# chzhang18/RAG

Hardware: AMD Instinct MI355X
Metric: disparity maps/sec at 384x1248 D=192 (Matching-Net forward) (higher is better)
Workload: dtype f32 (RAGMI_F32X3: level-3/6/12 3x3x3 convolutions with fp32 operands split into power-of-two-scaled FP16 hi+lo halves on the 16-bit matrix cores, hi*hi + hi*lo + lo*hi, fp32 accumulate: fp32-class accuracy, bound in include/rag_amd.h; strict_fp32 holds the RAGMI_F32 number); 1 GPU; BASELINE configs[1]: 1 stereo pair(s)/GPU/step, 384x1248, D=192, f32, all-conv genotype, (left_fea,right_fea)->disp, inputs resident in HBM; global_batch=1, launch=hipGraph, ranks_seen=1

## Files before the change

### include/rag_amd.h

```cpp
#ifndef RAG_AMD_H
#define RAG_AMD_H

#include <stdint.h>

#ifdef __cplusplus
extern "C" {
#endif

#define RAGMI_OK 0
#define RAGMI_EINVAL (-1)
#define RAGMI_EUNSUPPORTED (-2)
#define RAGMI_ELAUNCH (-3)

#define RAGMI_F32 0
#define RAGMI_BF16 1
#define RAGMI_F32X3 2

#define RAGMI_MAX_GROUPS 16

int ragmi_version(void);
const char* ragmi_last_error(void);

int ragmi_costvol_fwd(const void* left_fea, const void* right_fea, void* cost,
                      int B, int C, int d, int h, int w, int dtype, void* stream);

int64_t ragmi_conv3d_k3_packed_elems(int Cout, int Cin);
int ragmi_conv3d_k3_pack(const void* weight, void* packed, int Cout, int Cin, int dtype, void* stream);

int ragmi_conv3d_k3_fwd(const void* x, int64_t x_bstride,
                        const void* packed_weight, const void* scale, const void* shift, int relu,
                        void* y, int64_t y_bstride, const int32_t* y_group_ch,
                        const void* res, int64_t res_bstride, const int32_t* res_group_ch,
                        int B, int Cin, int Cout, int D, int H, int W,
                        int dtype, void* stream);

typedef struct {
  const void* weight;
  const void* scale;
  const void* shift;
  int32_t relu;
  void* y;
  int64_t y_bstride;
  int32_t y_ch0;
  int32_t cout;
} ragmi_tail_t;
int ragmi_down2_tail_supported(int D, int H, int W);

#define RAGMI_CONV_RELU 1
#define RAGMI_CONV_X_G4 2
#define RAGMI_CONV_Y_G4 4
#define RAGMI_TAIL_G4 4
#define RAGMI_TAIL_F32 8
#define RAGMI_TAIL_ROWS 16
#define RAGMI_OUT_F32 0x100
int ragmi_conv3d_k3_g4_caps(int Cin, int Cout, int B, int D, int H, int W, int nset, int ntail, int ndown, int dtype);

#define RAGMI_STORE_QUARTER_ROWS 2
int ragmi_conv3d_k3_quarter_store_supported(int Cin, int Cout, int B, int D, int H, int W, int nset, int ntail, int ndown, int dtype);
int ragmi_quarter_store_rows(int n_in, unsigned char* used);

int ragmi_conv3d_k3_fwd_ex(const void* x, int64_t x_bstride,
                           const void* packed_weight, const void* scale, const void* shift, int relu,
                           void* y, int64_t y_bstride, const int32_t* y_group_ch,
                           const void* res, int64_t res_bstride, const int32_t* res_group_ch,
                           int B, int Cin, int Cout, int D, int H, int W,
                           int store_main, int ntail, const ragmi_tail_t* tails, int dtype, void* stream);
int ragmi_conv3d_k3_dual_fwd_ex(const void* x, int64_t x_bstride,
                                int CinA, const void* packedA, const void* scaleA, const void* shiftA,
                                int CinB, const void* packedB, const void* scaleB, const void* shiftB,
                                int relu, void* y, int64_t y_bstride, const int32_t* y_group_ch,
                                const void* res, int64_t res_bstride, const int32_t* res_group_ch,
                                int B, int Cout, int D, int H, int W,
                                int store_main, int ntail, const ragmi_tail_t* tails, int dtype, void* stream);

int ragmi_conv3d_k3_small_fwd(const void* x, int64_t x_bstride, const void* weight, const void* scale,
                              const void* shift, int relu, void* y, int64_t y_bstride, int y_ch0,
                              const void* res, int64_t res_bstride, int res_ch0,
                              int B, int Cin, int Cout, int D, int H, int W, int dtype, void* stream);

int ragmi_conv3d_k3_small_fwd_ex(const void* x, int64_t x_bstride, const void* weight, const void* scale,
                                 const void* shift, int relu, void* y, int64_t y_bstride, int y_ch0,
                                 const void* res, int64_t res_bstride, int res_ch0,
                                 int B, int Cin, int Cout, int D, int H, int W, int dtype, int y_dtype, void* stream);

int ragmi_conv3d_k3_dual_fwd(const void* x, int64_t x_bstride,
                             int CinA, const void* packedA, const void* scaleA, const void* shiftA,
                             int CinB, const void* packedB, const void* scaleB, const void* shiftB,
                             int relu, void* y, int64_t y_bstride, const int32_t* y_group_ch,
                             const void* res, int64_t res_bstride, const int32_t* res_group_ch,
                             int B, int Cout, int D, int H, int W, int dtype, void* stream);

int ragmi_conv3d_k3_plan(int Cout, int B, int D, int H, int W, int nset, int32_t* log_tx,
                         int32_t* rows_per_lane, int32_t* launch_groups, int32_t max_launches);

int ragmi_conv3d_k1_fwd(const void* x, int64_t x_bstride,
                        const void* weight, const void* scale, const void* shift, int relu,
                        void* y, int64_t y_bstride, int y_ch0,
                        int B, int Cin, int Cout, int64_t DHW,
                        int dtype, void* stream);

int ragmi_conv3d_k1_chain_supported(int Cin, int Cmid, int Cout);
int ragmi_conv3d_k1_chain_fwd(const void* x, int64_t x_bstride, const void* weight1, const void* scale1, const void* shift1, int relu1,
                              int Cmid, const void* weight2, const void* scale2, const void* shift2, int relu2,
                              void* y, int64_t y_bstride, int y_ch0, int B, int Cin, int Cout, int64_t DHW, int dtype, void* stream);

int ragmi_conv3d_k1_fwd_ex(const void* x, int64_t x_bstride, const void* weight, int w_transposed, const void* scale,
                           const void* shift, int relu, void* y, int64_t y_bstride, int y_ch0, int B, int Cin,
                           int Cout, int64_t DHW, int dtype, void* stream);

int ragmi_conv3d_k1_resample_fwd(const void* x, int64_t x_bstride, int Di, int Hi, int Wi,
                                 const void* weight, const void* scale, const void* shift, int relu,
                                 void* y, int64_t y_bstride, int y_ch0,
                                 int B, int Cin, int Cout, int Do, int Ho, int Wo, int align_corners,
                                 int dtype, void* stream);

typedef struct {
  const void* x;
  int64_t x_bstride;
  int32_t Di, Hi, Wi;
  const void* weight;
  const void* scale;
  const void* shift;
  int32_t relu;
  int32_t y_ch0;
  int32_t Cin, Cout;
} ragmi_k1r_t;
int ragmi_conv3d_k1_resample_pair_fwd(const ragmi_k1r_t* a, const ragmi_k1r_t* b, void* y, int64_t y_bstride,
                                      int B, int Do, int Ho, int Wo, int align_corners, int dtype, void* stream);
int ragmi_conv3d_k1_resample_multi_fwd(const ragmi_k1r_t* const* specs, void* const* ys, const int64_t* y_bstrides, int n, int B,
                                       int Do, int Ho, int Wo, int align_corners, int dtype, void* stream);

typedef struct {
  const void* x;
  int64_t x_bstride;
  int32_t Cin, Hi, Wi;
  const void* weight;
  const void* scale;
  const void* shift;
  int32_t relu;
} ragmi_cell2d_in_t;
int ragmi_cell2d_supported(int C, int Cin0, int Cin1, int Cout, int H, int W, int dtype);
int ragmi_cell2d_fwd(const ragmi_cell2d_in_t* s0, const ragmi_cell2d_in_t* s1, int C, const void* packedA, const void* scaleA,
                     const void* shiftA, const void* packedB, const void* scaleB, const void* shiftB, int relu, void* y,
                     int64_t y_bstride, const int32_t* y_group_ch, int B, int Cout, int H, int W, int dtype, void* stream);

int ragmi_trilinear3d_fwd(const void* x, void* y, int B, int C,
                          int Di, int Hi, int Wi, int Do, int Ho, int Wo,
                          int align_corners, int dtype, void* stream);

int ragmi_upconv3d_c1_supported(int Cin, int Di, int Hi, int Wi);
int ragmi_upconv3d_c1_fwd(const void* x, int64_t x_bstride, const void* weight, const void* scale, const void* shift, int relu, void* y,
                          int64_t y_bstride, int y_ch0, int B, int Cin, int Di, int Hi, int Wi, int dtype, int y_dtype, void* stream);

int ragmi_trilinear3d_act_fwd(const void* x, int64_t x_bstride, void* y, int64_t y_bstride, int y_ch0, int relu, int B, int C,
                              int Di, int Hi, int Wi, int Do, int Ho, int Wo, int align_corners, int dtype, void* stream);

int ragmi_conv2d_k3_strided_fwd(const void* x, const void* weight, const void* scale, const void* shift, int relu,
                                void* y, int B, int Cin, int Cout, int H, int W, int stride, int dtype, void* stream);

int ragmi_add_fwd(const void* a, int64_t a_bstride, int a_ch0,
                  const void* b, int64_t b_bstride, int b_ch0,
                  void* y, int64_t y_bstride, int y_ch0,
                  int B, int C, int64_t DHW, int dtype, void* stream);

int ragmi_disp_softargmin_fwd(const void* cost, void* out, int B, int d, int h, int w,
                              int maxdisp, int Ho, int Wo, int dtype, void* stream);

int ragmi_disparity_regression_fwd(const void* prob, void* out, int B, int D, int H, int W,
                                   int dtype, void* stream);

int64_t ragmi_costvol_stem_weights_elems(int C, int Cout);
int ragmi_costvol_stem_prepare(const void* weight, void* variants, int C, int Cout, void* stream);
int64_t ragmi_costvol_stem_workspace_elems(int B, int C, int Cout, int D, int H, int W);
int ragmi_costvol_stem_fwd(const void* left, const void* right, const void* variants, const void* scale, const void* shift, int relu,
                           void* y, int64_t y_bstride, void* workspace, int B, int C, int Cout, int D, int H, int W,
                           int ntail, const ragmi_tail_t* tails, int dtype, void* stream);

int ragmi_costvol_stem_conv3d_supported(int C, int Cmid, int Cout, int B, int D, int H, int W, int ntail, int dtype);
int ragmi_costvol_stem_conv3d_fwd(const void* left, const void* right, const void* variants, const void* scale0, const void* shift0, int relu0,
                                  void* workspace, int ntail0, const ragmi_tail_t* tails0,
                                  const void* packed_weight, const void* scale, const void* shift, int relu,
                                  void* y, int64_t y_bstride, const int32_t* y_group_ch, int store_main, int ntail, const ragmi_tail_t* tails,
                                  int B, int C, int Cmid, int Cout, int D, int H, int W, int dtype, void* stream);

int ragmi_conv3d_k3_uses_x3(int Cin, int Cout, int B, int D, int H, int W, int nset, int has_res, int ntail, int dtype);

int ragmi_conv3d_k3_pack_ex(const void* weight, void* packed, int Cout, int Cin, int transpose, int planar2d, int dtype, void* stream);

int ragmi_conv3d_k3_pack_for(const void* weight, void* packed, int Cout, int Cin, int transpose, int planar2d, int for_dtype, void* stream);


int64_t ragmi_bn_workspace_elems(int B, int C, int64_t DHW);
int ragmi_bn_train_stats_fwd(const void* x, int64_t x_bstride, int B, int C, int64_t DHW, const void* gamma, const void* beta,
                             void* running_mean, void* running_var, void* num_batches_tracked, float momentum, float eps,
                             void* workspace, void* mean, void* invstd, void* scale, void* shift, void* stream);

int ragmi_bn_train_act_fwd(const void* x, int64_t x_bstride, int B, int C, int64_t DHW, const void* gamma, const void* beta,
                           void* running_mean, void* running_var, void* num_batches_tracked, float momentum, float eps, int relu,
                           void* workspace, void* mean, void* invstd, void* scale, void* shift, void* y, int64_t y_bstride, int y_ch0,
                           const void* res, int64_t res_bstride, int res_ch0, void* stream);

int ragmi_bn_act_bwd(const void* dy, int64_t dy_bstride, int dy_ch0, const void* x, int64_t x_bstride, const void* scale,
                     const void* shift, int relu, const void* mean, const void* invstd, int training, int B, int C, int64_t DHW,
                     void* workspace, void* dx, int64_t dx_bstride, void* dgamma, void* dbeta, int accumulate, void* stream);

int ragmi_bn_act_fwd(const void* x, int64_t x_bstride, const void* scale, const void* shift, int relu,
                     const void* res, int64_t res_bstride, int res_ch0,
                     void* y, int64_t y_bstride, int y_ch0, int B, int C, int64_t DHW, void* stream);

int ragmi_bn_act_bwd_coeffs(const void* dy, int64_t dy_bstride, int dy_ch0, const void* x, int64_t x_bstride,
                            const void* scale, const void* shift, int relu, const void* mean, const void* invstd, int training,
                            int B, int C, int64_t DHW, void* workspace, void* c1, void* c2, void* c3, void* dgamma, void* dbeta,
                            int accumulate, void* stream);

int ragmi_bn_act_bwd_apply(const void* dy, int64_t dy_bstride, int dy_ch0, const void* x, int64_t x_bstride,
                           const void* scale, const void* shift, int relu, const void* c1, const void* c2, const void* c3,
                           void* dx, int64_t dx_bstride, int B, int C, int64_t DHW, void* stream);

int64_t ragmi_conv3d_k3_wgrad_workspace_elems(int B, int Cin, int Cout, int D, int H, int W);
int ragmi_conv3d_k3_wgrad(const void* x, int64_t x_bstride, const void* g, int64_t g_bstride, int g_ch0, void* const* dw_list, int n_dw,
                          int accumulate, int planar2d, void* workspace, int B, int Cin, int Cout, int D, int H, int W, void* stream);

int ragmi_conv3d_k1_wgrad(const void* x, int64_t x_bstride, const void* g, int64_t g_bstride, int g_ch0, void* dw,
                          int B, int Cin, int Cout, int64_t DHW, void* stream);

int ragmi_trilinear3d_bwd(const void* dy, void* dx, int B, int C, int Di, int Hi, int Wi, int Do, int Ho, int Wo,
                          int align_corners, void* stream);

int ragmi_costvol_bwd(const void* dcost, void* dleft, void* dright, int B, int C, int d, int h, int w, void* stream);

int ragmi_disp_softargmin_bwd(const void* cost, const void* dout, void* dcost, int B, int d, int h, int w,
                              int maxdisp, int Ho, int Wo, void* stream);

int ragmi_conv2d_k3_strided_dgrad(const void* g, const void* weight, void* dx, int B, int Cin, int Cout, int H, int W, int stride,
                                  void* stream);
int ragmi_conv2d_k3_strided_wgrad(const void* x, const void* g, void* dw, int B, int Cin, int Cout, int H, int W, int stride,
                                  void* stream);

int ragmi_disparity_regression_bwd(const void* dout, void* dprob, int B, int D, int H, int W, void* stream);

int ragmi_stereo_metrics_fwd(const void* disp_est, const void* disp_gt, int B, int H, int W, float maxdisp, void* acc, void* out,
                             void* stream);

int ragmi_masked_smooth_l1_bwd(const void* disp_est, const void* disp_gt, const void* out, const void* gout, void* ddisp,
                               int B, int H, int W, float maxdisp, void* stream);

int64_t ragmi_selfsup_loss_workspace_elems(int B, int H, int W);
int ragmi_selfsup_loss_fwd(const void* left, const void* right, const void* disp, int B, int C, int H, int W, int dtype,
                           void* workspace, void* out, void* unit_grad, void* stream);

int ragmi_selfsup_loss_bwd(const void* unit_grad, const void* gout, void* grad, int64_t n, void* stream);

int ragmi_depth_head_supported(int Cin, int Hi, int Wi, int H, int W, int scale, int dtype);
int ragmi_depth_head_fwd(const void* y, const void* w3, const void* w1, const void* b1, void* out, int B, int Cin, int Hi, int Wi,
                         int H, int W, int scale, float max_depth, int dtype, void* stream);

int ragmi_depth_metrics_workspace_elems(long long n);
int ragmi_depth_metrics_fwd(const void* est, const void* gt, long long n, float variance_focus, void* workspace, void* out10, int dtype,
                            void* stream);

int64_t ragmi_depth_head_bwd_workspace_elems(int B, int Cin, int H, int W);
int ragmi_depth_head_bwd(const void* y, const void* w3, const void* w1, const void* b1, const void* d_out, void* dy, void* dw3,
                         void* dw1, void* db1, int accumulate, void* workspace, int B, int Cin, int Hi, int Wi, int H, int W, int scale,
                         float max_depth, int dtype, void* stream);

int ragmi_silog_loss_workspace_elems(long long n);
int ragmi_silog_loss_fwd(const void* est, const void* gt, long long n, float variance_focus, void* workspace, void* out, void* saved,
                         int dtype, void* stream);

int ragmi_silog_loss_bwd(const void* est, const void* gt, long long n, float variance_focus, const void* saved, const void* gout,
                         void* grad, int dtype, void* stream);

int64_t ragmi_sgd_workspace_bytes(void);
int ragmi_sgd_clip_step(void* param, void* grad, void* momentum_buf, int64_t n, float lr, float momentum, float weight_decay,
                        float max_norm, int first_step, void* workspace, void* norm_out, void* stream);

#define RAGMI_GT_F32 0
#define RAGMI_GT_U16 1
int ragmi_prep_batch(const void* left_u8, const void* right_u8, const void* gt, int gt_dtype, float gt_scale, const void* origin,
                     void* left, void* right, void* gt_out, int B, int Hs, int Ws, int H, int W, float mean0, float mean1, float mean2,
                     float std0, float std1, float std2, const void* stats_left, const void* stats_right, const void* stats_source,
                     void* stream);

int64_t ragmi_color_stats_workspace_elems(int B, int Hs, int Ws);
int ragmi_color_stats(const void* img_u8, int B, int Hs, int Ws, void* workspace, void* stats, void* stream);

int ragmi_color_transfer(const void* target_u8, const void* stats_target, const void* stats_source, void* out_u8, int B, int H, int W,
                         void* stream);

int ragmi_prep_batch_resized(const void* left_u8, const void* right_u8, const void* gt, int gt_dtype, float gt_scale, const void* origin,
                             void* left, void* right, void* gt_out, int B, int Hs, int Ws, int Hr, int Wr, int H, int W, float mean0,
                             float mean1, float mean2, float std0, float std1, float std2, const void* ybounds, const void* ytaps_i32,
                             const void* ytaps_f64, int yksize, const void* xbounds, const void* xtaps_i32, const void* xtaps_f64,
                             int xksize, void* stream);
int ragmi_resize_lanczos_u8(const void* src_u8, void* dst_u8, int B, int Hs, int Ws, int Hr, int Wr, const void* ybounds,
                            const void* ytaps_i32, int yksize, const void* xbounds, const void* xtaps_i32, int xksize, void* stream);
int ragmi_resize_lanczos_u16(const void* src_u16, void* dst_u16, int B, int Hs, int Ws, int Hr, int Wr, const void* ybounds,
                             const void* ytaps_f64, int yksize, const void* xbounds, const void* xtaps_f64, int xksize, void* stream);

int ragmi_graph_node_census(void* graph, int32_t* n_kernel, int32_t* n_memcpy, int32_t* n_memset, int32_t* n_other);

#ifdef __cplusplus
}
#endif
#endif
```

### rag_amd/_lib.py

```python
import ctypes
import os
import threading

_HERE = os.path.dirname(os.path.abspath(__file__))
_LIB = None
_LOCK = threading.Lock()

c_void_p, c_int, c_int64, c_float = ctypes.c_void_p, ctypes.c_int, ctypes.c_int64, ctypes.c_float
c_int32_p = ctypes.POINTER(ctypes.c_int32)

class TailSpec(ctypes.Structure):
    _fields_ = [("weight", c_void_p), ("scale", c_void_p), ("shift", c_void_p), ("relu", ctypes.c_int32),
                ("y", c_void_p), ("y_bstride", c_int64), ("y_ch0", ctypes.c_int32), ("cout", ctypes.c_int32)]


c_tail_p = ctypes.POINTER(TailSpec)


class K1RSpec(ctypes.Structure):
    _fields_ = [("x", c_void_p), ("x_bstride", c_int64), ("Di", ctypes.c_int32), ("Hi", ctypes.c_int32), ("Wi", ctypes.c_int32),
                ("weight", c_void_p), ("scale", c_void_p), ("shift", c_void_p), ("relu", ctypes.c_int32),
                ("y_ch0", ctypes.c_int32), ("Cin", ctypes.c_int32), ("Cout", ctypes.c_int32)]


c_k1r_p = ctypes.POINTER(K1RSpec)


class Cell2dIn(ctypes.Structure):
    _fields_ = [("x", c_void_p), ("x_bstride", c_int64), ("Cin", ctypes.c_int32), ("Hi", ctypes.c_int32), ("Wi", ctypes.c_int32),
                ("weight", c_void_p), ("scale", c_void_p), ("shift", c_void_p), ("relu", ctypes.c_int32)]


c_cell2d_p = ctypes.POINTER(Cell2dIn)

SIGNATURES = {
    "ragmi_version": (c_int, []),
    "ragmi_last_error": (ctypes.c_char_p, []),
    "ragmi_graph_node_census": (c_int, [c_void_p, c_int32_p, c_int32_p, c_int32_p, c_int32_p]),
    "ragmi_costvol_fwd": (c_int, [c_void_p, c_void_p, c_void_p, c_int, c_int, c_int, c_int, c_int, c_int, c_void_p]),
    "ragmi_costvol_stem_weights_elems": (c_int64, [c_int, c_int]),
    "ragmi_costvol_stem_prepare": (c_int, [c_void_p, c_void_p, c_int, c_int, c_void_p]),
    "ragmi_costvol_stem_workspace_elems": (c_int64, [c_int, c_int, c_int, c_int, c_int, c_int]),
    "ragmi_costvol_stem_fwd": (c_int, [c_void_p, c_void_p, c_void_p, c_void_p, c_void_p, c_int, c_void_p, c_int64, c_void_p,
                                       c_int, c_int, c_int, c_int, c_int, c_int, c_int, c_tail_p, c_int, c_void_p]),
    "ragmi_costvol_stem_conv3d_supported": (c_int, [c_int] * 9),
    "ragmi_costvol_stem_conv3d_fwd": (c_int, [c_void_p, c_void_p, c_void_p, c_void_p, c_void_p, c_int, c_void_p, c_int, c_tail_p,
                                              c_void_p, c_void_p, c_void_p, c_int, c_void_p, c_int64, c_int32_p, c_int, c_int, c_tail_p,
                                              c_int, c_int, c_int, c_int, c_int, c_int, c_int, c_int, c_void_p]),
    "ragmi_conv3d_k3_uses_x3": (c_int, [c_int] * 10),
    "ragmi_conv3d_k3_g4_caps": (c_int, [c_int] * 10),
    "ragmi_conv3d_k3_quarter_store_supported": (c_int, [c_int] * 10),
    "ragmi_quarter_store_rows": (c_int, [c_int, ctypes.POINTER(ctypes.c_ubyte)]),
    "ragmi_conv3d_k3_packed_elems": (c_int64, [c_int, c_int]),
    "ragmi_conv3d_k3_pack": (c_int, [c_void_p, c_void_p, c_int, c_int, c_int, c_void_p]),
    "ragmi_conv3d_k3_fwd": (c_int, [c_void_p, c_int64, c_void_p, c_void_p, c_void_p, c_int,
                                    c_void_p, c_int64, c_int32_p, c_void_p, c_int64, c_int32_p,
                                    c_int, c_int, c_int, c_int, c_int, c_int, c_int, c_void_p]),
    "ragmi_conv3d_k3_small_fwd": (c_int, [c_void_p, c_int64, c_void_p, c_void_p, c_void_p, c_int, c_void_p, c_int64, c_int,
                                          c_void_p, c_int64, c_int, c_int, c_int, c_int, c_int, c_int, c_int, c_int, c_void_p]),
    "ragmi_conv3d_k3_small_fwd_ex": (c_int, [c_void_p, c_int64, c_void_p, c_void_p, c_void_p, c_int, c_void_p, c_int64, c_int,
                                             c_void_p, c_int64, c_int, c_int, c_int, c_int, c_int, c_int, c_int, c_int, c_int, c_void_p]),
    "ragmi_conv3d_k3_dual_fwd": (c_int, [c_void_p, c_int64, c_int, c_void_p, c_void_p, c_void_p,
                                         c_int, c_void_p, c_void_p, c_void_p, c_int, c_void_p, c_int64, c_int32_p,
                                         c_void_p, c_int64, c_int32_p, c_int, c_int, c_int, c_int, c_int, c_int, c_void_p]),
    "ragmi_conv3d_k3_fwd_ex": (c_int, [c_void_p, c_int64, c_void_p, c_void_p, c_void_p, c_int,
                                       c_void_p, c_int64, c_int32_p, c_void_p, c_int64, c_int32_p,
                                       c_int, c_int, c_int, c_int, c_int, c_int, c_int, c_int, c_tail_p, c_int, c_void_p]),
    "ragmi_conv3d_k3_dual_fwd_ex": (c_int, [c_void_p, c_int64, c_int, c_void_p, c_void_p, c_void_p,
                                            c_int, c_void_p, c_void_p, c_void_p, c_int, c_void_p, c_int64, c_int32_p,
                                            c_void_p, c_int64, c_int32_p, c_int, c_int, c_int, c_int, c_int,
                                            c_int, c_int, c_tail_p, c_int, c_void_p]),
    "ragmi_conv3d_k3_plan": (c_int, [c_int, c_int, c_int, c_int, c_int, c_int, c_int32_p, c_int32_p, c_int32_p, c_int]),
    "ragmi_conv3d_k1_fwd": (c_int, [c_void_p, c_int64, c_void_p, c_void_p, c_void_p, c_int,
                                    c_void_p, c_int64, c_int, c_int, c_int, c_int, c_int64, c_int, c_void_p]),
    "ragmi_conv3d_k1_chain_supported": (c_int, [c_int] * 3),
    "ragmi_conv3d_k1_chain_fwd": (c_int, [c_void_p, c_int64, c_void_p, c_void_p, c_void_p, c_int, c_int, c_void_p, c_void_p, c_void_p, c_int,
                                          c_void_p, c_int64, c_int, c_int, c_int, c_int, c_int64, c_int, c_void_p]),
    "ragmi_conv3d_k1_fwd_ex": (c_int, [c_void_p, c_int64, c_void_p, c_int, c_void_p, c_void_p, c_int,
                                       c_void_p, c_int64, c_int, c_int, c_int, c_int, c_int64, c_int, c_void_p]),
    "ragmi_conv3d_k1_resample_fwd": (c_int, [c_void_p, c_int64, c_int, c_int, c_int, c_void_p, c_void_p, c_void_p, c_int,
                                             c_void_p, c_int64, c_int, c_int, c_int, c_int, c_int, c_int, c_int, c_int, c_int, c_void_p]),
    "ragmi_conv3d_k1_resample_pair_fwd": (c_int, [c_k1r_p, c_k1r_p, c_void_p, c_int64, c_int, c_int, c_int, c_int, c_int, c_int, c_void_p]),
    "ragmi_conv3d_k1_resample_multi_fwd": (c_int, [ctypes.POINTER(c_k1r_p), ctypes.POINTER(c_void_p), ctypes.POINTER(c_int64), c_int, c_int,
                                                   c_int, c_int, c_int, c_int, c_int, c_void_p]),
    "ragmi_down2_tail_supported": (c_int, [c_int, c_int, c_int]),
    "ragmi_cell2d_supported": (c_int, [c_int] * 7),
    "ragmi_cell2d_fwd": (c_int, [c_cell2d_p, c_cell2d_p, c_int, c_void_p, c_void_p, c_void_p, c_void_p, c_void_p, c_void_p, c_int,
                                 c_void_p, c_int64, c_int32_p, c_int, c_int, c_int, c_int, c_int, c_void_p]),
    "ragmi_upconv3d_c1_supported": (c_int, [c_int, c_int, c_int, c_int]),
    "ragmi_upconv3d_c1_fwd": (c_int, [c_void_p, c_int64, c_void_p, c_void_p, c_void_p, c_int, c_void_p, c_int64, c_int, c_int, c_int, c_int,
                                      c_int, c_int, c_int, c_int, c_void_p]),
    "ragmi_trilinear3d_act_fwd": (c_int, [c_void_p, c_int64, c_void_p, c_int64, c_int, c_int, c_int, c_int, c_int, c_int, c_int, c_int,
                                          c_int, c_int, c_int, c_int, c_void_p]),
    "ragmi_trilinear3d_fwd": (c_int, [c_void_p, c_void_p, c_int, c_int, c_int, c_int, c_int, c_int, c_int, c_int,
                                      c_int, c_int, c_void_p]),
    "ragmi_conv2d_k3_strided_fwd": (c_int, [c_void_p, c_void_p, c_void_p, c_void_p, c_int, c_void_p, c_int, c_int, c_int, c_int, c_int,
                                            c_int, c_int, c_void_p]),
    "ragmi_add_fwd": (c_int, [c_void_p, c_int64, c_int, c_void_p, c_int64, c_int, c_void_p, c_int64, c_int,
                              c_int, c_int, c_int64, c_int, c_void_p]),
    "ragmi_bn_workspace_elems": (c_int64, [c_int, c_int, c_int64]),
    "ragmi_bn_train_stats_fwd": (c_int, [c_void_p, c_int64, c_int, c_int, c_int64, c_void_p, c_void_p, c_void_p, c_void_p, c_void_p,
                                         c_float, c_float, c_void_p, c_void_p, c_void_p, c_void_p, c_void_p, c_void_p]),
    "ragmi_conv3d_k3_pack_ex": (c_int, [c_void_p, c_void_p, c_int, c_int, c_int, c_int, c_int, c_void_p]),
    "ragmi_conv3d_k3_pack_for": (c_int, [c_void_p, c_void_p, c_int, c_int, c_int, c_int, c_int, c_void_p]),
    "ragmi_sgd_workspace_bytes": (c_int64, []),
    "ragmi_sgd_clip_step": (c_int, [c_void_p, c_void_p, c_void_p, c_int64, c_float, c_float, c_float, c_float, c_int, c_void_p, c_void_p,
                                    c_void_p]),
    "ragmi_bn_train_act_fwd": (c_int, [c_void_p, c_int64, c_int, c_int, c_int64, c_void_p, c_void_p, c_void_p, c_void_p, c_void_p, c_float,
                                       c_float, c_int, c_void_p, c_void_p, c_void_p, c_void_p, c_void_p, c_void_p, c_int64, c_int,
                                       c_void_p, c_int64, c_int, c_void_p]),
    "ragmi_bn_act_bwd": (c_int, [c_void_p, c_int64, c_int, c_void_p, c_int64, c_void_p, c_void_p, c_int, c_void_p, c_void_p, c_int, c_int,
                                 c_int, c_int64, c_void_p, c_void_p, c_int64, c_void_p, c_void_p, c_int, c_void_p]),
    "ragmi_bn_act_fwd": (c_int, [c_void_p, c_int64, c_void_p, c_void_p, c_int, c_void_p, c_int64, c_int, c_void_p, c_int64, c_int,
                                 c_int, c_int, c_int64, c_void_p]),
    "ragmi_bn_act_bwd_coeffs": (c_int, [c_void_p, c_int64, c_int, c_void_p, c_int64, c_void_p, c_void_p, c_int, c_void_p, c_void_p, c_int,
                                        c_int, c_int, c_int64, c_void_p, c_void_p, c_void_p, c_void_p, c_void_p, c_void_p, c_int, c_void_p]),
    "ragmi_bn_act_bwd_apply": (c_int, [c_void_p, c_int64, c_int, c_void_p, c_int64, c_void_p, c_void_p, c_int, c_void_p, c_void_p,
                                       c_void_p, c_void_p, c_int64, c_int, c_int, c_int64, c_void_p]),
    "ragmi_conv3d_k3_wgrad_workspace_elems": (c_int64, [c_int, c_int, c_int, c_int, c_int, c_int]),
    "ragmi_conv3d_k3_wgrad": (c_int, [c_void_p, c_int64, c_void_p, c_int64, c_int, ctypes.POINTER(c_void_p), c_int, c_int, c_int, c_void_p,
                                      c_int, c_int, c_int, c_int, c_int, c_int, c_void_p]),
    "ragmi_conv3d_k1_wgrad": (c_int, [c_void_p, c_int64, c_void_p, c_int64, c_int, c_void_p, c_int, c_int, c_int, c_int64, c_void_p]),
    "ragmi_trilinear3d_bwd": (c_int, [c_void_p, c_void_p, c_int, c_int, c_int, c_int, c_int, c_int, c_int, c_int, c_int, c_void_p]),
    "ragmi_costvol_bwd": (c_int, [c_void_p, c_void_p, c_void_p, c_int, c_int, c_int, c_int, c_int, c_void_p]),
    "ragmi_conv2d_k3_strided_dgrad": (c_int, [c_void_p, c_void_p, c_void_p, c_int, c_int, c_int, c_int, c_int, c_int, c_void_p]),
    "ragmi_conv2d_k3_strided_wgrad": (c_int, [c_void_p, c_void_p, c_void_p, c_int, c_int, c_int, c_int, c_int, c_int, c_void_p]),
    "ragmi_disparity_regression_bwd": (c_int, [c_void_p, c_void_p, c_int, c_int, c_int, c_int, c_void_p]),
    "ragmi_stereo_metrics_fwd": (c_int, [c_void_p, c_void_p, c_int, c_int, c_int, c_float, c_void_p, c_void_p, c_void_p]),
    "ragmi_masked_smooth_l1_bwd": (c_int, [c_void_p, c_void_p, c_void_p, c_void_p, c_void_p, c_int, c_int, c_int, c_float, c_void_p]),
    "ragmi_selfsup_loss_workspace_elems": (c_int64, [c_int, c_int, c_int]),
    "ragmi_selfsup_loss_fwd": (c_int, [c_void_p, c_void_p, c_void_p, c_int, c_int, c_int, c_int, c_int, c_void_p, c_void_p, c_void_p,
                                       c_void_p]),
    "ragmi_selfsup_loss_bwd": (c_int, [c_void_p, c_void_p, c_void_p, c_int64, c_void_p]),
    "ragmi_depth_head_supported": (c_int, [c_int] * 7),
    "ragmi_depth_head_fwd": (c_int, [c_void_p, c_void_p, c_void_p, c_void_p, c_void_p, c_int, c_int, c_int, c_int, c_int, c_int, c_int,
                                     c_float, c_int, c_void_p]),
    "ragmi_depth_metrics_workspace_elems": (c_int, [ctypes.c_longlong]),
    "ragmi_depth_metrics_fwd": (c_int, [c_void_p, c_void_p, ctypes.c_longlong, c_float, c_void_p, c_void_p, c_int, c_void_p]),
    "ragmi_depth_head_bwd_workspace_elems": (c_int64, [c_int, c_int, c_int, c_int]),
    "ragmi_depth_head_bwd": (c_int, [c_void_p, c_void_p, c_void_p, c_void_p, c_void_p, c_void_p, c_void_p, c_void_p, c_void_p, c_int,
                                     c_void_p, c_int, c_int, c_int, c_int, c_int, c_int, c_int, c_float, c_int, c_void_p]),
    "ragmi_silog_loss_workspace_elems": (c_int, [ctypes.c_longlong]),
    "ragmi_silog_loss_fwd": (c_int, [c_void_p, c_void_p, ctypes.c_longlong, c_float, c_void_p, c_void_p, c_void_p, c_int, c_void_p]),
    "ragmi_silog_loss_bwd": (c_int, [c_void_p, c_void_p, ctypes.c_longlong, c_float, c_void_p, c_void_p, c_void_p, c_int, c_void_p]),
    "ragmi_prep_batch": (c_int, [c_void_p, c_void_p, c_void_p, c_int, c_float, c_void_p, c_void_p, c_void_p, c_void_p,
                                 c_int, c_int, c_int, c_int, c_int, c_float, c_float, c_float, c_float, c_float, c_float,
                                 c_void_p, c_void_p, c_void_p, c_void_p]),
    "ragmi_color_stats_workspace_elems": (c_int64, [c_int, c_int, c_int]),
    "ragmi_color_stats": (c_int, [c_void_p, c_int, c_int, c_int, c_void_p, c_void_p, c_void_p]),
    "ragmi_color_transfer": (c_int, [c_void_p, c_void_p, c_void_p, c_void_p, c_int, c_int, c_int, c_void_p]),
    "ragmi_prep_batch_resized": (c_int, [c_void_p, c_void_p, c_void_p, c_int, c_float, c_void_p, c_void_p, c_void_p, c_void_p,
                                         c_int, c_int, c_int, c_int, c_int, c_int, c_int, c_float, c_float, c_float, c_float, c_float,
                                         c_float, c_void_p, c_void_p, c_void_p, c_int, c_void_p, c_void_p, c_void_p, c_int, c_void_p]),
    "ragmi_resize_lanczos_u8": (c_int, [c_void_p, c_void_p, c_int, c_int, c_int, c_int, c_int, c_void_p, c_void_p, c_int, c_void_p,
                                        c_void_p, c_int, c_void_p]),
    "ragmi_resize_lanczos_u16": (c_int, [c_void_p, c_void_p, c_int, c_int, c_int, c_int, c_int, c_void_p, c_void_p, c_int, c_void_p,
                                         c_void_p, c_int, c_void_p]),
    "ragmi_disp_softargmin_bwd": (c_int, [c_void_p, c_void_p, c_void_p, c_int, c_int, c_int, c_int, c_int, c_int, c_int, c_void_p]),
    "ragmi_disp_softargmin_fwd": (c_int, [c_void_p, c_void_p, c_int, c_int, c_int, c_int, c_int, c_int, c_int,
                                          c_int, c_void_p]),
    "ragmi_disparity_regression_fwd": (c_int, [c_void_p, c_void_p, c_int, c_int, c_int, c_int, c_int, c_void_p]),
}


def lib_path() -> str:
    return os.environ.get("RAG_AMD_LIB", os.path.join(_HERE, "lib", "librag_amd.so"))


def load_library():
    global _LIB
    if _LIB is not None:
        return _LIB
    with _LOCK:
        if _LIB is None:
            path = lib_path()
            if not os.path.exists(path):
                raise RuntimeError(
                    f"rag_amd: HIP library not found at {path}. Build it with `make` at the repo root "
                    "(or `python -c 'import __graft_entry__ as g; g.build()'`). There is no CPU fallback.")
            lib = ctypes.CDLL(path)
            for name, (restype, argtypes) in SIGNATURES.items():
                fn = getattr(lib, name)
                fn.restype = restype
                fn.argtypes = argtypes
            _LIB = lib
    return _LIB


def check(status: int, what: str) -> None:
    if status != 0:
        msg = load_library().ragmi_last_error()
        raise RuntimeError(f"rag_amd.{what} failed with status {status}: {msg.decode() if msg else ''}")
```

### rag_amd/csrc/conv3d_c1.hip

```cpp
#include "conv3d_k3.h"

namespace ragmi {

constexpr int C1_TY = 64, C1_TX = 32, C1_THREADS = 512;
constexpr int C1_ROWS = C1_TY + 2, C1_COLS = C1_TX;
constexpr int C1_TILE = C1_ROWS * C1_COLS, C1_EDGE = C1_ROWS * 2;
constexpr int C1_NB = 2 * C1_TX + 2 * C1_ROWS;
static_assert(C1_TY * (C1_TX / 4) == C1_THREADS && C1_NB <= C1_THREADS, "staging map");
constexpr int C1_MAX_CIN = 64;
constexpr int64_t C1_MIN_VOXELS = 1 << 18;
#ifndef C1_ZSEG_OVERRIDE
constexpr int C1_ZSEG = 4;
#else
constexpr int C1_ZSEG = C1_ZSEG_OVERRIDE;
#endif

struct C1Args {
  const void* x;
  const float* w;
  const float* scale;
  const float* shift;
  void* y;
  int64_t x_bstride, y_bstride;
  int y_ch0, relu;
  int B, Cin, D, H, W;
  int tiles_x, tiles_y, nseg, nwork;
};

template <class T, class TO, int ZSEG>
__global__ __launch_bounds__(C1_THREADS, 2) void conv3d_c1_kernel(C1Args a) {
  constexpr int NP = ZSEG + 2;
  constexpr int NPS = (NP + 5) / 6 * 6;
  __shared__ __attribute__((aligned(16))) float tile[2][C1_TILE];
  __shared__ float edge[2][C1_EDGE];
  __shared__ __attribute__((aligned(16))) float wl[C1_MAX_CIN * 28];
  const int tid = threadIdx.x, tx = tid & 7, ty = tid >> 3;
  const int chunk = (a.nwork + 7) / 8, j = blockIdx.x;
  int t = (j & 7) * chunk + (j >> 3);
  if ((j >> 3) >= chunk || t >= a.nwork) return;
  const int x0 = (t % a.tiles_x) * C1_TX; t /= a.tiles_x;
  const int y0 = (t % a.tiles_y) * C1_TY; t /= a.tiles_y;
  const int seg = t % a.nseg, b = t / a.nseg;
  const int zs = seg * ZSEG, ze = min(a.D, zs + ZSEG);
  const int HW = a.H * a.W;
  const int64_t DHW = (int64_t)HW * a.D;
  for (int i = tid; i < a.Cin * 28; i += C1_THREADS) wl[i] = (i % 28) < 27 ? a.w[(i / 28) * 27 + i % 28] : 0.f;
  int offA, dstA, offB, dstB;
  bool okA, okB;
  {
    const int r = 1 + (tid >> 3), q = tid & 7, gy = y0 - 1 + r, gx = x0 + 4 * q;
    dstA = r * C1_COLS + 4 * q;
    okA = gy < a.H && gx + 3 < a.W;
    offA = okA ? gy * a.W + gx : 0;
  }
  {
    const int e = min(tid, C1_NB - 1);
    int r, gx;
    if (e < 2 * C1_TX) { r = e < C1_TX ? 0 : C1_ROWS - 1; gx = x0 + (e & (C1_TX - 1)); dstB = r * C1_COLS + (e & (C1_TX - 1)); }
    else { r = (e - 2 * C1_TX) >> 1; const int side = (e - 2 * C1_TX) & 1; gx = side ? x0 + C1_TX : x0 - 1; dstB = C1_TILE + r * 2 + side; }
    const int gy = y0 - 1 + r;
    okB = tid < C1_NB && (unsigned)gy < (unsigned)a.H && (unsigned)gx < (unsigned)a.W;
    offB = okB ? gy * a.W + gx : 0;
  }
  const bool hasB = tid < C1_NB;
  float* const pB[2] = {dstB < C1_TILE ? tile[0] + dstB : edge[0] + (dstB - C1_TILE), dstB < C1_TILE ? tile[1] + dstB : edge[1] + (dstB - C1_TILE)};
  const T* const xb = static_cast<const T*>(a.x) + (int64_t)b * a.x_bstride;
  float pfA[3][4], pfB[3];
  auto plane_live = [&](int zi) { const int z = zs - 1 + zi; return zi < NP && z >= 0 && z <= min(ze, a.D - 1); };
  auto prefetch = [&](int c, int zi, int slot) {
#ifdef C1_DIAG_NOLOAD
    return;
#endif
    const T* const pc = xb + (int64_t)min(c, a.Cin - 1) * DHW + (int64_t)min(max(zs - 1 + zi, 0), a.D - 1) * HW;
    ld4(pc + offA, pfA[slot]);
    pfB[slot] = ld(pc + offB);
  };
  auto commit = [&](int buf, int slot) {
    *reinterpret_cast<float4*>(tile[buf] + dstA) = okA ? make_float4(pfA[slot][0], pfA[slot][1], pfA[slot][2], pfA[slot][3]) : make_float4(0.f, 0.f, 0.f, 0.f);
    if (hasB) *pB[buf] = okB ? pfB[slot] : 0.f;
  };
  float acc[ZSEG][4];
#pragma unroll
  for (int k = 0; k < ZSEG; ++k)
#pragma unroll
    for (int i = 0; i < 4; ++i) acc[k][i] = 0.f;
  prefetch(0, 0, 0);
  prefetch(0, 1, 1);
  prefetch(0, 2, 2);
  commit(0, 0);
  __syncthreads();
  const float4* const my4 = reinterpret_cast<const float4*>(&tile[0][0]) + ty * (C1_COLS / 4) + tx;
  const float* const myedge = &edge[0][0] + ty * 2 + (tx == 7 ? 1 : 0);
  const bool left_edge = tx == 0, right_edge = tx == 7;
  for (int c = 0; c < a.Cin; ++c) {
    float w[28];
#pragma unroll
    for (int i = 0; i < 28; i += 4) {
      const float4 q = *reinterpret_cast<const float4*>(wl + c * 28 + i);
      w[i] = q.x; w[i + 1] = q.y; w[i + 2] = q.z; w[i + 3] = q.w;
    }
    static_for<NPS>([&](auto zi_) {
      constexpr int zi = decltype(zi_)::value;
      if constexpr ((zi + 3) % NPS < NP) prefetch(zi + 3 < NPS ? c : c + 1, (zi + 3) % NPS, zi % 3);
#ifdef C1_DIAG_NOFMA
      if (false) {
#else
      if (plane_live(zi)) {
#endif
        float in[3][6];
#pragma unroll
        for (int r = 0; r < 3; ++r) {
#ifdef C1_DIAG_NOLDS
          const float4 m = make_float4(pfA[0][0] + r, pfA[1][1], pfA[2][2], pfA[0][3] + zi);
          const float e = pfB[0];
#else
          const float4 m = my4[(zi & 1) * (C1_TILE / 4) + r * (C1_COLS / 4)];
          const float e = myedge[(zi & 1) * C1_EDGE + r * 2];
#endif
          const float fl = __int_as_float(__builtin_amdgcn_update_dpp(0, __float_as_int(m.w), 0x111, 0xF, 0xF, false));
          const float fr = __int_as_float(__builtin_amdgcn_update_dpp(0, __float_as_int(m.x), 0x101, 0xF, 0xF, false));
          in[r][0] = left_edge ? e : fl; in[r][1] = m.x; in[r][2] = m.y; in[r][3] = m.z; in[r][4] = m.w; in[r][5] = right_edge ? e : fr;
        }
        static_for<3>([&](auto dz_) {
          constexpr int dz = decltype(dz_)::value, k = zi - dz;
          if constexpr (zi < NP && k >= 0 && k < ZSEG) {
            if (zs + k < ze) {
#pragma unroll
              for (int dy = 0; dy < 3; ++dy)
#pragma unroll
                for (int dx = 0; dx < 3; ++dx)
#pragma unroll
                  for (int i = 0; i < 4; ++i) acc[k][i] = fmaf(w[dz * 9 + dy * 3 + dx], in[dy][i + dx], acc[k][i]);
            }
          }
        });
      }
      if constexpr ((zi + 1) % NPS < NP) commit((zi + 1) & 1, (zi + 1) % 3);
#ifndef C1_DIAG_NOBARRIER
      __syncthreads();
#endif
    });
  }
  const float sc = a.scale ? a.scale[0] : 1.f, sh = a.shift ? a.shift[0] : 0.f;
  TO* const yb = static_cast<TO*>(a.y) + (int64_t)b * a.y_bstride + (int64_t)a.y_ch0 * DHW;
  const int gx = x0 + 4 * tx, gy = y0 + ty;
  if (gy < a.H && gx < a.W) {
#pragma unroll
    for (int k = 0; k < ZSEG; ++k) {
      if (zs + k >= ze) continue;
      float v[4];
#pragma unroll
      for (int i = 0; i < 4; ++i) {
        const float u = fmaf(acc[k][i], sc, sh);
        v[i] = a.relu ? fmaxf(u, 0.f) : u;
      }
      st4(yb + (int64_t)(zs + k) * HW + gy * a.W + gx, v);
    }
  }
}

constexpr int CU_TY = 64, CU_TX = 32, CU_THREADS = 256, CU_ZSEG = 4;
constexpr int CU_PZ = CU_ZSEG / 2 + 2, CU_PY = CU_TY / 2 + 2, CU_PX = CU_TX / 2 + 2, CU_RS = CU_PX + 2;
constexpr int CU_BLK = CU_PZ * CU_PY * CU_RS;
constexpr int CU_NPF = (CU_PZ * CU_PY * CU_PX + CU_THREADS - 1) / CU_THREADS;

struct CUArgs {
  const void* x;
  const float* w;
  const float* scale;
  const float* shift;
  void* y;
  int64_t x_bstride, y_bstride;
  int y_ch0, relu;
  int B, Cin, Di, Hi, Wi;
  float sd, sh, sw;
  int tiles_x, tiles_y, nseg, nwork;
};

template <class T, class TO>
__global__ __launch_bounds__(CU_THREADS, 2) void upconv3d_c1_kernel(CUArgs a) {
  constexpr int ZSEG = CU_ZSEG, NP = ZSEG + 2;
  __shared__ __attribute__((aligned(16))) float blk[2][CU_BLK];
  __shared__ __attribute__((aligned(16))) float wl[C1_MAX_CIN * 28];
  const int tid = threadIdx.x, tx = tid & 7, ty = tid >> 3;
  const int D = 2 * a.Di, H = 2 * a.Hi, W = 2 * a.Wi;
  const int chunk = (a.nwork + 7) / 8, j = blockIdx.x;
  int t = (j & 7) * chunk + (j >> 3);
  if ((j >> 3) >= chunk || t >= a.nwork) return;
  const int x0 = (t % a.tiles_x) * CU_TX; t /= a.tiles_x;
  const int y0 = (t % a.tiles_y) * CU_TY; t /= a.tiles_y;
  const int seg = t % a.nseg, b = t / a.nseg;
  const int zs = seg * ZSEG, ze = min(D, zs + ZSEG);
  const int HWi = a.Hi * a.Wi;
  const int64_t DHWi = (int64_t)HWi * a.Di;
  for (int i = tid; i < a.Cin * 28; i += CU_THREADS) wl[i] = (i % 28) < 27 ? a.w[(i / 28) * 27 + i % 28] : 0.f;
  const int pz0 = zs / 2 - 1, py0 = y0 / 2 - 1, px0 = x0 / 2 - 1;
  int soff[CU_NPF];
#pragma unroll
  for (int p = 0; p < CU_NPF; ++p) {
    const int e = min(tid + p * CU_THREADS, CU_PZ * CU_PY * CU_PX - 1);
    const int cx = e % CU_PX, cy = (e / CU_PX) % CU_PY, cz = e / (CU_PX * CU_PY);
    soff[p] = min(max(pz0 + cz, 0), a.Di - 1) * HWi + min(max(py0 + cy, 0), a.Hi - 1) * a.Wi + min(max(px0 + cx, 0), a.Wi - 1);
  }
  const T* const xb = static_cast<const T*>(a.x) + (int64_t)b * a.x_bstride;
  float pf[CU_NPF];
  auto prefetch = [&](int c) {
    const T* const pc = xb + (int64_t)min(c, a.Cin - 1) * DHWi;
#pragma unroll
    for (int p = 0; p < CU_NPF; ++p) pf[p] = ld(pc + soff[p]);
  };
  auto commit = [&](float* buf) {
#pragma unroll
    for (int p = 0; p < CU_NPF; ++p) {
      const int e = tid + p * CU_THREADS;
      if (e < CU_PZ * CU_PY * CU_PX) buf[(e / CU_PX) * CU_RS + e % CU_PX] = pf[p];
    }
  };
  float wy0[4], wy1[4], wx0[6], wx1[6];
  bool ylow[4], xlow[6];
#pragma unroll
  for (int r = 0; r < 4; ++r) {
    const int gy = y0 + 2 * ty - 1 + r;
    const LinIdx l = lin_index(min(max(gy, 0), H - 1), a.Hi, H, a.sh, 1);
    const int expect = py0 + ty + (r >= 2 ? 1 : 0);
    ylow[r] = l.i0 < expect;
    const bool in = (unsigned)gy < (unsigned)H;
    wy0[r] = in ? l.w0 : 0.f; wy1[r] = in ? l.w1 : 0.f;
  }
#pragma unroll
  for (int i = 0; i < 6; ++i) {
    const int gx = x0 + 4 * tx - 1 + i;
    const LinIdx l = lin_index(min(max(gx, 0), W - 1), a.Wi, W, a.sw, 1);
    const int expect = px0 + 2 * tx + (i >= 4 ? 2 : (i >= 2 ? 1 : 0));
    xlow[i] = l.i0 < expect;
    const bool in = (unsigned)gx < (unsigned)W;
    wx0[i] = in ? l.w0 : 0.f; wx1[i] = in ? l.w1 : 0.f;
  }
  float acc[ZSEG][2][4];
#pragma unroll
  for (int k = 0; k < ZSEG; ++k)
#pragma unroll
    for (int r = 0; r < 2; ++r)
#pragma unroll
      for (int i = 0; i < 4; ++i) acc[k][r][i] = 0.f;
  prefetch(0);
  commit(blk[0]);
  __syncthreads();
  const int wbase = ty * CU_RS + 2 * tx;
  for (int c = 0; c < a.Cin; ++c) {
    const float* const cur = blk[c & 1];
    prefetch(c + 1);
    float w[28];
#pragma unroll
    for (int i = 0; i < 28; i += 4) {
      const float4 q = *reinterpret_cast<const float4*>(wl + c * 28 + i);
      w[i] = q.x; w[i + 1] = q.y; w[i + 2] = q.z; w[i + 3] = q.w;
    }
    static_for<NP>([&](auto zi_) {
      constexpr int zi = decltype(zi_)::value;
      const int z = zs - 1 + zi;
      if (z >= 0 && z <= min(ze, D - 1)) {
        const LinIdx lz = lin_index(z, a.Di, D, a.sd, 1);
        const int pa = lz.i0 - pz0, pb = lz.i1 - pz0;
        float in[4][6];
        {
          float rz[3][4];
#pragma unroll
          for (int rr = 0; rr < 3; ++rr) {
            const float* const qa = cur + pa * (CU_PY * CU_RS) + wbase + rr * CU_RS;
            const float* const qb = cur + pb * (CU_PY * CU_RS) + wbase + rr * CU_RS;
            const float2 a0 = *reinterpret_cast<const float2*>(qa), a1 = *reinterpret_cast<const float2*>(qa + 2);
            const float2 b0 = *reinterpret_cast<const float2*>(qb), b1 = *reinterpret_cast<const float2*>(qb + 2);
            rz[rr][0] = lerp2(lz.w0, a0.x, lz.w1, b0.x); rz[rr][1] = lerp2(lz.w0, a0.y, lz.w1, b0.y);
            rz[rr][2] = lerp2(lz.w0, a1.x, lz.w1, b1.x); rz[rr][3] = lerp2(lz.w0, a1.y, lz.w1, b1.y);
          }
          float yv[4][4];
#pragma unroll
          for (int r = 0; r < 4; ++r)
#pragma unroll
            for (int q = 0; q < 4; ++q) {
              const float lo = r >= 2 ? (ylow[r] ? rz[0][q] : rz[1][q]) : rz[0][q];
              const float hi = r >= 2 ? (ylow[r] ? rz[1][q] : rz[2][q]) : rz[1][q];
              yv[r][q] = lerp2(wy0[r], lo, wy1[r], hi);
            }
#pragma unroll
          for (int r = 0; r < 4; ++r)
#pragma unroll
            for (int i = 0; i < 6; ++i) {
              const int e = i >= 4 ? 2 : (i >= 2 ? 1 : 0);
              const float lo = e > 0 ? (xlow[i] ? yv[r][e - 1] : yv[r][e]) : yv[r][e];
              const float hi = e > 0 ? (xlow[i] ? yv[r][e] : yv[r][e + 1]) : yv[r][e + 1];
              in[r][i] = lerp2(wx0[i], lo, wx1[i], hi);
            }
        }
        static_for<3>([&](auto dz_) {
          constexpr int dz = decltype(dz_)::value, k = zi - dz;
          if constexpr (k >= 0 && k < ZSEG) {
            if (zs + k < ze) {
#pragma unroll
              for (int r = 0; r < 2; ++r)
#pragma unroll
                for (int dy = 0; dy < 3; ++dy)
#pragma unroll
                  for (int dx = 0; dx < 3; ++dx)
#pragma unroll
                    for (int i = 0; i < 4; ++i) acc[k][r][i] = fmaf(w[dz * 9 + dy * 3 + dx], in[r + dy][i + dx], acc[k][r][i]);
            }
          }
        });
      }
    });
    commit(blk[(c + 1) & 1]);
    __syncthreads();
  }
  const float sc = a.scale ? a.scale[0] : 1.f, sh = a.shift ? a.shift[0] : 0.f;
  const int64_t HW = (int64_t)H * W;
  TO* const yb = static_cast<TO*>(a.y) + (int64_t)b * a.y_bstride + (int64_t)a.y_ch0 * HW * D;
  const int gx = x0 + 4 * tx;
#pragma unroll
  for (int k = 0; k < ZSEG; ++k) {
    if (zs + k >= ze) continue;
#pragma unroll
    for (int r = 0; r < 2; ++r) {
      const int gy = y0 + 2 * ty + r;
      if (gy >= H || gx >= W) continue;
      float v[4];
#pragma unroll
      for (int i = 0; i < 4; ++i) {
        const float u = fmaf(acc[k][r][i], sc, sh);
        v[i] = a.relu ? fmaxf(u, 0.f) : u;
      }
      st4(yb + (int64_t)(zs + k) * HW + (int64_t)gy * W + gx, v);
    }
  }
}

template <class T, class TO>
static int upconv_launch_typed(CUArgs a, hipStream_t st) {
  const int D = 2 * a.Di, H = 2 * a.Hi, W = 2 * a.Wi;
  a.tiles_x = (int)ceil_div(W, CU_TX); a.tiles_y = (int)ceil_div(H, CU_TY); a.nseg = (int)ceil_div(D, CU_ZSEG);
  const int64_t nwork = (int64_t)a.tiles_x * a.tiles_y * a.nseg * a.B;
  RAGMI_REQUIRE(nwork < (1ll << 28), RAGMI_EUNSUPPORTED, "upconv3d_c1: too many tiles");
  a.nwork = (int)nwork;
  hipLaunchKernelGGL((upconv3d_c1_kernel<T, TO>), dim3((unsigned)(ceil_div(nwork, 8) * 8)), dim3(CU_THREADS), 0, st, a);
  return check_launch("upconv3d_c1");
}

}

extern "C" int ragmi_upconv3d_c1_supported(int Cin, int Di, int Hi, int Wi) {
  using namespace ragmi;
  return (Cin >= 1 && Cin <= C1_MAX_CIN && Di >= 2 && Hi >= 2 && Wi >= 2 && (2 * Wi) % 4 == 0 && (int64_t)Cin * Di * Hi * Wi < (1ll << 31)) ? 1 : 0;
}

extern "C" int ragmi_upconv3d_c1_fwd(const void* x, int64_t x_bstride, const void* weight, const void* scale, const void* shift, int relu,
                                     void* y, int64_t y_bstride, int y_ch0, int B, int Cin, int Di, int Hi, int Wi, int dtype, int y_dtype,
                                     void* stream) {
  using namespace ragmi;
  RAGMI_REQUIRE(x && weight && y, RAGMI_EINVAL, "upconv3d_c1: null pointer");
  RAGMI_REQUIRE((scale == nullptr) == (shift == nullptr), RAGMI_EINVAL, "upconv3d_c1: scale/shift must both be given or both NULL");
  RAGMI_REQUIRE(B > 0 && B <= 65535 && y_ch0 >= 0, RAGMI_EINVAL, "upconv3d_c1: bad size");
  RAGMI_REQUIRE(dtype_ok(dtype) && (y_dtype == dtype || (dtype == RAGMI_BF16 && y_dtype == RAGMI_F32)), RAGMI_EUNSUPPORTED,
                "upconv3d_c1: dtype %d -> %d not built", dtype, y_dtype);
  RAGMI_REQUIRE(ragmi_upconv3d_c1_supported(Cin, Di, Hi, Wi), RAGMI_EUNSUPPORTED,
                "upconv3d_c1: needs 1..%d input channels, every input axis >= 2 and an even input width", C1_MAX_CIN);
  RAGMI_REQUIRE(y_bstride % 4 == 0 && aligned4(y, y_dtype), RAGMI_EUNSUPPORTED, "upconv3d_c1: output rows must be 16-byte aligned");
  CUArgs a{};
  a.x = x; a.w = (const float*)weight; a.scale = (const float*)scale; a.shift = (const float*)shift; a.y = y;
  a.x_bstride = x_bstride; a.y_bstride = y_bstride; a.y_ch0 = y_ch0; a.relu = relu ? 1 : 0;
  a.B = B; a.Cin = Cin; a.Di = Di; a.Hi = Hi; a.Wi = Wi;
  a.sd = lin_scale(Di, 2 * Di, 1); a.sh = lin_scale(Hi, 2 * Hi, 1); a.sw = lin_scale(Wi, 2 * Wi, 1);
  hipStream_t st = static_cast<hipStream_t>(stream);
  if (dtype == RAGMI_BF16) return y_dtype == RAGMI_F32 ? upconv_launch_typed<bf16_t, float>(a, st) : upconv_launch_typed<bf16_t, bf16_t>(a, st);
  return upconv_launch_typed<float, float>(a, st);
}

namespace ragmi {

bool c1_eligible(const K3Args& a, int dtype, int y_dtype) {
#ifdef C1_DISABLE
  return false;
#endif
  if (a.Cout != 1 || a.res != nullptr || a.Cin > C1_MAX_CIN || a.W % 4 != 0) return false;
  if ((int64_t)a.D * a.H * a.W < C1_MIN_VOXELS || (int64_t)a.Cin * a.D * a.H * a.W >= (1ll << 31)) return false;
  return a.x_bstride % 4 == 0 && a.y_bstride % 4 == 0 && aligned4(a.x, dtype) && aligned4(a.y, y_dtype);
}

template <class T, class TO>
static int c1_launch_typed(const C1Args& a, hipStream_t st) {
  constexpr int ZSEG = C1_ZSEG;
  C1Args b = a;
  b.tiles_x = (int)ceil_div(a.W, C1_TX); b.tiles_y = (int)ceil_div(a.H, C1_TY); b.nseg = (int)ceil_div(a.D, ZSEG);
  const int64_t nwork = (int64_t)b.tiles_x * b.tiles_y * b.nseg * a.B;
  RAGMI_REQUIRE(nwork < (1ll << 28), RAGMI_EUNSUPPORTED, "conv3d_c1: too many tiles");
  b.nwork = (int)nwork;
  const unsigned grid = (unsigned)(ceil_div(nwork, 8) * 8);
  hipLaunchKernelGGL((conv3d_c1_kernel<T, TO, ZSEG>), dim3(grid), dim3(C1_THREADS), 0, st, b);
  return check_launch("conv3d_c1");
}

int c1_launch(const K3Args& k, int dtype, int y_dtype, hipStream_t st) {
  C1Args a{};
  a.x = k.x; a.w = k.wp[0]; a.scale = k.scale[0]; a.shift = k.shift[0]; a.y = k.y;
  a.x_bstride = k.x_bstride; a.y_bstride = k.y_bstride; a.y_ch0 = k.y_ch[0]; a.relu = k.relu & 1;
  a.B = k.B; a.Cin = k.Cin; a.D = k.D; a.H = k.H; a.W = k.W;
  if (dtype == RAGMI_BF16) return y_dtype == RAGMI_F32 ? c1_launch_typed<bf16_t, float>(a, st) : c1_launch_typed<bf16_t, bf16_t>(a, st);
  return c1_launch_typed<float, float>(a, st);
}

}
```

### rag_amd/modules.py

```python
from __future__ import annotations

from collections import namedtuple
from types import MappingProxyType
from typing import Dict, List, Optional, Sequence, Tuple

import numpy as np

import torch
import torch.nn as nn

from . import autograd as ag
from . import ops

Genotype = namedtuple("Genotype_2D", "normal normal_concat reduce reduce_concat")
PRIMITIVES_3D = ["skip_connect_3d", "3d_conv_3x3"]

ALL_CONV_ROWS = np.array([[0, 1], [1, 1], [2, 1], [3, 1], [5, 1], [6, 1]])
ALL_SKIP_ROWS = np.array([[0, 0], [1, 0], [2, 0], [3, 0], [5, 0], [6, 0]])
ALL_CONV_GENOTYPE = Genotype(normal=ALL_CONV_ROWS, normal_concat=None, reduce=ALL_CONV_ROWS, reduce_concat=None)


def _volume(size) -> int:
    n = 1
    for v in size:
        n *= int(v)
    return n


ALL_SKIP_GENOTYPE = Genotype(normal=ALL_SKIP_ROWS, normal_concat=None, reduce=ALL_SKIP_ROWS, reduce_concat=None)


class Identity_3d(nn.Module):

    def forward(self, x):
        return x


class _ConvBR(nn.Module):

    NDIM = 3

    def __init__(self, C_in, C_out, kernel_size, stride, padding, bn=True, relu=True):
        super().__init__()
        self.relu = relu
        self.use_bn = bn
        if self.NDIM == 3:
            self.conv = nn.Conv3d(C_in, C_out, kernel_size, stride=stride, padding=padding, bias=False)
            self.bn = nn.BatchNorm3d(C_out)
        else:
            self.conv = nn.Conv2d(C_in, C_out, kernel_size, stride=stride, padding=padding, bias=False)
            self.bn = nn.BatchNorm2d(C_out)
        self._initialize_weights()
        self._cache = None

    def _initialize_weights(self):
        nn.init.kaiming_normal_(self.conv.weight, mode="fan_out", nonlinearity="relu")
        nn.init.constant_(self.bn.weight, 1)
        nn.init.constant_(self.bn.bias, 0)

    def _geometry(self) -> int:
        k, n = self.conv.kernel_size, self.NDIM
        same = self.conv.padding == tuple((ki - 1) // 2 for ki in k) and self.conv.dilation == (1,) * n and self.conv.groups == 1
        if same and k in ((1,) * n, (3,) * n) and self.conv.stride == (1,) * n:
            return k[0]
        if same and n == 2 and k == (3, 3) and self.conv.stride[0] == self.conv.stride[1] > 1:
            return -3
        raise NotImplementedError("rag_amd ConvBR: only 1x1(x1)/pad0 and 3x3(x3)/pad1 at stride 1 (plus the strided 2-D 3x3 "
                                  "stem) are built (everything the reference instantiates)")

    def _small(self) -> bool:
        return (self.NDIM == 3 and self.conv.out_channels <= 2 and self.conv.in_channels % 4 == 0
                and self.conv.in_channels <= 128)

    def stamp(self) -> tuple:
        w, bn = self.conv.weight, self.bn
        return (w.data_ptr(), w._version, bn.weight._version, bn.bias._version, bn.running_mean._version,
                bn.running_var._version, bn.weight.data_ptr(), str(w.device), self.use_bn)

    def prepared(self) -> Tuple[torch.Tensor, Optional[torch.Tensor], Optional[torch.Tensor]]:
        if self.use_bn and self.bn.training:
            raise RuntimeError("rag_amd ConvBR: folded BatchNorm parameters requested in train mode (internal error: "
                               "train-mode units run through rag_amd.autograd)")
        stamp = self.stamp()
        if self._cache is None or self._cache[0] != stamp:
            k = self._geometry()
            w = self.conv.weight.detach()
            with torch.no_grad():
                if k == -3 or (k == 3 and self._small()):
                    wk = w.contiguous()
                elif k == 3:
                    wk = ops.conv3d_k3_pack(w)
                else:
                    wk = w.reshape(w.shape[0], w.shape[1]).contiguous()
                if self.use_bn:
                    bn = self.bn
                    scale = (bn.weight.detach() * torch.rsqrt(bn.running_var.detach() + bn.eps)).float().contiguous()
                    shift = (bn.bias.detach() - bn.running_mean.detach() * scale).float().contiguous()
                else:
                    scale = shift = None
            self._cache = (stamp, wk, scale, shift)
        return self._cache[1], self._cache[2], self._cache[3]

    def autograd_mode(self, *inputs) -> bool:
        return (ag.needs_grad(*inputs, self.conv.weight, self.bn.weight, self.bn.bias)
                or (self.use_bn and self.bn.training))

    def _forward_autograd(self, x: torch.Tensor, resample_to: Optional[Sequence[int]]) -> torch.Tensor:
        if x.dtype != torch.float32:
            raise NotImplementedError("rag_amd: the training path is fp32 (bf16 storage is inference only)")
        if self._geometry() == -3:
            return ag.StridedStemFn.apply(x if x.dim() == 4 else x.squeeze(2), self.conv.weight, self.bn.weight, self.bn.bias, self)
        squeeze = x.dim() == 4
        if squeeze:
            x = x.unsqueeze(2)
        if resample_to is not None:
            x = ag.resample(x, resample_to, True)
        y = ag.ConvBRFn.apply(x, self.conv.weight, self.bn.weight, self.bn.bias, self)
        return y.squeeze(2) if squeeze else y

    def costvol_fusable(self, C_fea: int) -> bool:
        return (self.NDIM == 3 and self._geometry() == 3 and self.conv.in_channels == 2 * C_fea and C_fea <= 16
                and self.conv.out_channels <= 16)

    def costvol_variants(self) -> torch.Tensor:
        w = self.conv.weight
        key = (w.data_ptr(), w._version, str(w.device))
        hit = getattr(self, "_cv_cache", None)
        if hit is None or hit[0] != key:
            with torch.no_grad():
                hit = (key, ops.costvol_stem_prepare(w.detach()))
            self._cv_cache = hit
        return hit[1]

    def forward_costvol(self, left_fea, right_fea, maxdisp, tails=None, out_g4: bool = False) -> torch.Tensor:
        _wk, scale, shift = self.prepared()
        return ops.costvol_stem(left_fea, right_fea, maxdisp, self.costvol_variants(), self.conv.out_channels, scale, shift,
                                self.relu, tails=tails, out_g4=out_g4)

    def as_tail(self, out: torch.Tensor, out_ch0: int, g4: bool = False) -> "ops.Tail":
        if self._geometry() != 1 or self.conv.out_channels > 4:
            raise ValueError("only 1x1x1 ConvBR with <= 4 output channels can be fused as a tail")
        wk, scale, shift = self.prepared()
        return ops.Tail(wk, scale, shift, self.relu, out, out_ch0, g4=g4)

    def as_down_tails(self, out: torch.Tensor, out_ch0: int) -> List["ops.Tail"]:
        if self._geometry() != 1 or self.conv.out_channels > 8:
            raise ValueError("only 1x1x1 ConvBR with <= 8 output channels can be fused as down-sampling tails")
        wk, scale, shift = self.prepared()
        tails = []
        for c0 in range(0, self.conv.out_channels, 4):
            c1 = min(c0 + 4, self.conv.out_channels)
            tails.append(ops.Tail(wk[c0:c1], None if scale is None else scale[c0:c1], None if shift is None else shift[c0:c1],
                                  self.relu, out, out_ch0 + c0, down=True))
        return tails

    def forward(self, x: torch.Tensor, out: Optional[torch.Tensor] = None, out_ch0: int = 0,
                resample_to: Optional[Sequence[int]] = None, tails: Optional[Sequence["ops.Tail"]] = None,
                store_main: bool = True, out_dtype: Optional[torch.dtype] = None, x_g4: bool = False) -> torch.Tensor:
        if self.autograd_mode(x):
            if out is not None or tails:
                raise RuntimeError("rag_amd ConvBR: fused destinations/tails belong to the inference executor")
            return self._forward_autograd(x, resample_to)
        k = self._geometry()
        wk, scale, shift = self.prepared()
        cout = self.conv.out_channels
        if x_g4 and (k != 3 or self._small() or resample_to is not None or x.dim() != 5):
            raise RuntimeError("rag_amd ConvBR: a G4 input is taken by the 3x3x3 form only")
        if k == -3:
            return ops.conv2d_k3_strided(x if x.dim() == 4 else x[:, :, 0], wk, scale, shift, self.relu, self.conv.stride[0])
        squeeze = x.dim() == 4
        if squeeze:
            x = x.unsqueeze(2)
        mixed = out is not None and out.dtype != x.dtype
        if mixed:
            if k != 1 or x.dtype != torch.bfloat16 or out.dtype != torch.float32:
                raise RuntimeError("rag_amd ConvBR: only a 1x1x1 conv crosses from bf16 storage to an fp32 destination")
            resample_to = tuple(x.shape[2:]) if resample_to is None else resample_to
        elif resample_to is not None and tuple(resample_to) == tuple(x.shape[2:]):
            resample_to = None
        if resample_to is not None:
            if k != 1:
                raise NotImplementedError("ConvBR: fused resample is built for the 1x1x1 form only")
            if out is None:
                out = torch.empty((x.shape[0], cout) + tuple(int(v) for v in resample_to), device=x.device, dtype=x.dtype)
            if not mixed and _volume(resample_to) > _volume(x.shape[2:]) and cout <= x.shape[1]:
                low = torch.empty((x.shape[0], cout) + tuple(x.shape[2:]), device=x.device, dtype=x.dtype)
                ops.conv3d_k1(x, wk, scale, shift, False, low)
                ops.trilinear3d_act(low, resample_to, True, self.relu, out, out_ch0)
            else:
                ops.conv3d_k1_resample(x, resample_to, True, wk, scale, shift, self.relu, out, out_ch0)
            return out[:, :, 0] if squeeze else out
        if out is None:
            odt = out_dtype if (out_dtype is not None and k == 3 and self._small()) else x.dtype
            out = torch.empty((x.shape[0], cout) + tuple(x.shape[2:]), device=x.device, dtype=odt)
        if k == 3 and self._small():
            ops.conv3d_k3_small(x, wk, scale, shift, self.relu, out, out_ch0)
        elif k == 3:
            groups = [out_ch0 + 4 * g for g in range(ops.packed_groups(cout))]
            ops.conv3d_k3(x, wk, cout, scale, shift, self.relu, out, groups, tails=tails, store_main=store_main, x_g4=x_g4)
        else:
            ops.conv3d_k1(x, wk, scale, shift, self.relu, out, out_ch0)
        return out[:, :, 0] if squeeze else out


class ConvBR_3d(_ConvBR):
    NDIM = 3


class ConvBR_2d(_ConvBR):
    NDIM = 2


class Identity_2d(nn.Module):

    def forward(self, x):
        return x


def _skip(C, stride):
    if stride != 1:
        raise NotImplementedError("skip_connect_3d with stride != 1 is dead code in the reference (FactorizedReduce typo)")
    return Identity_3d()


OPS_3d = {
    "skip_connect_3d": _skip,
    "3d_conv_3x3": lambda C, stride: ConvBR_3d(C, C, 3, stride, 1),
}


PRIMITIVES = ["skip_connect_2d", "conv_3x3"]


def _skip_2d(C, stride):
    if stride != 1:
        raise NotImplementedError("skip_connect_2d with stride != 1 is dead code in the reference")
    return Identity_2d()


OPS_2d = {"skip_connect_2d": _skip_2d, "conv_3x3": lambda C, stride: ConvBR_2d(C, C, 3, stride, 1)}


class DisparityRegression(nn.Module):

    def __init__(self, maxdisp):
        super().__init__()
        self.maxdisp = maxdisp

    def forward(self, x):
        assert x.is_contiguous() is True
        if ag.needs_grad(x):
            return ag.DispRegFn.apply(x, self.maxdisp)
        return ops.disparity_regression(x, self.maxdisp)


class Disp(nn.Module):

    def __init__(self, maxdisp=192):
        super().__init__()
        self.maxdisp = maxdisp
        self.softmax = nn.Softmin(dim=1)
        self.disparity = DisparityRegression(maxdisp=self.maxdisp)

    def forward(self, x):
        if ag.needs_grad(x):
            return ag.DispFn.apply(x, self.maxdisp)
        return ops.disp_softargmin(x, self.maxdisp)


class _Cell(nn.Module):

    def __init__(self, steps, block_multiplier, prev_prev_fmultiplier, prev_filter_multiplier, genotype,
                 filter_multiplier, downup_sample):
        super().__init__()
        self.genotype = genotype
        self.C_in = block_multiplier * filter_multiplier
        self.C_out = filter_multiplier
        self.C_prev = int(block_multiplier * prev_filter_multiplier)
        self.C_prev_prev = int(block_multiplier * prev_prev_fmultiplier)
        self.downup_sample = downup_sample
        self.pre_preprocess = self.CONV(self.C_prev_prev, self.C_out, 1, 1, 0)
        self.preprocess = self.CONV(self.C_prev, self.C_out, 1, 1, 0)
        self._steps = steps
        self.block_multiplier = block_multiplier
        self._ops = nn.ModuleList()
        if downup_sample == -1:
            self.scale = 0.5
        elif downup_sample == 1:
            self.scale = 2
        for x in self._rows():
            self._ops.append(self.OPS[self.PRIMS[x[1]]](self.C_out, stride=1))
        self._fused_cache: Dict[tuple, tuple] = {}

    def _rows(self):
        raise NotImplementedError

    def scale_dimension(self, dim, scale):
        return int((float(dim) - 1.0) * scale + 1.0) if dim % 2 == 1 else int(float(dim) * scale)

    def _contributions(self) -> Dict[int, List[Tuple[int, nn.Module]]]:
        selected = set(int(v) for v in np.asarray(self._rows())[:, 0])
        contribs: Dict[int, List[Tuple[int, nn.Module]]] = {}
        offset, n_states, ops_index = 0, 2, 0
        for _ in range(self._steps):
            lst = []
            for j in range(n_states):
                if offset + j in selected:
                    lst.append((j, self._ops[ops_index]))
                    ops_index += 1
            contribs[n_states] = lst
            offset += n_states
            n_states += 1
        return contribs

    def _fused(self, mods: Sequence[ConvBR_3d]):
        key = tuple(id(m) for m in mods)
        stamps = tuple(m.stamp() for m in mods)
        hit = self._fused_cache.get(key)
        if hit is None or hit[0] != stamps:
            prep = [m.prepared() for m in mods]
            if len(mods) == 1:
                fused = prep[0]
            else:
                with torch.no_grad():
                    wk = ops.conv3d_k3_pack(torch.cat([m.conv.weight.detach() for m in mods]))
                fused = (wk, torch.cat([p[1] for p in prep]), torch.cat([p[2] for p in prep]))
            hit = (stamps, fused)
            self._fused_cache[key] = hit
        return hit[1]

    def _convbrs(self):
        units = self.__dict__.get("_convbr_cache")
        if units is None:
            units = [m for m in self.modules() if isinstance(m, _ConvBR)]
            self.__dict__["_convbr_cache"] = units
        return units

    def autograd_mode(self, *inputs) -> bool:
        units = self._convbrs()
        if torch.is_grad_enabled():
            if any(t is not None and t.requires_grad for t in inputs):
                return True
            if any(m.conv.weight.requires_grad or m.bn.weight.requires_grad or m.bn.bias.requires_grad for m in units):
                return True
        return any(m.use_bn and m.bn.training for m in units)

    def forward(self, prev_prev_input, prev_input):
        run = self._run_autograd if self.autograd_mode(prev_prev_input, prev_input) else self._run
        if prev_input.dim() == 4:
            return prev_input, run(prev_prev_input.unsqueeze(2), prev_input.unsqueeze(2)).squeeze(2)
        return prev_input, run(prev_prev_input, prev_input)

    def _run_autograd(self, prev_prev_input, prev_input):
        s0, s1 = prev_prev_input, prev_input
        if self.downup_sample != 0:
            s1 = ag.resample(s1, self.out_size(s1.shape[2:]), True)
        s0 = ag.resample(s0, s1.shape[2:], True)
        if s0.shape[1] != self.C_out:
            s0 = self.pre_preprocess(s0)
        s1 = self.preprocess(s1)
        states = [s0, s1]
        contribs = self._contributions()
        n_states = 2 + self._steps
        pending: Dict[int, list] = {k: [] for k in contribs}
        for k, lst in contribs.items():
            if not lst:
                raise ValueError("Cell_3d: a step with no selected branch (the reference fails in torch.cat here too)")
        for j in range(n_states):
            if j >= 2:
                acc = pending[j][0]
                for h in pending[j][1:]:
                    acc = ag.AddFn.apply(acc, h)
                states.append(acc)
            out_ops = [(k, op) for k, lst in contribs.items() for (src, op) in lst if src == j]
            convs = [(k, op) for (k, op) in out_ops if isinstance(op, _ConvBR)]
            grouped = (len(convs) > 1 and all(op._geometry() == 3 and op.use_bn and op.relu for _k, op in convs)
                       and states[j].dtype == torch.float32)
            if grouped:
                params = [p for _k, op in convs for p in (op.conv.weight, op.bn.weight, op.bn.bias)]
                fuse = all(len(pending[k]) == 1 and pending[k][0].dtype == torch.float32 for k, _op in convs)
                res = [pending[k][0] for k, _op in convs] if fuse else []
                outs = dict(zip([k for k, _op in convs],
                                ag.ConvBRGroupFn.apply(states[j], tuple(op for _k, op in convs), *params, *res)))
                if fuse:
                    for k, _op in convs:
                        pending[k].clear()
            for k, op in out_ops:
                pending[k].append(outs[k] if (grouped and isinstance(op, _ConvBR)) else op(states[j]))
        return torch.cat(states[-self.block_multiplier:], dim=1)

    def out_size(self, prev_size: Sequence[int]) -> Tuple[int, int, int]:
        if self.downup_sample == 0:
            return tuple(int(v) for v in prev_size)
        return tuple(self.scale_dimension(int(v), self.scale) for v in prev_size)

    def dual_branches(self, s0_in_pre: bool):
        contribs = self._contributions()
        a, b = ([(k, op) for k, lst in contribs.items() for (src, op) in lst if src == j and isinstance(op, _ConvBR)] for j in (0, 1))
        first_cat = 2 + self._steps - self.block_multiplier
        if not (a and s0_in_pre and [k for k, _ in a] == [k for k, _ in b] and all(len(contribs[k]) == 2 for k, _ in a)
                and len({k >= first_cat for k, _ in a}) == 1):
            return None, None, False
        return a, b, len(a) == self._steps and self.block_multiplier == self._steps

    def _run(self, prev_prev_input, prev_input, plan: Optional["_CellPlan"] = None, pre: Optional[torch.Tensor] = None,
             tails: Optional[Sequence["ops.Tail"]] = None):
        C = self.C_out
        if C % 4 != 0 or self.block_multiplier > self._steps:
            raise NotImplementedError("rag_amd.Cell_3d: filter_multiplier must be a multiple of 4 and "
                                      "block_multiplier <= steps (true for every cell the reference builds)")
        s0, s1 = prev_prev_input, prev_input
        pre_has = plan.has if plan is not None else (False, False)
        a, b, whole = self.dual_branches(pre_has[0] or s0.shape[1] != C)
        if plan is None:
            plan = _CellPlan(size=self.out_size(s1.shape[2:]), dtype=s1.dtype, has=pre_has, g4=False, dual=whole, store_main=True, tails=False,
                             shared_pre=False, quarter=False)
        size = tuple(int(v) for v in plan.size)
        if not pre_has[0] and s0.shape[1] == C and tuple(s0.shape[2:]) != size:
            s0 = ops.trilinear3d(s0, size, True)
        D, H, W = size
        if (D == 1 and whole and pre is None and not tails and plan.store_main and s0.shape[1] != C and s1.dtype == torch.float32
                and s0.dtype == torch.float32 and ops.get_conv_precision() == "f16x3"
                and ops.cell2d_supported(C, s0.shape[1], s1.shape[1], C * self._steps, H, W)):
            cat = torch.empty((s1.shape[0], self.block_multiplier * C, D, H, W), device=s1.device, dtype=s1.dtype)
            pa, sa, ha = self._fused([op for _k, op in a])
            pb, sb, hb = self._fused([op for _k, op in b])
            groups = [(k - 2) * C + 4 * g for k, _op in a for g in range(C // 4)]
            ops.cell2d(s0, self.pre_preprocess.prepared() + (self.pre_preprocess.relu,), s1,
                       self.preprocess.prepared() + (self.preprocess.relu,), C, pa, sa, ha, pb, sb, hb, C * self._steps, True, cat, groups)
            return cat
        if pre is None:
            pre = torch.empty((s1.shape[0], 2 * C, D, H, W), device=s1.device, dtype=plan.dtype)
        B, dev, adt = pre.shape[0], pre.device, pre.dtype
        n_states = 2 + self._steps
        first_cat = n_states - self.block_multiplier
        contribs = self._contributions()
        cat = (pre if not plan.store_main else
               torch.empty((B, self.block_multiplier * C, D, H, W), device=dev, dtype=adt))
        scratch = (torch.empty((B, (first_cat - 2) * C, D, H, W), device=dev, dtype=adt)
                   if first_cat > 2 else None)

        where: List[Tuple[torch.Tensor, int]] = []
        grows = any(s is not None and _volume(size) > _volume(s.shape[2:]) and C <= s.shape[1] for s in (s0, s1))
        if not pre_has[0] and not pre_has[1] and s0.shape[1] != C and not grows and s0.dtype == s1.dtype == adt:
            w0, sc0, sh0 = self.pre_preprocess.prepared()
            w1, sc1, sh1 = self.preprocess.prepared()
            ops.conv3d_k1_resample_pair([(s0, w0, sc0, sh0, self.pre_preprocess.relu, 0),
                                         (s1, w1, sc1, sh1, self.preprocess.relu, C)], size, pre)
            where.append((pre, 0))
        else:
            if pre_has[0]:
                where.append((pre, 0))
            elif s0.shape[1] != C:
                self.pre_preprocess(s0, out=pre, out_ch0=0, resample_to=size)
                where.append((pre, 0))
            else:
                where.append((s0.contiguous(), 0))
            if not pre_has[1]:
                self.preprocess(s1, out=pre, out_ch0=C, resample_to=size)
        where.append((pre, C))
        for k in range(2, n_states):
            where.append((cat, (k - first_cat) * C) if k >= first_cat else (scratch, (k - 2) * C))

        written = {k: False for k in contribs}
        pending_id = {k: [j for (j, op) in lst if not isinstance(op, _ConvBR)] for k, lst in contribs.items()}
        for k, lst in contribs.items():
            if not lst:
                raise ValueError("Cell_3d: a step with no selected branch (the reference fails in torch.cat here too)")

        def finalize(k: int) -> None:
            buf, ch = where[k]
            ids = pending_id[k]
            while ids:
                if not written[k]:
                    if len(ids) >= 2:
                        (ba, ca), (bb, cb) = where[ids[0]], where[ids[1]]
                        ops.add(ba, ca, bb, cb, buf, ch, C)
                        del ids[:2]
                    else:
                        bs, cs = where[ids.pop(0)]
                        torch.mul(bs[:, cs:cs + C], 1, out=buf[:, ch:ch + C])
                    written[k] = True
                else:
                    bs, cs = where[ids.pop(0)]
                    ops.add(buf, ch, bs, cs, buf, ch, C)

        done = set()
        if a is not None:
            pa, sa, ha = self._fused([op for _k, op in a])
            pb, sb, hb = self._fused([op for _k, op in b])
            groups = [where[k][1] + 4 * g for k, _op in a for g in range(C // 4)]
            ops.conv3d_k3_dual(pre, C, pa, sa, ha, pb, sb, hb, C * len(a), True, where[a[0][0]][0], groups,
                               tails=tails, store_main=plan.store_main, x_g4=plan.g4, quarter=plan.quarter)
            for j, branches in enumerate((a, b)):
                for k, op in branches:
                    written[k] = True
                    done.add((j, id(op)))

        for j in range(n_states):
            if j >= 2:
                finalize(j)
            parts: Dict[object, list] = {}
            for k, lst in contribs.items():
                for (src, op) in lst:
                    if src != j or not isinstance(op, _ConvBR) or (j, id(op)) in done:
                        continue
                    if written[k]:
                        res = where[k]
                    else:
                        ready = [i for i in pending_id[k] if i <= j]
                        if ready:
                            pending_id[k].remove(ready[0])
                            res = where[ready[0]]
                        else:
                            res = None
                    written[k] = True
                    parts.setdefault(None if res is None else id(res[0]), []).append((k, op, res))
            if not parts:
                continue
            xbuf, xch = where[j]
            x = xbuf[:, xch:xch + C]
            for items in parts.values():
                mods = [op for (_k, op, _r) in items]
                packed, scale, shift = self._fused(mods)
                out_groups, res_groups = [], []
                for (k, _op, res) in items:
                    out_groups += [where[k][1] + 4 * g for g in range(C // 4)]
                    if res is not None:
                        res_groups += [res[1] + 4 * g for g in range(C // 4)]
                res_buf = items[0][2][0] if items[0][2] is not None else None
                by_buf: Dict[int, list] = {}
                for idx, (k, _op, _res) in enumerate(items):
                    by_buf.setdefault(id(where[k][0]), []).append(idx)
                if len(by_buf) == 1:
                    ops.conv3d_k3(x, packed, C * len(mods), scale, shift, True, where[items[0][0]][0], out_groups,
                                  res_buf, res_groups if res_buf is not None else None)
                else:
                    for idxs in by_buf.values():
                        sub = [items[i] for i in idxs]
                        p2, s2, h2 = self._fused([op for (_k, op, _r) in sub])
                        og = [where[k][1] + 4 * g for (k, _o, _r) in sub for g in range(C // 4)]
                        rg = [r[1] + 4 * g for (_k, _o, r) in sub if r is not None for g in range(C // 4)]
                        ops.conv3d_k3(x, p2, C * len(sub), s2, h2, True, where[sub[0][0]][0], og,
                                      res_buf, rg if res_buf is not None else None)
        for k in contribs:
            finalize(k)
        return cat if plan.store_main else None


class Cell_3d(_Cell):
    CONV, OPS, PRIMS = ConvBR_3d, OPS_3d, PRIMITIVES_3D

    def _rows(self):
        return self.genotype.reduce


class Cell_2d(_Cell):
    CONV, OPS, PRIMS = ConvBR_2d, OPS_2d, PRIMITIVES

    def _rows(self):
        return self.genotype.normal


_CELL3D_ARCH = ((4, 4, 4, 0), (4, 4, 4, 0), (4, 4, 4, 0), (4, 4, 8, -1),
                (4, 8, 16, -1), (8, 16, 8, 1), (16, 8, 16, -1), (8, 16, 16, 0))


_CellPlan = namedtuple("_CellPlan", "size dtype has g4 dual store_main tails shared_pre quarter")
_ChainPlan = namedtuple("_ChainPlan", "sizes cdt consumers stored cells stem0_g4 stems_fused stem_tail_rows")


def _down_tail_ok(prod, cons, B, src, dst, src_dt, dst_dt) -> bool:
    return ((src_dt != torch.float32 or ops.get_conv_precision() == "f16x3")
            and (dst_dt == src_dt or (src_dt == torch.bfloat16 and dst_dt == torch.float32))
            and tuple(2 * v for v in dst) == tuple(src) and ops.down2_tail_supported(*src)
            and cons.C_out <= 8 and cons.C_out % 4 == 0 and prod.downup_sample == 0 and prod.C_out == 4 and prod.C_out * prod._steps <= 16
            and ops.conv3d_k3_uses_x3(2 * prod.C_out, prod.C_out * prod._steps, B, *src, nset=2, ntail=1, dtype=src_dt))


def _plan_chain(stem0, stem1, cells, B: int, C_fea: int, vol, adt: torch.dtype, folded: bool) -> _ChainPlan:
    n = len(cells)
    f32, bf16 = torch.float32, torch.bfloat16
    caps = ops.conv3d_k3_g4_caps
    x3 = (adt == f32 and ops.get_conv_precision() == "f16x3") or adt == bf16
    sizes, cdt = {-2: tuple(vol), -1: tuple(vol)}, {-2: adt, -1: adt}
    cout = {-2: stem0.conv.out_channels, -1: stem1.conv.out_channels}
    for i, c in enumerate(cells):
        sizes[i] = c.out_size(sizes[i - 1])
        deep = adt == bf16 and ops.bf16_deep_fp32_enabled() and (
            _volume(sizes[i]) * ops.bf16_deep_fp32_ratio() <= _volume(vol) or f32 in (cdt[i - 1], cdt[i - 2]))
        cdt[i] = f32 if deep else adt
        cout[i] = c.block_multiplier * c.C_out

    consumers = {}
    for i in range(-2, n):
        found = []
        for j, role in ((i + 1, 1), (i + 2, 0)):
            c = cells[j] if 0 <= j < n else None
            if c is None or (role == 0 and (c.C_prev_prev == c.C_out or (j > 0 and cells[j - 1].downup_sample != 0))):
                continue
            if c.downup_sample == 0 and c.C_out == 4 and cdt[j] == cdt[i]:
                found.append((j, role, False))
            elif c.downup_sample == -1 and i >= 0 and _down_tail_ok(cells[i], c, B, sizes[i], sizes[j], cdt[i], cdt[j]):
                found.append((j, role, True))
        consumers[i] = tuple(found)
    nfull = {i: sum(not d for (_j, _r, d) in consumers[i]) for i in consumers}
    ndown = {i: sum((cells[j].C_out + 3) // 4 for (j, _r, d) in consumers[i] if d) for i in consumers}
    dual = [c.dual_branches((i, 0, False) in consumers[i - 2] or (i, 0, True) in consumers[i - 2] or cout[i - 2] != c.C_out)[2]
            for i, c in enumerate(cells)]
    tails = {i: bool(consumers[i]) and dual[i] and cout[i] <= 16 for i in range(n)}
    tails[-2] = tails[-1] = True

    g4_ok = x3 and ops.g4_enabled()
    writes = {i: bool(g4_ok and nfull[i] and tails[i]
                      and caps(2 * c.C_out, cout[i], B, *sizes[i], nset=2, ntail=nfull[i], ndown=ndown[i], dtype=cdt[i]) & 2)
              for i, c in enumerate(cells)}
    writes[-2] = bool(g4_ok and nfull[-2] and (folded or caps(stem0.conv.in_channels, cout[-2], B, *vol, nset=1, ntail=nfull[-2], dtype=adt) & 2))
    writes[-1] = bool(g4_ok and nfull[-1] and caps(cout[-2], cout[-1], B, *vol, nset=1, ntail=nfull[-1], dtype=adt) & 2)
    g4 = [bool((j, 1, False) in consumers[j - 1] and (j, 0, False) in consumers[j - 2] and writes[j - 1] and writes[j - 2] and dual[j]
               and caps(2 * c.C_out, cout[j], B, *sizes[j], nset=2, ntail=nfull[j] if tails[j] else 0, ndown=ndown[j] if tails[j] else 0,
                        dtype=cdt[j]) & 1) for j, c in enumerate(cells)]
    changed = True
    while changed:
        changed = False
        for i in range(-2, n):
            js = [j for (j, _r, d) in consumers[i] if not d]
            if len({g4[j] for j in js}) > 1:
                for j in js:
                    g4[j] = False
                changed = True
    alone = folded and (0, 0, False) in consumers[-2]
    stem0_g4 = bool(g4_ok and alone and caps(cout[-2], cout[-1], B, *vol, nset=1, ntail=nfull[-1], dtype=adt) & 1)
    stems_fused = bool(x3 and alone and ops.stem_fusion_enabled() and cout[-2] == 12 and stem1._geometry() == 3 and not stem1._small()
                       and ops.costvol_stem_conv3d_supported(C_fea, 12, cout[-1], B, *vol, ntail=nfull[-1], dtype=adt))
    stem_tail_rows = stems_fused and ops.stem_tail_rows_enabled() and cout[-1] == 12

    stored = {i: i == n - 1 or not tails[i] or len(consumers[i]) < sum(0 <= j < n for j in (i + 1, i + 2)) for i in range(-1, n)}
    stored[-2] = not stems_fused
    quarter = {i: bool(ops.quarter_store_enabled() and 0 <= i and i + 2 < n and stored[i] and tails[i] and dual[i]
                       and consumers[i] == ((i + 1, 1, True),) and cdt[i] == cdt[i + 2] == f32 and ops.get_conv_precision() == "f16x3"
                       and cells[i + 2].C_prev_prev != cells[i + 2].C_out
                       and tuple(4 * v for v in sizes[i + 2]) == tuple(sizes[i])
                       and ops.quarter_store_supported(2 * cells[i].C_out, cout[i], B, *sizes[i], nset=2, ntail=0, ndown=ndown[i], dtype=cdt[i]))
               for i in range(n)}
    has = [[False, False] for _ in cells]
    plans = []
    for i in range(-2, n):
        if i >= 0:
            j = i + 1
            shared = (j < n and not any(has[i]) and not has[j][0] and sizes[i] == sizes[j] != sizes[i - 1] and stored[i - 2] and stored[i - 1]
                      and cout[i - 2] != cells[i].C_out and cout[i - 1] != cells[j].C_out and len({cdt[i - 2], cdt[i - 1], cdt[i], cdt[j]}) == 1
                      and _volume(sizes[i]) <= min(_volume(sizes[i - 2]), _volume(sizes[i - 1])))
            if shared:
                has[i], has[j][0] = [True, True], True
            plans.append(_CellPlan(sizes[i], cdt[i], tuple(has[i]), g4[i], dual[i], stored[i], tails[i], shared, quarter[i]))
        for (j, role, _d) in consumers[i]:
            has[j][role] = True
    ro = MappingProxyType
    return _ChainPlan(ro(sizes), ro(cdt), ro(consumers), ro(stored), tuple(plans), stem0_g4, stems_fused, stem_tail_rows)


class MatchingNet(nn.Module):

    def __init__(self, genotype=ALL_CONV_GENOTYPE, maxdisp: int = 192):
        super().__init__()
        self._init_matching(genotype, maxdisp)

    def _init_matching(self, genotype, maxdisp):
        self._step = 3
        self._block_multiplier = 3
        self._filter_multiplier = 4
        self._num_layers_3d = 8
        initial_fm = self._filter_multiplier * self._block_multiplier
        if not hasattr(self, "length"):
            self.length, self.arch_init = {}, {}
        for name in ("stem_3d0", "stem_3d1", "last_3_3d", "last_6_3d", "last_12_3d"):
            self.length[name] = 1
            self.arch_init[name] = [0]
        self.cells_3d = nn.ModuleList()
        self.stem3d0 = nn.ModuleList([ConvBR_3d(initial_fm * 2, initial_fm, 3, stride=1, padding=1)])
        self.stem3d1 = nn.ModuleList([ConvBR_3d(initial_fm, initial_fm, 3, stride=1, padding=1)])
        for i in range(self._num_layers_3d):
            self.cells_3d.append(nn.ModuleList([self._new_cell_3d(i, genotype)]))
            self.arch_init["cell_3d" + str(i)] = [0]
            self.length["cell_3d" + str(i)] = 1
        self.last_3_3d = nn.ModuleList([ConvBR_3d(initial_fm, 1, 3, 1, 1, bn=False, relu=False)])
        self.last_6_3d = nn.ModuleList([ConvBR_3d(initial_fm * 2, initial_fm, 1, 1, 0)])
        self.last_12_3d = nn.ModuleList([ConvBR_3d(initial_fm * 4, initial_fm * 2, 1, 1, 0)])
        self.maxdisp = maxdisp
        self.disp = Disp(self.maxdisp)

    def _new_cell_3d(self, i: int, genotype) -> Cell_3d:
        pp, p, fm, du = _CELL3D_ARCH[i]
        return Cell_3d(self._step, self._block_multiplier, pp, p, genotype, fm, du)

    def matching(self, x, task_arch, path=None, features=None):
        def unit(name):
            return task_arch[name][0] if task_arch is not None else None

        cells = []
        for i, cell in enumerate(self.cells_3d):
            arch_cell = None
            if task_arch is not None:
                arch_cell = task_arch["cell_3d" + str(i)][0]
            elif path is not None:
                arch_cell = path[i + 1]
            cells.append(cell[arch_cell])
        last = self._run_chain(x, self.stem3d0[unit("stem_3d0")], self.stem3d1[unit("stem_3d1")], cells, features)
        return self._head(self._vol_size(x, features), last, unit("last_3_3d"), unit("last_6_3d"), unit("last_12_3d"))

    def search_matching(self, x, selected_ops, t, features=None):
        cells = [cell[selected_ops[i + 10]] for i, cell in enumerate(self.cells_3d)]
        last = self._run_chain(x, self.stem3d0[selected_ops[8]], self.stem3d1[selected_ops[9]], cells, features)
        return self._head(self._vol_size(x, features), last, t, t, t)

    def _vol_size(self, x, features):
        if x is not None:
            return tuple(x.shape[2:])
        return (int(self.maxdisp / 3),) + tuple(features[0].shape[2:])

    def _run_chain(self, x, stem0, stem1, cells, features=None):
        train = (stem0.autograd_mode(*(features if x is None else (x,))) or stem1.autograd_mode()
                 or any(c.autograd_mode() for c in cells))
        if x is None and (train or not stem0.costvol_fusable(features[0].shape[1])):
            x = self.cost_volume(*features)
        if train:
            out = (stem0(x),)
            out = (out[0], stem1(out[0]))
            for c in cells:
                out = c(out[0], out[1])
            return out[-1]
        n = len(cells)
        ref = x if x is not None else features[0]
        B, dev = ref.shape[0], ref.device
        plan = _plan_chain(stem0, stem1, cells, B, ref.shape[1], self._vol_size(x, features), ref.dtype, x is None)
        sizes, keep1 = plan.sizes, plan.stored[-1]
        self.last_g4_plan = {"pre": {j: cp.g4 for j, cp in enumerate(plan.cells)}, "stem0_out": plan.stem0_g4,
                             "stems_fused": plan.stems_fused, **({"stem_tail_rows": plan.stem_tail_rows} if plan.stems_fused else {}),
                             "quarter": {j: cp.quarter for j, cp in enumerate(plan.cells)}}
        pre: Dict[int, torch.Tensor] = {}

        def buf(j):
            if j not in pre:
                pre[j] = torch.empty((B, 2 * cells[j].C_out) + sizes[j], device=dev, dtype=plan.cdt[j])
            return pre[j]

        def unit(j, role):
            return cells[j].preprocess if role else cells[j].pre_preprocess, buf(j), cells[j].C_out * role

        def tails(i):
            out = []
            for (j, role, down) in plan.consumers[i]:
                mod, dst, ch0 = unit(j, role)
                out += mod.as_down_tails(dst, ch0) if down else [mod.as_tail(dst, ch0, g4=plan.cells[j].g4)]
            return out or None

        T: Dict[int, Optional[torch.Tensor]] = {-2: None}
        t0, t1 = tails(-2), tails(-1)
        if plan.stems_fused:
            _w0, scale0, shift0 = stem0.prepared()
            wk1, scale1, shift1 = stem1.prepared()
            cout1 = stem1.conv.out_channels
            if plan.stem_tail_rows:
                key = (stem1.stamp(), cells[0].pre_preprocess.stamp())
                hit = getattr(stem1, "_rows_cache", None)
                if hit is None or hit[0] != key:
                    with torch.no_grad():
                        hit = (key, ops.conv3d_k3_pack(ops.stem_tail_rows_weight(stem1.conv.weight.detach(), t0[0].weight2d)))
                    stem1._rows_cache = hit
                wk1 = hit[1]
            out1 = torch.empty((B, cout1) + sizes[-1], device=dev, dtype=ref.dtype) if keep1 else None
            ops.costvol_stem_conv3d(features[0], features[1], self.maxdisp, stem0.costvol_variants(), 12, scale0, shift0, stem0.relu, t0,
                                    wk1, cout1, scale1, shift1, stem1.relu, out1, [4 * g for g in range(ops.packed_groups(cout1))],
                                    tails=t1, store_main=keep1, tail0_rows=plan.stem_tail_rows)
        else:
            if x is None:
                T[-2] = stem0.forward_costvol(features[0], features[1], self.maxdisp, tails=t0, out_g4=plan.stem0_g4)
            else:
                T[-2] = stem0(x, tails=t0)
            out1 = stem1(T[-2], tails=t1, store_main=keep1, x_g4=plan.stem0_g4)
        T[-1] = out1 if keep1 else None
        for i, (c, cp) in enumerate(zip(cells, plan.cells)):
            if cp.shared_pre:
                cj = cells[i + 1]
                ops.conv3d_k1_resample_multi([(T[i - 2],) + c.pre_preprocess.prepared() + (c.pre_preprocess.relu, buf(i), 0),
                                              (T[i - 1],) + c.preprocess.prepared() + (c.preprocess.relu, buf(i), c.C_out),
                                              (T[i - 1],) + cj.pre_preprocess.prepared() + (cj.pre_preprocess.relu, buf(i + 1), 0)], sizes[i])
            T[i] = c._run(T[i - 2], T[i - 1], cp, pre.get(i), tails(i) if cp.tails else None)
            if not cp.tails:
                for (j, role, down) in plan.consumers[i]:
                    mod, dst, ch0 = unit(j, role)
                    mod(T[i], out=dst, out_ch0=ch0, resample_to=sizes[j] if down else None)
            T.pop(i - 2, None)
        return T[n - 1]

    def _head(self, vol, last_output, i3, i6, i12):
        d, h, w = vol
        f32 = torch.float32
        if last_output.size()[3] == h:
            return self.last_3_3d[i3](last_output, out_dtype=f32)
        heads = (self.last_3_3d[i3], self.last_6_3d[i6], self.last_12_3d[i12])
        up = ag.resample if any(m.autograd_mode(last_output) for m in heads) else ops.trilinear3d
        def up_last3(y):
            m3 = self.last_3_3d[i3]
            if (up is ops.trilinear3d and m3._small() and m3.conv.out_channels == 1 and tuple(y.shape[2:]) == (d // 2, h // 2, w // 2)
                    and (d, h, w) == (2 * (d // 2), 2 * (h // 2), 2 * (w // 2)) and ops.upconv3d_c1_supported(y.shape[1], d // 2, h // 2, w // 2)):
                wk, scale, shift = m3.prepared()
                return ops.upconv3d_c1(y, wk, scale, shift, m3.relu, out_dtype=f32)
            return m3(up(y, (d, h, w), True), out_dtype=f32)

        if last_output.size()[3] == h // 2:
            return up_last3(self.last_6_3d[i6](last_output))
        if last_output.size()[3] == h // 4:
            m12 = self.last_12_3d[i12]
            if (last_output.dtype == torch.bfloat16 and ops.bf16_head_fp32_enabled() and not m12.autograd_mode(last_output)
                    and m12._geometry() == 1):
                y12 = m12(last_output, out=torch.empty((last_output.shape[0], m12.conv.out_channels) + tuple(last_output.shape[2:]),
                                                       device=last_output.device, dtype=f32))
            else:
                m6 = self.last_6_3d[i6]
                half = (d // 2, h // 2, w // 2)
                if (up is ops.trilinear3d and m12._geometry() == 1 and m6._geometry() == 1 and ops.chain_k1_enabled()
                        and _volume(half) > _volume(last_output.shape[2:]) and m6.conv.out_channels <= m6.conv.in_channels
                        and ops.conv3d_k1_chain_supported(m12.conv.in_channels, m12.conv.out_channels, m6.conv.out_channels)):
                    w1, s1, h1 = m12.prepared()
                    w2, s2, h2 = m6.prepared()
                    low = torch.empty((last_output.shape[0], m6.conv.out_channels) + tuple(last_output.shape[2:]), device=last_output.device,
                                      dtype=last_output.dtype)
                    ops.conv3d_k1_chain(last_output, w1, s1, h1, m12.relu, w2, s2, h2, False, low)
                    y = torch.empty((last_output.shape[0], m6.conv.out_channels) + half, device=last_output.device, dtype=last_output.dtype)
                    ops.trilinear3d_act(low, half, True, m6.relu, y, 0)
                    return up_last3(y)
                y12 = m12(last_output)
            y = self.last_6_3d[i6](y12, resample_to=(d // 2, h // 2, w // 2))
            return up_last3(y)
        raise ValueError("MatchingNet: feature height must be a multiple of 4 (input H a multiple of 12)")

    def cost_volume(self, left_fea, right_fea):
        if ag.needs_grad(left_fea, right_fea):
            return ag.CostVolFn.apply(left_fea, right_fea, self.maxdisp)
        return ops.costvol(left_fea, right_fea, self.maxdisp)

    def forward(self, left_fea, right_fea, task_arch=None):
        if task_arch is None:
            task_arch = self.arch_init
        if left_fea.shape != right_fea.shape or left_fea.dim() != 4:
            raise ValueError("MatchingNet: left/right features must both be [B, C, h, w]")
        cost = self.matching(None, task_arch, None, features=(left_fea, right_fea))
        return self.disp(cost)
```

### rag_amd/ops.py

```python
from __future__ import annotations

import ctypes
import os
from typing import List, Optional, Sequence

import torch

from ._lib import K1RSpec, TailSpec, check, load_library

F32, BF16, F32X3 = 0, 1, 2
_DT = {torch.float32: F32, torch.bfloat16: BF16}

_CONV_PRECISIONS = ("f16x3", "fp32")
_PRECISION_ALIASES = {"bf16x3": "f16x3", "split": "f16x3"}
_conv_precision = "fp32" if os.environ.get("RAGMI_X3", "1").strip() == "0" else "f16x3"


def set_conv_precision(precision: str) -> str:
    global _conv_precision
    precision = _PRECISION_ALIASES.get(precision, precision)
    if precision not in _CONV_PRECISIONS:
        raise ValueError(f"conv precision must be one of {_CONV_PRECISIONS}, got {precision!r}")
    old, _conv_precision = _conv_precision, precision
    return old


def get_conv_precision() -> str:
    return _conv_precision


class conv_precision:

    def __init__(self, precision: str):
        self.precision = precision

    def __enter__(self):
        self.old = set_conv_precision(self.precision)
        return self

    def __exit__(self, *exc):
        set_conv_precision(self.old)
        return False


def _conv_dt(dt: int) -> int:
    return F32X3 if (dt == F32 and _conv_precision == "f16x3") else dt


def _stream() -> int:
    return torch.cuda.current_stream().cuda_stream


def _need_gpu(*ts: torch.Tensor) -> None:
    for t in ts:
        if t is None:
            continue
        if not t.is_cuda:
            raise RuntimeError("rag_amd ops run on the MI355X only (got a CPU tensor); there is no CPU fallback")
        if t.dtype != torch.float32:
            raise RuntimeError(f"rag_amd ops: dtype {t.dtype} not built for this argument (fp32 only)")


def _act(*ts: torch.Tensor) -> int:
    dt = None
    for t in ts:
        if t is None:
            continue
        if not t.is_cuda:
            raise RuntimeError("rag_amd ops run on the MI355X only (got a CPU tensor); there is no CPU fallback")
        if t.dtype not in _DT:
            raise RuntimeError(f"rag_amd ops: activation dtype {t.dtype} not built (float32 or bfloat16)")
        if dt is not None and t.dtype != dt:
            raise RuntimeError("rag_amd ops: activation tensors of one call must share a dtype")
        dt = t.dtype
    return _DT[dt]


def _act_with_tails(x, out, res, tails) -> int:
    dt = _act(x, out, res, *[t.out for t in (tails or []) if not (t.down and x.dtype == torch.bfloat16 and t.out.dtype == torch.float32)])
    for t in (tails or []):
        if not t.out.is_cuda:
            raise RuntimeError("rag_amd ops run on the MI355X only (got a CPU tensor); there is no CPU fallback")
    return dt


def _planes(t: torch.Tensor) -> int:
    inner = 1
    for i in range(t.dim() - 1, 0, -1):
        if t.shape[i] != 1 and t.stride(i) != inner:
            raise RuntimeError(f"rag_amd ops: planes must be dense N-C-D-H-W, got strides {t.stride()} for {tuple(t.shape)}")
        inner *= t.shape[i]
    return int(t.stride(0))


def _i32_array(vals: Optional[Sequence[int]]):
    if vals is None:
        return None
    return (ctypes.c_int32 * len(vals))(*[int(v) for v in vals])


CONV_X_G4, CONV_Y_G4, TAIL_G4 = 2, 4, 4
TAIL_ROWS = 16
_STEM_TAIL_ROWS = [os.environ.get("RAGMI_STEM_TAIL_ROWS", "1") != "0"]


def set_stem_tail_rows(enabled: bool) -> None:
    _STEM_TAIL_ROWS[0] = bool(enabled)


def stem_tail_rows_enabled() -> bool:
    return _STEM_TAIL_ROWS[0]


TAIL_F32, OUT_F32 = 8, 0x100
_BF16_DEEP_F32 = [os.environ.get("RAGMI_BF16_DEEP_F32", "1") != "0"]


def set_bf16_deep_fp32(enabled: bool) -> None:
    _BF16_DEEP_F32[0] = bool(enabled)


def bf16_deep_fp32_enabled() -> bool:
    return _BF16_DEEP_F32[0]


_BF16_HEAD_F32 = [os.environ.get("RAGMI_BF16_HEAD_F32", "1") != "0"]


def set_bf16_head_fp32(enabled: bool) -> None:
    _BF16_HEAD_F32[0] = bool(enabled)


def bf16_head_fp32_enabled() -> bool:
    return _BF16_HEAD_F32[0]


_BF16_DEEP_RATIO = [int(os.environ.get("RAGMI_BF16_DEEP_RATIO", "8"))]


def bf16_deep_fp32_ratio() -> int:
    return _BF16_DEEP_RATIO[0]
_G4 = [os.environ.get("RAGMI_G4", "1") != "0"]


_FUSE_STEMS = [os.environ.get("RAGMI_FUSE_STEMS", "1") != "0"]


def set_stem_fusion(enabled: bool) -> None:
    _FUSE_STEMS[0] = bool(enabled)


def stem_fusion_enabled() -> bool:
    return _FUSE_STEMS[0]


STORE_QUARTER_ROWS = 2
_QUARTER_STORE = [os.environ.get("RAGMI_QUARTER_STORE", "1") != "0"]


def set_quarter_store(enabled: bool) -> None:
    _QUARTER_STORE[0] = bool(enabled)


def quarter_store_enabled() -> bool:
    return _QUARTER_STORE[0]


def quarter_store_supported(cin: int, cout: int, B: int, D: int, H: int, W: int, nset: int = 2, ntail: int = 0, ndown: int = 1,
                            dtype: torch.dtype = torch.float32) -> bool:
    return bool(load_library().ragmi_conv3d_k3_quarter_store_supported(cin, cout, B, D, H, W, nset, ntail, ndown, _conv_dt(_DT[dtype])))


def quarter_store_rows(n_in: int) -> Optional[List[bool]]:
    used = (ctypes.c_ubyte * max(int(n_in), 1))()
    if not load_library().ragmi_quarter_store_rows(int(n_in), used):
        return None
    return [bool(v) for v in used]


def set_g4(enabled: bool) -> None:
    _G4[0] = bool(enabled)


def g4_enabled() -> bool:
    return _G4[0]



def to_g4(t: torch.Tensor) -> torch.Tensor:
    B, C = t.shape[:2]
    sp = tuple(t.shape[2:])
    perm = (0, 1) + tuple(range(3, 3 + len(sp))) + (2,)
    return t.reshape((B, C // 4, 4) + sp).permute(perm).contiguous().view(t.shape)


def from_g4(t: torch.Tensor) -> torch.Tensor:
    B, C = t.shape[:2]
    sp = tuple(t.shape[2:])
    n = len(sp)
    perm = (0, 1, 2 + n) + tuple(range(2, 2 + n))
    return t.reshape((B, C // 4) + sp + (4,)).permute(perm).contiguous().view(t.shape)


def conv3d_k3_g4_caps(cin: int, cout: int, B: int, D: int, H: int, W: int, nset: int = 1, ntail: int = 0, ndown: int = 0,
                      dtype: torch.dtype = torch.float32) -> int:
    return int(load_library().ragmi_conv3d_k3_g4_caps(cin, cout, B, D, H, W, nset, ntail, ndown, _conv_dt(_DT[dtype])))


class Tail:

    def __init__(self, weight2d: torch.Tensor, scale: Optional[torch.Tensor], shift: Optional[torch.Tensor], relu: bool,
                 out: torch.Tensor, out_ch0: int, down: bool = False, g4: bool = False):
        _need_gpu(weight2d, scale, shift)
        _act(out)
        for t in (weight2d, scale, shift):
            if t is not None and not t.is_contiguous():
                raise ValueError("Tail: weight / scale / shift must be contiguous (row slices of contiguous tensors are)")
        self.weight2d, self.scale, self.shift, self.relu, self.out, self.out_ch0 = weight2d, scale, shift, relu, out, out_ch0
        self.down = bool(down)
        self.g4 = bool(g4)
        if self.g4 and (self.down or weight2d.shape[0] != 4 or out_ch0 % 4 or not out.is_contiguous()):
            raise ValueError("Tail: a G4 destination takes a full-resolution tail of 4 channels at a group-aligned channel of a contiguous tensor")

    def spec(self) -> TailSpec:
        p = lambda t: t.data_ptr() if t is not None else None
        f32 = TAIL_F32 if (self.down and self.out.dtype == torch.float32) else 0
        return TailSpec(p(self.weight2d), p(self.scale), p(self.shift), int(self.relu) | (2 if self.down else 0) | (TAIL_G4 if self.g4 else 0) | f32, self.out.data_ptr(),
                        _planes(self.out), int(self.out_ch0), int(self.weight2d.shape[0]))


def _tail_array(tails: Optional[Sequence["Tail"]]):
    if not tails:
        return 0, None
    if sum(1 for t in tails if not t.down) > 2 or sum(1 for t in tails if t.down) > 2:
        raise ValueError("at most two full-resolution and two down-sampling tails per conv launch")
    arr = (TailSpec * len(tails))(*[t.spec() for t in tails])
    return len(tails), arr


def costvol(left_fea: torch.Tensor, right_fea: torch.Tensor, maxdisp: int, out: Optional[torch.Tensor] = None) -> torch.Tensor:
    dt = _act(left_fea, right_fea, out)
    if left_fea.shape != right_fea.shape or left_fea.dim() != 4:
        raise ValueError("costvol: left/right features must both be [B, C, h, w]")
    left_fea, right_fea = left_fea.contiguous(), right_fea.contiguous()
    B, C, h, w = left_fea.shape
    d = int(maxdisp / 3)
    if out is None:
        out = torch.empty((B, 2 * C, d, h, w), device=left_fea.device, dtype=left_fea.dtype)
    check(load_library().ragmi_costvol_fwd(left_fea.data_ptr(), right_fea.data_ptr(), out.data_ptr(),
                                           B, C, d, h, w, dt, _stream()), "costvol")
    return out


def costvol_stem_prepare(weight: torch.Tensor) -> torch.Tensor:
    _need_gpu(weight)
    Cout, C2 = weight.shape[:2]
    if tuple(weight.shape[2:]) != (3, 3, 3) or C2 % 2:
        raise ValueError("costvol_stem_prepare: weight must be [Cout, 2C, 3, 3, 3]")
    lib = load_library()
    out = torch.empty((lib.ragmi_costvol_stem_weights_elems(C2 // 2, Cout),), device=weight.device, dtype=torch.float32)
    check(lib.ragmi_costvol_stem_prepare(weight.detach().contiguous().data_ptr(), out.data_ptr(), C2 // 2, Cout, _stream()),
          "costvol_stem_prepare")
    return out


def costvol_stem(left_fea: torch.Tensor, right_fea: torch.Tensor, maxdisp: int, variants: torch.Tensor, cout: int,
                 scale: Optional[torch.Tensor], shift: Optional[torch.Tensor], relu: bool, out: Optional[torch.Tensor] = None,
                 tails: Optional[Sequence[Tail]] = None, out_g4: bool = False) -> torch.Tensor:
    _need_gpu(variants, scale, shift)
    dt = _act(left_fea, right_fea, out, *[t.out for t in (tails or [])])
    if left_fea.shape != right_fea.shape or left_fea.dim() != 4:
        raise ValueError("costvol_stem: left/right features must both be [B, C, h, w]")
    left_fea, right_fea = left_fea.contiguous(), right_fea.contiguous()
    B, C, h, w = left_fea.shape
    d = int(maxdisp / 3)
    if out is None:
        out = torch.empty((B, cout, d, h, w), device=left_fea.device, dtype=left_fea.dtype)
    if tuple(out.shape[2:]) != (d, h, w) or out.shape[1] < cout or out.shape[0] != B:
        raise ValueError("costvol_stem: out must be [B, >=Cout, maxdisp/3, h, w]")
    lib = load_library()
    ws = torch.empty((lib.ragmi_costvol_stem_workspace_elems(B, C, cout, d, h, w),), device=left_fea.device, dtype=torch.float32)
    ntail, tarr = _tail_array(tails)
    p = lambda t: t.data_ptr() if t is not None else None
    if out_g4 and (not out.is_contiguous() or out.shape[1] != cout):
        raise ValueError("costvol_stem: a G4 output is a contiguous [B, Cout, ...] buffer")
    check(lib.ragmi_costvol_stem_fwd(left_fea.data_ptr(), right_fea.data_ptr(), variants.data_ptr(), p(scale), p(shift), int(relu) | (CONV_Y_G4 if out_g4 else 0),
                                     out.data_ptr(), _planes(out), ws.data_ptr(), B, C, cout, d, h, w, ntail, tarr, _conv_dt(dt), _stream()),
          "costvol_stem")
    return out


def costvol_stem_conv3d_supported(C: int, cmid: int, cout: int, B: int, d: int, h: int, w: int, ntail: int = 0,
                                  dtype: torch.dtype = torch.float32) -> bool:
    return bool(load_library().ragmi_costvol_stem_conv3d_supported(C, cmid, cout, B, d, h, w, ntail, _conv_dt(_DT[dtype])))


def costvol_stem_conv3d(left_fea: torch.Tensor, right_fea: torch.Tensor, maxdisp: int, variants: torch.Tensor, cmid: int,
                        scale0: Optional[torch.Tensor], shift0: Optional[torch.Tensor], relu0: bool, tails0: Optional[Sequence[Tail]],
                        packed: torch.Tensor, cout: int, scale: Optional[torch.Tensor], shift: Optional[torch.Tensor], relu: bool,
                        out: Optional[torch.Tensor], out_group_ch: Optional[Sequence[int]] = None,
                        tails: Optional[Sequence[Tail]] = None, store_main: bool = True, tail0_rows: bool = False) -> Optional[torch.Tensor]:
    _need_gpu(variants, scale0, shift0, packed, scale, shift)
    dt = _act(left_fea, right_fea, out, *[t.out for t in (tails0 or [])], *[t.out for t in (tails or [])])
    if left_fea.shape != right_fea.shape or left_fea.dim() != 4:
        raise ValueError("costvol_stem_conv3d: left/right features must both be [B, C, h, w]")
    if out is None and store_main:
        raise ValueError("costvol_stem_conv3d: store_main needs an output buffer")
    left_fea, right_fea = left_fea.contiguous(), right_fea.contiguous()
    B, C, h, w = left_fea.shape
    d = int(maxdisp / 3)
    lib = load_library()
    ws = torch.empty((lib.ragmi_costvol_stem_workspace_elems(B, C, cmid, d, h, w),), device=left_fea.device, dtype=torch.float32)
    n0, t0 = _tail_array(tails0)
    n1, t1 = _tail_array(tails)
    if tail0_rows:
        if n0 != 1 or cout != 12:
            raise ValueError("costvol_stem_conv3d: tail0_rows takes exactly one tail behind a 12-channel stem3d1")
        t0[0].relu |= TAIL_ROWS
    p = lambda t: t.data_ptr() if t is not None else None
    check(lib.ragmi_costvol_stem_conv3d_fwd(left_fea.data_ptr(), right_fea.data_ptr(), variants.data_ptr(), p(scale0), p(shift0), int(relu0),
                                            ws.data_ptr(), n0, t0, packed.data_ptr(), p(scale), p(shift), int(relu),
                                            p(out), _planes(out) if out is not None else 0, _i32_array(out_group_ch), int(store_main), n1, t1,
                                            B, C, cmid, cout, d, h, w, _conv_dt(dt), _stream()), "costvol_stem_conv3d")
    return out


def stem_tail_rows_weight(weight: torch.Tensor, tail_weight2d: torch.Tensor) -> torch.Tensor:
    if weight.dim() != 5 or weight.shape[0] != 12 or tuple(tail_weight2d.shape) != (4, weight.shape[1]):
        raise ValueError("stem_tail_rows_weight: a [12, Cin, 3, 3, 3] weight and a [4, Cin] tail")
    rows = torch.zeros((4,) + tuple(weight.shape[1:]), device=weight.device, dtype=weight.dtype)
    rows[:, :, 1, 1, 1] = tail_weight2d
    return torch.cat([weight, rows], dim=0).contiguous()


def conv3d_k3_pack(weight: torch.Tensor, transpose: bool = False, for_current_precision: bool = False) -> torch.Tensor:
    _need_gpu(weight)
    planar = weight.dim() == 4
    if tuple(weight.shape[2:]) != ((3, 3) if planar else (3, 3, 3)):
        raise ValueError("conv3d_k3_pack: weight must be [Cout, Cin, 3, 3, 3] (or [Cout, Cin, 3, 3])")
    Cout, Cin = (weight.shape[1], weight.shape[0]) if transpose else (weight.shape[0], weight.shape[1])
    lib = load_library()
    n = lib.ragmi_conv3d_k3_packed_elems(Cout, Cin)
    packed = torch.empty((n,), device=weight.device, dtype=torch.float32)
    w = weight.detach().contiguous()
    if for_current_precision:
        check(lib.ragmi_conv3d_k3_pack_for(w.data_ptr(), packed.data_ptr(), Cout, Cin, int(transpose), int(planar), _conv_dt(F32), _stream()),
              "conv3d_k3_pack_for")
    else:
        check(lib.ragmi_conv3d_k3_pack_ex(w.data_ptr(), packed.data_ptr(), Cout, Cin, int(transpose), int(planar), F32, _stream()),
              "conv3d_k3_pack")
    return packed


def conv3d_k3_plan(cout: int, B: int, D: int, H: int, W: int, nset: int = 1):
    log_tx, rows = ctypes.c_int32(), ctypes.c_int32()
    groups = (ctypes.c_int32 * 16)()
    n = load_library().ragmi_conv3d_k3_plan(cout, B, D, H, W, nset, ctypes.byref(log_tx), ctypes.byref(rows), groups, 16)
    if n < 0:
        check(n, "conv3d_k3_plan")
    return log_tx.value, rows.value, [groups[i] for i in range(n)]


def packed_groups(cout: int) -> int:
    return (cout + 3) // 4


def conv3d_k3(x: torch.Tensor, packed: torch.Tensor, cout: int, scale: Optional[torch.Tensor], shift: Optional[torch.Tensor],
              relu: bool, out: torch.Tensor, out_group_ch: Optional[Sequence[int]] = None,
              res: Optional[torch.Tensor] = None, res_group_ch: Optional[Sequence[int]] = None,
              tails: Optional[Sequence[Tail]] = None, store_main: bool = True, x_g4: bool = False) -> torch.Tensor:
    if x_g4 and not x.is_contiguous():
        raise ValueError("conv3d_k3: a G4 input is a contiguous buffer")
    _need_gpu(packed, scale, shift)
    dt = _act_with_tails(x, out, res, tails)
    B, Cin, D, H, W = x.shape
    xb = _planes(x)
    yb = _planes(out)
    rb = _planes(res) if res is not None else 0
    ng = packed_groups(cout)
    if out_group_ch is not None and len(out_group_ch) != ng:
        raise ValueError("conv3d_k3: out_group_ch needs one entry per group of 4 output channels")
    if res is not None and res_group_ch is None:
        res_group_ch = out_group_ch
    if tuple(out.shape[2:]) != (D, H, W) or out.shape[0] != B:
        raise ValueError("conv3d_k3: out must be [B, C, D, H, W] of the input's spatial size")
    max_ch = max(out_group_ch) + 4 if out_group_ch is not None else cout
    if max_ch > out.shape[1] + (3 if cout % 4 else 0):
        raise ValueError("conv3d_k3: destination channels exceed the output buffer")
    ntail, tarr = _tail_array(tails)
    check(load_library().ragmi_conv3d_k3_fwd_ex(
        x.data_ptr(), xb, packed.data_ptr(),
        scale.data_ptr() if scale is not None else None, shift.data_ptr() if shift is not None else None, int(relu) | (CONV_X_G4 if x_g4 else 0),
        out.data_ptr(), yb, _i32_array(out_group_ch),
        res.data_ptr() if res is not None else None, rb, _i32_array(res_group_ch),
        B, Cin, cout, D, H, W, int(store_main), ntail, tarr, _conv_dt(dt), _stream()), "conv3d_k3")
    return out


def conv3d_k3_small(x: torch.Tensor, weight: torch.Tensor, scale, shift, relu: bool, out: torch.Tensor, out_ch0: int = 0,
                    res: Optional[torch.Tensor] = None, res_ch0: int = 0) -> torch.Tensor:
    _need_gpu(weight, scale, shift)
    dt = _act(x, res)
    ydt = _act(out)
    if ydt != dt and not (dt == BF16 and ydt == F32):
        raise RuntimeError("conv3d_k3_small: out must have x's dtype (or be float32 when x is bfloat16)")
    B, Cin, D, H, W = x.shape
    cout = weight.shape[0]
    w = weight.detach().contiguous()
    if out_ch0 + cout > out.shape[1] or tuple(out.shape[2:]) != (D, H, W):
        raise ValueError("conv3d_k3_small: output buffer too small / wrong spatial size")
    ptr = lambda t: t.data_ptr() if t is not None else None
    check(load_library().ragmi_conv3d_k3_small_fwd_ex(
        x.data_ptr(), _planes(x), w.data_ptr(), ptr(scale), ptr(shift), int(relu), out.data_ptr(), _planes(out), out_ch0,
        ptr(res), _planes(res) if res is not None else 0, res_ch0, B, Cin, cout, D, H, W, dt, ydt, _stream()), "conv3d_k3_small")
    return out


def conv3d_k3_dual(x: torch.Tensor, cin_a: int, packed_a: torch.Tensor, scale_a, shift_a,
                   packed_b: torch.Tensor, scale_b, shift_b, cout: int, relu: bool, out: torch.Tensor,
                   out_group_ch: Optional[Sequence[int]] = None, res: Optional[torch.Tensor] = None,
                   res_group_ch: Optional[Sequence[int]] = None, tails: Optional[Sequence[Tail]] = None,
                   store_main: bool = True, x_g4: bool = False, quarter: bool = False) -> torch.Tensor:
    if quarter and not store_main:
        raise ValueError("conv3d_k3_dual: quarter=True qualifies a main store")
    if x_g4 and not x.is_contiguous():
        raise ValueError("conv3d_k3_dual: a G4 input is a contiguous buffer")
    _need_gpu(packed_a, packed_b, scale_a, shift_a, scale_b, shift_b)
    dt = _act_with_tails(x, out, res, tails)
    B, Cx, D, H, W = x.shape
    ng = packed_groups(cout)
    if out_group_ch is not None and len(out_group_ch) != ng:
        raise ValueError("conv3d_k3_dual: out_group_ch needs one entry per group of 4 output channels")
    if res is not None and res_group_ch is None:
        res_group_ch = out_group_ch
    if tuple(out.shape[2:]) != (D, H, W) or out.shape[0] != B or not 0 < cin_a < Cx:
        raise ValueError("conv3d_k3_dual: bad shapes")
    ptr = lambda t: t.data_ptr() if t is not None else None
    ntail, tarr = _tail_array(tails)
    check(load_library().ragmi_conv3d_k3_dual_fwd_ex(
        x.data_ptr(), _planes(x), cin_a, packed_a.data_ptr(), ptr(scale_a), ptr(shift_a),
        Cx - cin_a, packed_b.data_ptr(), ptr(scale_b), ptr(shift_b), int(relu) | (CONV_X_G4 if x_g4 else 0),
        out.data_ptr(), _planes(out), _i32_array(out_group_ch),
        ptr(res), _planes(res) if res is not None else 0, _i32_array(res_group_ch),
        B, cout, D, H, W, int(store_main) | (STORE_QUARTER_ROWS if quarter else 0), ntail, tarr, _conv_dt(dt), _stream()), "conv3d_k3_dual")
    return out


def conv3d_k1(x: torch.Tensor, weight2d: torch.Tensor, scale: Optional[torch.Tensor], shift: Optional[torch.Tensor],
              relu: bool, out: torch.Tensor, out_ch0: int = 0, transposed: bool = False) -> torch.Tensor:
    _need_gpu(weight2d, scale, shift)
    dt = _act(x, out)
    B, Cin = x.shape[:2]
    Cout = weight2d.shape[1 if transposed else 0]
    if not weight2d.is_contiguous() or weight2d.shape[0 if transposed else 1] != Cin:
        raise ValueError("conv3d_k1: weight must be contiguous [Cout, Cin] (or [Cin, Cout] with transposed=True)")
    dhw = 1
    for s in x.shape[2:]:
        dhw *= s
    if out_ch0 + Cout > out.shape[1] or tuple(out.shape[2:]) != tuple(x.shape[2:]):
        raise ValueError("conv3d_k1: output buffer too small / wrong spatial size")
    check(load_library().ragmi_conv3d_k1_fwd_ex(
        x.data_ptr(), _planes(x), weight2d.data_ptr(), int(transposed),
        scale.data_ptr() if scale is not None else None, shift.data_ptr() if shift is not None else None, int(relu),
        out.data_ptr(), _planes(out), out_ch0, B, Cin, Cout, dhw, dt, _stream()), "conv3d_k1")
    return out


_CHAIN_K1 = [os.environ.get("RAGMI_CHAIN_K1", "1") != "0"]


def set_chain_k1(enabled: bool) -> None:
    _CHAIN_K1[0] = bool(enabled)


def chain_k1_enabled() -> bool:
    return _CHAIN_K1[0]


def conv3d_k1_chain_supported(cin: int, cmid: int, cout: int) -> bool:
    return bool(load_library().ragmi_conv3d_k1_chain_supported(int(cin), int(cmid), int(cout)))


def conv3d_k1_chain(x: torch.Tensor, w1: torch.Tensor, scale1, shift1, relu1: bool, w2: torch.Tensor, scale2, shift2, relu2: bool,
                    out: torch.Tensor, out_ch0: int = 0) -> torch.Tensor:
    _need_gpu(w1, scale1, shift1, w2, scale2, shift2)
    dt = _act(x, out)
    B, Cin = x.shape[:2]
    Cmid, Cout = w1.shape[0], w2.shape[0]
    if not (w1.is_contiguous() and w2.is_contiguous()) or w1.shape[1] != Cin or w2.shape[1] != Cmid:
        raise ValueError("conv3d_k1_chain: weights must be contiguous [Cmid, Cin] and [Cout, Cmid]")
    dhw = 1
    for sdim in x.shape[2:]:
        dhw *= sdim
    if out_ch0 + Cout > out.shape[1] or tuple(out.shape[2:]) != tuple(x.shape[2:]):
        raise ValueError("conv3d_k1_chain: output buffer too small / wrong spatial size")
    p = lambda t: t.data_ptr() if t is not None else None
    check(load_library().ragmi_conv3d_k1_chain_fwd(x.data_ptr(), _planes(x), w1.data_ptr(), p(scale1), p(shift1), int(relu1), Cmid,
                                                   w2.data_ptr(), p(scale2), p(shift2), int(relu2), out.data_ptr(), _planes(out), out_ch0,
                                                   B, Cin, Cout, dhw, dt, _stream()), "conv3d_k1_chain")
    return out


def conv3d_k1_resample(x: torch.Tensor, size: Sequence[int], align_corners: bool, weight2d: torch.Tensor,
                       scale: Optional[torch.Tensor], shift: Optional[torch.Tensor], relu: bool, out: torch.Tensor,
                       out_ch0: int = 0) -> torch.Tensor:
    _need_gpu(weight2d, scale, shift)
    if x.dtype == torch.bfloat16 and out.dtype == torch.float32:
        dt = _act(x) | OUT_F32
        _act(out)
    else:
        dt = _act(x, out)
    B, Cin, Di, Hi, Wi = x.shape
    Do, Ho, Wo = [int(v) for v in size]
    Cout = weight2d.shape[0]
    if out_ch0 + Cout > out.shape[1] or tuple(out.shape[2:]) != (Do, Ho, Wo):
        raise ValueError("conv3d_k1_resample: output buffer too small / wrong spatial size")
    check(load_library().ragmi_conv3d_k1_resample_fwd(
        x.data_ptr(), _planes(x), Di, Hi, Wi, weight2d.data_ptr(),
        scale.data_ptr() if scale is not None else None, shift.data_ptr() if shift is not None else None, int(relu),
        out.data_ptr(), _planes(out), out_ch0, B, Cin, Cout, Do, Ho, Wo, int(bool(align_corners)), dt, _stream()),
        "conv3d_k1_resample")
    return out


def conv3d_k1_resample_pair(specs, size: Sequence[int], out: torch.Tensor) -> torch.Tensor:
    arr = []
    dt = _act(out, *[s[0] for s in specs])
    for (x, w2d, scale, shift, relu, ch0) in specs:
        _need_gpu(w2d, scale, shift)
        p = lambda t: t.data_ptr() if t is not None else None
        arr.append(K1RSpec(x.data_ptr(), _planes(x), x.shape[2], x.shape[3], x.shape[4], w2d.data_ptr(), p(scale), p(shift),
                           int(relu), int(ch0), x.shape[1], w2d.shape[0]))
        if ch0 + w2d.shape[0] > out.shape[1]:
            raise ValueError("conv3d_k1_resample_pair: output buffer too small")
    Do, Ho, Wo = [int(v) for v in size]
    if tuple(out.shape[2:]) != (Do, Ho, Wo):
        raise ValueError("conv3d_k1_resample_pair: wrong output spatial size")
    check(load_library().ragmi_conv3d_k1_resample_pair_fwd(ctypes.byref(arr[0]), ctypes.byref(arr[1]), out.data_ptr(), _planes(out),
                                                           out.shape[0], Do, Ho, Wo, 1, dt, _stream()), "conv3d_k1_resample_pair")
    return out


def conv3d_k1_resample_multi(specs, size: Sequence[int]) -> None:
    if not 1 <= len(specs) <= 3:
        raise ValueError("conv3d_k1_resample_multi: 1..3 specs")
    dt = _act(*[s[0] for s in specs], *[s[5] for s in specs])
    Do, Ho, Wo = [int(v) for v in size]
    arr, ys, bs = [], [], []
    p = lambda t: t.data_ptr() if t is not None else None
    for (x, w2d, scale, shift, relu, out, ch0) in specs:
        _need_gpu(w2d, scale, shift)
        if tuple(out.shape[2:]) != (Do, Ho, Wo) or ch0 + w2d.shape[0] > out.shape[1] or out.shape[0] != x.shape[0]:
            raise ValueError("conv3d_k1_resample_multi: output buffer too small / wrong size")
        arr.append(K1RSpec(x.data_ptr(), _planes(x), x.shape[2], x.shape[3], x.shape[4], w2d.data_ptr(), p(scale), p(shift),
                           int(relu), int(ch0), x.shape[1], w2d.shape[0]))
        ys.append(out.data_ptr())
        bs.append(_planes(out))
    n = len(arr)
    from ._lib import c_k1r_p
    parr = (c_k1r_p * n)(*[ctypes.pointer(a) for a in arr])
    check(load_library().ragmi_conv3d_k1_resample_multi_fwd(parr, (ctypes.c_void_p * n)(*ys), (ctypes.c_int64 * n)(*bs), n, specs[0][0].shape[0],
                                                            Do, Ho, Wo, 1, dt, _stream()), "conv3d_k1_resample_multi")


def cell2d_supported(C: int, cin0: int, cin1: int, cout: int, H: int, W: int, dtype=torch.float32) -> bool:
    if dtype != torch.float32:
        return False
    return bool(load_library().ragmi_cell2d_supported(int(C), int(cin0), int(cin1), int(cout), int(H), int(W), _conv_dt(_DT[dtype])))


def cell2d(s0: torch.Tensor, pre0, s1: torch.Tensor, pre1, C: int, packed_a: torch.Tensor, scale_a, shift_a,
           packed_b: torch.Tensor, scale_b, shift_b, cout: int, relu: bool, out: torch.Tensor,
           out_group_ch: Optional[Sequence[int]] = None) -> torch.Tensor:
    from ._lib import Cell2dIn
    _need_gpu(packed_a, packed_b, scale_a, shift_a, scale_b, shift_b)
    dt = _act(s0, s1, out)
    H, W = int(out.shape[-2]), int(out.shape[-1])
    B = out.shape[0]
    p = lambda t: t.data_ptr() if t is not None else None
    ins = []
    for x, (w2d, sc, sh, rl) in ((s0, pre0), (s1, pre1)):
        _need_gpu(w2d, sc, sh)
        if x.shape[0] != B or w2d.shape != (C, x.shape[1]) or not w2d.is_contiguous():
            raise ValueError("cell2d: input / 1x1 weight shapes do not match")
        ins.append(Cell2dIn(x.data_ptr(), _planes(x), x.shape[1], x.shape[-2], x.shape[-1], w2d.data_ptr(), p(sc), p(sh), int(bool(rl))))
    groups = list(out_group_ch) if out_group_ch is not None else [4 * g for g in range(cout // 4)]
    if len(groups) != cout // 4 or cout % 4 or any(g < 0 or g + 4 > out.shape[1] for g in groups):
        raise ValueError("cell2d: bad destination channel groups")
    garr = (ctypes.c_int32 * len(groups))(*groups)
    check(load_library().ragmi_cell2d_fwd(ctypes.byref(ins[0]), ctypes.byref(ins[1]), int(C), packed_a.data_ptr(), p(scale_a), p(shift_a),
                                          packed_b.data_ptr(), p(scale_b), p(shift_b), int(bool(relu)), out.data_ptr(), _planes(out), garr,
                                          B, int(cout), H, W, _conv_dt(dt), _stream()), "cell2d")
    return out


def conv2d_k3_strided(x: torch.Tensor, weight: torch.Tensor, scale, shift, relu: bool, stride: int) -> torch.Tensor:
    _need_gpu(weight, scale, shift)
    dt = _act(x)
    x = x.contiguous()
    B, Cin, H, W = x.shape
    Cout = weight.shape[0]
    Ho, Wo = (H - 1) // stride + 1, (W - 1) // stride + 1
    out = torch.empty((B, Cout, Ho, Wo), device=x.device, dtype=x.dtype)
    w = weight.detach().contiguous()
    p = lambda t: t.data_ptr() if t is not None else None
    check(load_library().ragmi_conv2d_k3_strided_fwd(x.data_ptr(), w.data_ptr(), p(scale), p(shift), int(relu), out.data_ptr(),
                                                     B, Cin, Cout, H, W, int(stride), dt, _stream()), "conv2d_k3_strided")
    return out


def down2_tail_supported(D: int, H: int, W: int) -> bool:
    return bool(load_library().ragmi_down2_tail_supported(int(D), int(H), int(W)))


def upconv3d_c1_supported(cin: int, di: int, hi: int, wi: int) -> bool:
    return bool(load_library().ragmi_upconv3d_c1_supported(int(cin), int(di), int(hi), int(wi)))


def upconv3d_c1(x: torch.Tensor, weight: torch.Tensor, scale: Optional[torch.Tensor], shift: Optional[torch.Tensor], relu: bool,
                out: Optional[torch.Tensor] = None, out_ch0: int = 0, out_dtype: Optional[torch.dtype] = None) -> torch.Tensor:
    _need_gpu(weight, scale, shift)
    dt = _act(x)
    B, Cin, Di, Hi, Wi = x.shape
    if tuple(weight.shape) != (1, Cin, 3, 3, 3):
        raise ValueError("upconv3d_c1: weight must be [1, Cin, 3, 3, 3]")
    if out is None:
        out = torch.empty((B, 1, 2 * Di, 2 * Hi, 2 * Wi), device=x.device, dtype=out_dtype or x.dtype)
    ydt = _act(out)
    if tuple(out.shape[2:]) != (2 * Di, 2 * Hi, 2 * Wi) or out.shape[0] != B or out_ch0 >= out.shape[1]:
        raise ValueError("upconv3d_c1: out must be [B, >= out_ch0 + 1, 2Di, 2Hi, 2Wi]")
    ptr = lambda t: t.data_ptr() if t is not None else None
    check(load_library().ragmi_upconv3d_c1_fwd(x.data_ptr(), _planes(x), weight.detach().contiguous().data_ptr(), ptr(scale), ptr(shift),
                                               int(relu), out.data_ptr(), _planes(out), int(out_ch0), B, Cin, Di, Hi, Wi, dt, ydt, _stream()),
          "upconv3d_c1")
    return out


def trilinear3d(x: torch.Tensor, size: Sequence[int], align_corners: bool) -> torch.Tensor:
    dt = _act(x)
    x = x.contiguous()
    B, C, Di, Hi, Wi = x.shape
    Do, Ho, Wo = [int(s) for s in size]
    out = torch.empty((B, C, Do, Ho, Wo), device=x.device, dtype=x.dtype)
    check(load_library().ragmi_trilinear3d_fwd(x.data_ptr(), out.data_ptr(), B, C, Di, Hi, Wi, Do, Ho, Wo,
                                               int(bool(align_corners)), dt, _stream()), "trilinear3d")
    return out


def trilinear3d_act(x: torch.Tensor, size: Sequence[int], align_corners: bool, relu: bool, out: torch.Tensor,
                    out_ch0: int = 0) -> torch.Tensor:
    dt = _act(x, out)
    B, C, Di, Hi, Wi = x.shape
    Do, Ho, Wo = [int(s) for s in size]
    if out_ch0 + C > out.shape[1] or tuple(out.shape[2:]) != (Do, Ho, Wo):
        raise ValueError("trilinear3d_act: output buffer too small / wrong spatial size")
    check(load_library().ragmi_trilinear3d_act_fwd(x.data_ptr(), _planes(x), out.data_ptr(), _planes(out), out_ch0, int(relu), B, C,
                                                   Di, Hi, Wi, Do, Ho, Wo, int(bool(align_corners)), dt, _stream()), "trilinear3d_act")
    return out


def add(a: torch.Tensor, a_ch0: int, b: torch.Tensor, b_ch0: int, out: torch.Tensor, out_ch0: int, channels: int) -> torch.Tensor:
    dt = _act(a, b, out)
    dhw = 1
    for s in a.shape[2:]:
        dhw *= s
    check(load_library().ragmi_add_fwd(a.data_ptr(), _planes(a), a_ch0, b.data_ptr(), _planes(b), b_ch0,
                                       out.data_ptr(), _planes(out), out_ch0, a.shape[0], channels, dhw, dt, _stream()), "add")
    return out


def disp_softargmin(cost: torch.Tensor, maxdisp: int) -> torch.Tensor:
    dt = _act(cost)
    if cost.dim() == 5:
        if cost.shape[1] != 1:
            raise ValueError("disp_softargmin: expected a single-channel cost volume")
        cost = cost[:, 0]
    cost = cost.contiguous()
    B, d, h, w = cost.shape
    out = torch.empty((B, 3 * h, 3 * w), device=cost.device, dtype=torch.float32)
    check(load_library().ragmi_disp_softargmin_fwd(cost.data_ptr(), out.data_ptr(), B, d, h, w, int(maxdisp),
                                                   3 * h, 3 * w, dt, _stream()), "disp_softargmin")
    return out


def disparity_regression(prob: torch.Tensor, maxdisp: int) -> torch.Tensor:
    dt = _act(prob)
    assert prob.is_contiguous()
    B, D, H, W = prob.shape
    if D != maxdisp:
        raise ValueError("disparity_regression: prob.shape[1] must equal maxdisp")
    out = torch.empty((B, H, W), device=prob.device, dtype=torch.float32)
    check(load_library().ragmi_disparity_regression_fwd(prob.data_ptr(), out.data_ptr(), B, D, H, W, dt, _stream()),
          "disparity_regression")
    return out


def _vol(t: torch.Tensor) -> int:
    n = 1
    for s in t.shape[2:]:
        n *= s
    return n


def bn_train_stats(x: torch.Tensor, gamma: torch.Tensor, beta: torch.Tensor, running_mean: Optional[torch.Tensor],
                   running_var: Optional[torch.Tensor], num_batches_tracked: Optional[torch.Tensor], momentum: float, eps: float):
    _need_gpu(x, gamma, beta, running_mean, running_var)
    B, C = x.shape[:2]
    lib = load_library()
    ws = torch.empty((lib.ragmi_bn_workspace_elems(B, C, _vol(x)),), device=x.device, dtype=torch.float32)
    out = torch.empty((4, C), device=x.device, dtype=torch.float32)
    if num_batches_tracked is not None and num_batches_tracked.dtype != torch.int64:
        raise RuntimeError("bn_train_stats: num_batches_tracked must be int64")
    p = lambda t: t.data_ptr() if t is not None else None
    check(lib.ragmi_bn_train_stats_fwd(x.data_ptr(), _planes(x), B, C, _vol(x), gamma.data_ptr(), beta.data_ptr(), p(running_mean),
                                       p(running_var), p(num_batches_tracked), float(momentum), float(eps), ws.data_ptr(),
                                       out[0].data_ptr(), out[1].data_ptr(), out[2].data_ptr(), out[3].data_ptr(), _stream()),
          "bn_train_stats")
    return out


def bn_train_act(x: torch.Tensor, gamma: torch.Tensor, beta: torch.Tensor, running_mean: Optional[torch.Tensor],
                 running_var: Optional[torch.Tensor], num_batches_tracked: Optional[torch.Tensor], momentum: float, eps: float, relu: bool,
                 res: Optional[torch.Tensor] = None):
    _need_gpu(x, gamma, beta, running_mean, running_var, res)
    B, C = x.shape[:2]
    if res is not None and tuple(res.shape) != tuple(x.shape):
        raise ValueError("bn_train_act: res must have the shape of x")
    lib = load_library()
    ws = torch.empty((lib.ragmi_bn_workspace_elems(B, C, _vol(x)),), device=x.device, dtype=torch.float32)
    st = torch.empty((4, C), device=x.device, dtype=torch.float32)
    y = torch.empty(x.shape, device=x.device, dtype=torch.float32)
    if num_batches_tracked is not None and num_batches_tracked.dtype != torch.int64:
        raise RuntimeError("bn_train_act: num_batches_tracked must be int64")
    p = lambda t: t.data_ptr() if t is not None else None
    check(lib.ragmi_bn_train_act_fwd(x.data_ptr(), _planes(x), B, C, _vol(x), gamma.data_ptr(), beta.data_ptr(), p(running_mean),
                                     p(running_var), p(num_batches_tracked), float(momentum), float(eps), int(relu), ws.data_ptr(),
                                     st[0].data_ptr(), st[1].data_ptr(), st[2].data_ptr(), st[3].data_ptr(), y.data_ptr(), _planes(y), 0,
                                     p(res), _planes(res) if res is not None else 0, 0, _stream()), "bn_train_act")
    return y, st


def bn_act_bwd(dy: torch.Tensor, x: torch.Tensor, scale, shift, relu: bool, mean, invstd, training: bool,
               out: Optional[torch.Tensor] = None, dgamma_into: Optional[torch.Tensor] = None, dbeta_into: Optional[torch.Tensor] = None):
    _need_gpu(dy, x, scale, shift, mean, invstd, out, dgamma_into, dbeta_into)
    B, C = x.shape[:2]
    lib = load_library()
    ws = torch.empty((lib.ragmi_bn_workspace_elems(B, C, _vol(x)),), device=x.device, dtype=torch.float32)
    dx = out if out is not None else torch.empty(x.shape, device=x.device, dtype=torch.float32)
    direct = dgamma_into is not None and dbeta_into is not None
    gb = None if direct else torch.empty((2, C), device=x.device, dtype=torch.float32)
    dg, db = (dgamma_into, dbeta_into) if direct else (gb[0], gb[1])
    check(lib.ragmi_bn_act_bwd(dy.data_ptr(), _planes(dy), 0, x.data_ptr(), _planes(x), scale.data_ptr(), shift.data_ptr(), int(relu),
                               mean.data_ptr(), invstd.data_ptr(), int(training), B, C, _vol(x), ws.data_ptr(), dx.data_ptr(), _planes(dx),
                               dg.data_ptr(), db.data_ptr(), int(direct), _stream()), "bn_act_bwd")
    return dx, (None if direct else gb[0]), (None if direct else gb[1])


def bn_act(x: torch.Tensor, scale: torch.Tensor, shift: torch.Tensor, relu: bool, out: Optional[torch.Tensor] = None,
           out_ch0: int = 0, res: Optional[torch.Tensor] = None, res_ch0: int = 0) -> torch.Tensor:
    _need_gpu(x, scale, shift, out, res)
    B, C = x.shape[:2]
    if out is None:
        out = torch.empty_like(x)
    check(load_library().ragmi_bn_act_fwd(x.data_ptr(), _planes(x), scale.data_ptr(), shift.data_ptr(), int(relu),
                                          res.data_ptr() if res is not None else None, _planes(res) if res is not None else 0, res_ch0,
                                          out.data_ptr(), _planes(out), out_ch0, B, C, _vol(x), _stream()), "bn_act")
    return out


def bn_act_bwd_coeffs(dy: torch.Tensor, dy_ch0: int, x: torch.Tensor, scale, shift, relu: bool, mean, invstd, training: bool,
                      dgamma_into: Optional[torch.Tensor] = None, dbeta_into: Optional[torch.Tensor] = None):
    _need_gpu(dy, x, scale, shift, mean, invstd, dgamma_into, dbeta_into)
    B, C = x.shape[:2]
    lib = load_library()
    ws = torch.empty((lib.ragmi_bn_workspace_elems(B, C, _vol(x)),), device=x.device, dtype=torch.float32)
    out = torch.empty((5, C), device=x.device, dtype=torch.float32)
    direct = dgamma_into is not None or dbeta_into is not None
    if direct and (dgamma_into is None or dbeta_into is None):
        raise ValueError("bn_act_bwd_coeffs: pass both dgamma_into and dbeta_into, or neither")
    dg, db = (dgamma_into, dbeta_into) if direct else (out[3], out[4])
    check(lib.ragmi_bn_act_bwd_coeffs(dy.data_ptr(), _planes(dy), dy_ch0, x.data_ptr(), _planes(x), scale.data_ptr(), shift.data_ptr(),
                                      int(relu), mean.data_ptr(), invstd.data_ptr(), int(training), B, C, _vol(x), ws.data_ptr(),
                                      out[0].data_ptr(), out[1].data_ptr(), out[2].data_ptr(), dg.data_ptr(), db.data_ptr(), int(direct),
                                      _stream()), "bn_act_bwd_coeffs")
    return out


def bn_act_bwd_apply(dy: torch.Tensor, dy_ch0: int, x: torch.Tensor, scale, shift, relu: bool, c1, c2, c3,
                     out: Optional[torch.Tensor] = None) -> torch.Tensor:
    _need_gpu(dy, x, scale, shift, c1, c2, c3, out)
    B, C = x.shape[:2]
    dx = out if out is not None else torch.empty(x.shape, device=x.device, dtype=torch.float32)
    check(load_library().ragmi_bn_act_bwd_apply(dy.data_ptr(), _planes(dy), dy_ch0, x.data_ptr(), _planes(x), scale.data_ptr(),
                                                shift.data_ptr(), int(relu), c1.data_ptr(), c2.data_ptr(), c3.data_ptr(), dx.data_ptr(),
                                                _planes(dx), B, C, _vol(x), _stream()), "bn_act_bwd_apply")
    return dx


def conv3d_k3_wgrad(x: torch.Tensor, g: torch.Tensor, cout: int, g_ch0: int = 0, into: Optional[Sequence[torch.Tensor]] = None,
                    planar2d: bool = False):
    _need_gpu(x, g, *(into or []))
    B, Cin, D, H, W = x.shape
    lib = load_library()
    n = lib.ragmi_conv3d_k3_wgrad_workspace_elems(B, Cin, cout, D, H, W)
    if n < 0:
        check(-2, "conv3d_k3_wgrad_workspace_elems")
    ws = torch.empty((n,), device=x.device, dtype=torch.float32)
    if into is None:
        dw = torch.empty((cout, Cin, 3, 3) if planar2d else (cout, Cin, 3, 3, 3), device=x.device, dtype=torch.float32)
        dsts, acc = [dw], 0
    else:
        want = (cout // len(into), Cin, 3, 3) if planar2d else (cout // len(into), Cin, 3, 3, 3)
        if any(tuple(t.shape) != want or not t.is_contiguous() for t in into):
            raise ValueError(f"conv3d_k3_wgrad: every destination must be a contiguous {want} tensor")
        dw, dsts, acc = None, list(into), 1
    arr = (ctypes.c_void_p * len(dsts))(*[t.data_ptr() for t in dsts])
    check(lib.ragmi_conv3d_k3_wgrad(x.data_ptr(), _planes(x), g.data_ptr(), _planes(g), g_ch0, arr, len(dsts), acc, int(planar2d),
                                    ws.data_ptr(), B, Cin, cout, D, H, W, _stream()), "conv3d_k3_wgrad")
    return dw


def conv3d_k1_wgrad(x: torch.Tensor, g: torch.Tensor, cout: int, g_ch0: int = 0, into: Optional[torch.Tensor] = None) -> torch.Tensor:
    _need_gpu(x, g, into)
    B, Cin = x.shape[:2]
    if into is not None and (into.numel() != cout * Cin or not into.is_contiguous()):
        raise ValueError("conv3d_k1_wgrad: destination must be contiguous with cout*Cin elements")
    dw = into if into is not None else torch.zeros((cout, Cin), device=x.device, dtype=torch.float32)
    check(load_library().ragmi_conv3d_k1_wgrad(x.data_ptr(), _planes(x), g.data_ptr(), _planes(g), g_ch0, dw.data_ptr(), B, Cin, cout,
                                               _vol(x), _stream()), "conv3d_k1_wgrad")
    return dw


def trilinear3d_bwd(dy: torch.Tensor, in_size: Sequence[int], align_corners: bool) -> torch.Tensor:
    _need_gpu(dy)
    dy = dy.contiguous()
    B, C, Do, Ho, Wo = dy.shape
    Di, Hi, Wi = [int(v) for v in in_size]
    dx = torch.empty((B, C, Di, Hi, Wi), device=dy.device, dtype=torch.float32)
    check(load_library().ragmi_trilinear3d_bwd(dy.data_ptr(), dx.data_ptr(), B, C, Di, Hi, Wi, Do, Ho, Wo, int(bool(align_corners)),
                                               _stream()), "trilinear3d_bwd")
    return dx


def costvol_bwd(dcost: torch.Tensor):
    _need_gpu(dcost)
    dcost = dcost.contiguous()
    B, C2, d, h, w = dcost.shape
    dl = torch.empty((B, C2 // 2, h, w), device=dcost.device, dtype=torch.float32)
    dr = torch.empty_like(dl)
    check(load_library().ragmi_costvol_bwd(dcost.data_ptr(), dl.data_ptr(), dr.data_ptr(), B, C2 // 2, d, h, w, _stream()), "costvol_bwd")
    return dl, dr


def disp_softargmin_bwd(cost: torch.Tensor, dout: torch.Tensor, maxdisp: int) -> torch.Tensor:
    _need_gpu(cost, dout)
    shape = cost.shape
    c4 = (cost[:, 0] if cost.dim() == 5 else cost).contiguous()
    B, d, h, w = c4.shape
    dout = dout.contiguous()
    dc = torch.zeros_like(c4)
    check(load_library().ragmi_disp_softargmin_bwd(c4.data_ptr(), dout.data_ptr(), dc.data_ptr(), B, d, h, w, int(maxdisp), 3 * h, 3 * w,
                                                   _stream()), "disp_softargmin_bwd")
    return dc.reshape(shape)


def conv2d_k3_strided_dgrad(g: torch.Tensor, weight: torch.Tensor, in_hw: Sequence[int], stride: int) -> torch.Tensor:
    _need_gpu(g, weight)
    g, w = g.contiguous(), weight.detach().contiguous()
    B, Cout = g.shape[:2]
    Cin, (H, W) = w.shape[1], [int(v) for v in in_hw]
    if tuple(g.shape[2:]) != ((H - 1) // stride + 1, (W - 1) // stride + 1):
        raise ValueError("conv2d_k3_strided_dgrad: gradient size does not match the input size / stride")
    dx = torch.empty((B, Cin, H, W), device=g.device, dtype=torch.float32)
    check(load_library().ragmi_conv2d_k3_strided_dgrad(g.data_ptr(), w.data_ptr(), dx.data_ptr(), B, Cin, Cout, H, W, int(stride),
                                                       _stream()), "conv2d_k3_strided_dgrad")
    return dx


def conv2d_k3_strided_wgrad(x: torch.Tensor, g: torch.Tensor, stride: int, into: Optional[torch.Tensor] = None) -> torch.Tensor:
    _need_gpu(x, g, into)
    x, g = x.contiguous(), g.contiguous()
    B, Cin, H, W = x.shape
    Cout = g.shape[1]
    if into is not None and (tuple(into.shape) != (Cout, Cin, 3, 3) or not into.is_contiguous()):
        raise ValueError("conv2d_k3_strided_wgrad: destination must be a contiguous [Cout, Cin, 3, 3] tensor")
    dw = into if into is not None else torch.zeros((Cout, Cin, 3, 3), device=x.device, dtype=torch.float32)
    check(load_library().ragmi_conv2d_k3_strided_wgrad(x.data_ptr(), g.data_ptr(), dw.data_ptr(), B, Cin, Cout, H, W, int(stride),
                                                       _stream()), "conv2d_k3_strided_wgrad")
    return dw


def disparity_regression_bwd(dout: torch.Tensor, maxdisp: int) -> torch.Tensor:
    _need_gpu(dout)
    dout = dout.contiguous()
    B, H, W = dout.shape
    dp = torch.empty((B, int(maxdisp), H, W), device=dout.device, dtype=torch.float32)
    check(load_library().ragmi_disparity_regression_bwd(dout.data_ptr(), dp.data_ptr(), B, int(maxdisp), H, W, _stream()),
          "disparity_regression_bwd")
    return dp



def conv3d_k3_uses_x3(cin: int, cout: int, B: int, D: int, H: int, W: int, nset: int = 1, has_res: bool = False, ntail: int = 0,
                      dtype: torch.dtype = torch.float32) -> bool:
    return bool(load_library().ragmi_conv3d_k3_uses_x3(cin, cout, B, D, H, W, nset, int(has_res), ntail, _conv_dt(_DT[dtype])))


def sgd_clip_step(param: torch.Tensor, grad: torch.Tensor, buf: torch.Tensor, lr: float, momentum: float, weight_decay: float,
                  max_norm: float, first_step: bool, workspace: Optional[torch.Tensor] = None,
                  norm_out: Optional[torch.Tensor] = None) -> torch.Tensor:
    _need_gpu(param, grad, buf, workspace, norm_out)
    for t in (param, grad, buf):
        if t.dim() != 1 or t.dtype != torch.float32 or not t.is_contiguous() or t.numel() != param.numel():
            raise RuntimeError("sgd_clip_step: param / grad / momentum buffers must be flat contiguous fp32 of equal length")
    lib = load_library()
    if workspace is None:
        workspace = torch.empty((lib.ragmi_sgd_workspace_bytes() // 4,), device=param.device, dtype=torch.float32)
    if norm_out is None:
        norm_out = torch.empty((1,), device=param.device, dtype=torch.float32)
    check(lib.ragmi_sgd_clip_step(param.data_ptr(), grad.data_ptr(), buf.data_ptr(), param.numel(), float(lr), float(momentum),
                                  float(weight_decay), float(max_norm), int(first_step), workspace.data_ptr(), norm_out.data_ptr(),
                                  _stream()), "sgd_clip_step")
    return norm_out


def depth_head_supported(cin: int, hi: int, wi: int, h: int, w: int, scale: int = 3, dtype=torch.float32) -> bool:
    return bool(load_library().ragmi_depth_head_supported(cin, hi, wi, h, w, scale, _DT.get(dtype, -1)))


def depth_head(y: torch.Tensor, w3: torch.Tensor, w1: torch.Tensor, b1: torch.Tensor, size: Sequence[int], scale: int = 3,
               max_depth: float = 80.0) -> torch.Tensor:
    for t in (y, w3, w1, b1):
        if not t.is_cuda:
            raise RuntimeError("rag_amd ops run on the MI355X only (got a CPU tensor); there is no CPU fallback")
    if y.dim() != 4 or w3.numel() != 9 * y.shape[1] or w1.numel() != 9 or b1.numel() != 1:
        raise ValueError("depth_head: y must be [B, Cin, Hi, Wi], w3 [1, Cin, 3, 3], w1 [1, 1, 3, 3], b1 [1]")
    dtypes = {y.dtype, w3.dtype, w1.dtype, b1.dtype}
    dt = _DT.get(y.dtype, -1) if len(dtypes) == 1 else -1
    y, w3, w1, b1 = y.contiguous(), w3.contiguous(), w1.contiguous(), b1.contiguous()
    B, C, Hi, Wi = y.shape
    H, W = (int(v) for v in size)
    out = torch.empty((B, scale * H, scale * W), device=y.device, dtype=torch.float32)
    check(load_library().ragmi_depth_head_fwd(y.data_ptr(), w3.data_ptr(), w1.data_ptr(), b1.data_ptr(), out.data_ptr(), B, C, Hi, Wi,
                                              H, W, int(scale), float(max_depth), dt, _stream()), "depth_head")
    return out


def depth_metrics(est: torch.Tensor, gt: torch.Tensor, variance_focus: float = 0.85) -> torch.Tensor:
    for t in (est, gt):
        if not t.is_cuda:
            raise RuntimeError("rag_amd ops run on the MI355X only (got a CPU tensor); there is no CPU fallback")
    if est.shape != gt.shape or est.numel() == 0:
        raise ValueError("depth_metrics: est and gt must have the same non-empty shape")
    dt = _DT.get(est.dtype, -1) if est.dtype == gt.dtype else -1
    est, gt = est.contiguous(), gt.contiguous()
    lib = load_library()
    n = est.numel()
    ws = torch.empty((max(2, lib.ragmi_depth_metrics_workspace_elems(n)),), device=est.device, dtype=torch.float32)
    out = torch.empty((10,), device=est.device, dtype=torch.float32)
    check(lib.ragmi_depth_metrics_fwd(est.data_ptr(), gt.data_ptr(), n, float(variance_focus), ws.data_ptr(), out.data_ptr(), dt,
                                      _stream()), "depth_metrics")
    return out


def depth_head_bwd(y: torch.Tensor, w3: torch.Tensor, w1: torch.Tensor, b1: torch.Tensor, d_out: torch.Tensor, size: Sequence[int],
                   scale: int = 3, max_depth: float = 80.0, dw3_into: Optional[torch.Tensor] = None,
                   dw1_into: Optional[torch.Tensor] = None, db1_into: Optional[torch.Tensor] = None):
    _need_gpu(y, w3, w1, b1, d_out)
    if y.dim() != 4 or w3.numel() != 9 * y.shape[1] or w1.numel() != 9 or b1.numel() != 1:
        raise ValueError("depth_head_bwd: y must be [B, Cin, Hi, Wi], w3 [1, Cin, 3, 3], w1 [1, 1, 3, 3], b1 [1]")
    B, C, Hi, Wi = y.shape
    H, W = (int(v) for v in size)
    if tuple(d_out.shape) != (B, scale * H, scale * W):
        raise ValueError(f"depth_head_bwd: d_out must be [{B}, {scale * H}, {scale * W}], got {tuple(d_out.shape)}")
    dtypes = {y.dtype, w3.dtype, w1.dtype, b1.dtype, d_out.dtype}
    dt = _DT.get(y.dtype, -1) if len(dtypes) == 1 else -1
    y, w3, w1, b1, d_out = y.contiguous(), w3.contiguous(), w1.contiguous(), b1.contiguous(), d_out.contiguous()
    outs, acc = [], 0
    for bit, (w, into) in enumerate(((w3, dw3_into), (w1, dw1_into), (b1, db1_into))):
        if into is not None:
            if into.numel() != w.numel() or into.dtype != torch.float32 or not into.is_contiguous() or into.device != w.device:
                raise ValueError("depth_head_bwd: an *_into target must be a contiguous fp32 tensor of the weight's size")
            outs.append(into)
            acc |= 1 << bit
        else:
            outs.append(torch.empty(w.shape, device=w.device, dtype=torch.float32))
    dy = torch.empty((B, C, Hi, Wi), device=y.device, dtype=torch.float32)
    lib = load_library()
    ws = torch.empty((max(2, lib.ragmi_depth_head_bwd_workspace_elems(B, C, H, W)),), device=y.device, dtype=torch.float32)
    check(lib.ragmi_depth_head_bwd(y.data_ptr(), w3.data_ptr(), w1.data_ptr(), b1.data_ptr(), d_out.data_ptr(), dy.data_ptr(),
                                   outs[0].data_ptr(), outs[1].data_ptr(), outs[2].data_ptr(), acc, ws.data_ptr(), B, C, Hi, Wi, H, W,
                                   int(scale), float(max_depth), dt, _stream()), "depth_head_bwd")
    return dy, outs[0], outs[1], outs[2]


def silog_loss(est: torch.Tensor, gt: torch.Tensor, variance_focus: float = 0.85):
    for t in (est, gt):
        if not t.is_cuda:
            raise RuntimeError("rag_amd ops run on the MI355X only (got a CPU tensor); there is no CPU fallback")
    if est.shape != gt.shape or est.numel() == 0:
        raise ValueError("silog_loss: est and gt must have the same non-empty shape")
    dt = _DT.get(est.dtype, -1) if est.dtype == gt.dtype else -1
    est, gt = est.contiguous(), gt.contiguous()
    lib = load_library()
    n = est.numel()
    ws = torch.empty((max(2, lib.ragmi_silog_loss_workspace_elems(n)),), device=est.device, dtype=torch.float32)
    out = torch.empty((1,), device=est.device, dtype=torch.float32)
    saved = torch.empty((3,), device=est.device, dtype=torch.float64)
    check(lib.ragmi_silog_loss_fwd(est.data_ptr(), gt.data_ptr(), n, float(variance_focus), ws.data_ptr(), out.data_ptr(),
                                   saved.data_ptr(), dt, _stream()), "silog_loss")
    return out, saved


def silog_loss_bwd(est: torch.Tensor, gt: torch.Tensor, saved: torch.Tensor, gout: torch.Tensor, variance_focus: float = 0.85):
    _need_gpu(gout)
    dt = _DT.get(est.dtype, -1) if est.dtype == gt.dtype else -1
    est, gt, gout = est.contiguous(), gt.contiguous(), gout.reshape(-1)[:1].contiguous()
    grad = torch.empty(est.shape, device=est.device, dtype=torch.float32)
    check(load_library().ragmi_silog_loss_bwd(est.data_ptr(), gt.data_ptr(), est.numel(), float(variance_focus), saved.data_ptr(),
                                              gout.data_ptr(), grad.data_ptr(), dt, _stream()), "silog_loss_bwd")
    return grad
```

Before: 1140 disparity maps/s.

## Add FP16 hi/lo matrix-core path for C1 upsample-conv head, opt-in via env

Adds a new kernel for the fused trilinear-upsample plus 3x3x3 single-output-channel head conv. It splits fp32 operands into FP16 hi/lo halves and runs them on the matrix cores, using pre-packed weight fragments that are cached per module. The existing FMA kernel is also split into a select-free interior body and a boundary body with per-tile selection, and odd input widths now go through a float2 store path. The matrix-core path is gated behind RAGMI_HEAD_X3, which defaults off, so by default only the interior/boundary specialization of the old kernel runs.

```diff
diff --git a/include/rag_amd.h b/include/rag_amd.h
--- a/include/rag_amd.h
+++ b/include/rag_amd.h
@@ -148,9 +148,17 @@
                           int Di, int Hi, int Wi, int Do, int Ho, int Wo,
                           int align_corners, int dtype, void* stream);
 
+#define RAGMI_UPCONV_SELECT_BODY 1
+#define RAGMI_UPCONV_NO_X3 2
 int ragmi_upconv3d_c1_supported(int Cin, int Di, int Hi, int Wi);
+int ragmi_upconv3d_c1_uses_x3(int Cin, int Di, int Hi, int Wi, int dtype);
+int64_t ragmi_upconv3d_c1_pack_bytes(int Cin);
+int ragmi_upconv3d_c1_pack(const void* weight, int Cin, void* packed, void* stream);
 int ragmi_upconv3d_c1_fwd(const void* x, int64_t x_bstride, const void* weight, const void* scale, const void* shift, int relu, void* y,
                           int64_t y_bstride, int y_ch0, int B, int Cin, int Di, int Hi, int Wi, int dtype, int y_dtype, void* stream);
+int ragmi_upconv3d_c1_fwd_ex(const void* x, int64_t x_bstride, const void* weight, const void* packed, const void* scale, const void* shift,
+                             int relu, void* y, int64_t y_bstride, int y_ch0, int B, int Cin, int Di, int Hi, int Wi, int dtype, int y_dtype,
+                             int flags, void* stream);
 
 int ragmi_trilinear3d_act_fwd(const void* x, int64_t x_bstride, void* y, int64_t y_bstride, int y_ch0, int relu, int B, int C,
                               int Di, int Hi, int Wi, int Do, int Ho, int Wo, int align_corners, int dtype, void* stream);
diff --git a/rag_amd/_lib.py b/rag_amd/_lib.py
--- a/rag_amd/_lib.py
+++ b/rag_amd/_lib.py
@@ -90,6 +90,11 @@
     "ragmi_upconv3d_c1_supported": (c_int, [c_int, c_int, c_int, c_int]),
     "ragmi_upconv3d_c1_fwd": (c_int, [c_void_p, c_int64, c_void_p, c_void_p, c_void_p, c_int, c_void_p, c_int64, c_int, c_int, c_int, c_int,
                                       c_int, c_int, c_int, c_int, c_void_p]),
+    "ragmi_upconv3d_c1_uses_x3": (c_int, [c_int, c_int, c_int, c_int, c_int]),
+    "ragmi_upconv3d_c1_pack_bytes": (c_int64, [c_int]),
+    "ragmi_upconv3d_c1_pack": (c_int, [c_void_p, c_int, c_void_p, c_void_p]),
+    "ragmi_upconv3d_c1_fwd_ex": (c_int, [c_void_p, c_int64, c_void_p, c_void_p, c_void_p, c_void_p, c_int, c_void_p, c_int64, c_int, c_int,
+                                         c_int, c_int, c_int, c_int, c_int, c_int, c_int, c_void_p]),
     "ragmi_trilinear3d_act_fwd": (c_int, [c_void_p, c_int64, c_void_p, c_int64, c_int, c_int, c_int, c_int, c_int, c_int, c_int, c_int,
                                           c_int, c_int, c_int, c_int, c_void_p]),
     "ragmi_trilinear3d_fwd": (c_int, [c_void_p, c_void_p, c_int, c_int, c_int, c_int, c_int, c_int, c_int, c_int,
diff --git a/rag_amd/csrc/conv3d_c1.hip b/rag_amd/csrc/conv3d_c1.hip
--- a/rag_amd/csrc/conv3d_c1.hip
+++ b/rag_amd/csrc/conv3d_c1.hip
@@ -1,4 +1,5 @@
 #include "conv3d_k3.h"
+#include "upconv3d_c1.h"
 
 namespace ragmi {
 
@@ -164,18 +165,8 @@
 constexpr int CU_BLK = CU_PZ * CU_PY * CU_RS;
 constexpr int CU_NPF = (CU_PZ * CU_PY * CU_PX + CU_THREADS - 1) / CU_THREADS;
 
-struct CUArgs {
-  const void* x;
-  const float* w;
-  const float* scale;
-  const float* shift;
-  void* y;
-  int64_t x_bstride, y_bstride;
-  int y_ch0, relu;
-  int B, Cin, Di, Hi, Wi;
-  float sd, sh, sw;
-  int tiles_x, tiles_y, nseg, nwork;
-};
+__device__ __forceinline__ void st2(float* p, float v0, float v1) { *reinterpret_cast<float2*>(p) = make_float2(v0, v1); }
+__device__ __forceinline__ void st2(bf16_t* p, float v0, float v1) { *reinterpret_cast<unsigned*>(p) = (unsigned)to_bf16(v0) | ((unsigned)to_bf16(v1) << 16); }
 
 template <class T, class TO>
 __global__ __launch_bounds__(CU_THREADS, 2) void upconv3d_c1_kernel(CUArgs a) {
@@ -216,123 +207,134 @@
       if (e < CU_PZ * CU_PY * CU_PX) buf[(e / CU_PX) * CU_RS + e % CU_PX] = pf[p];
     }
   };
-  float wy0[4], wy1[4], wx0[6], wx1[6];
-  bool ylow[4], xlow[6];
-#pragma unroll
-  for (int r = 0; r < 4; ++r) {
-    const int gy = y0 + 2 * ty - 1 + r;
-    const LinIdx l = lin_index(min(max(gy, 0), H - 1), a.Hi, H, a.sh, 1);
-    const int expect = py0 + ty + (r >= 2 ? 1 : 0);
-    ylow[r] = l.i0 < expect;
-    const bool in = (unsigned)gy < (unsigned)H;
-    wy0[r] = in ? l.w0 : 0.f; wy1[r] = in ? l.w1 : 0.f;
-  }
-#pragma unroll
-  for (int i = 0; i < 6; ++i) {
-    const int gx = x0 + 4 * tx - 1 + i;
-    const LinIdx l = lin_index(min(max(gx, 0), W - 1), a.Wi, W, a.sw, 1);
-    const int expect = px0 + 2 * tx + (i >= 4 ? 2 : (i >= 2 ? 1 : 0));
-    xlow[i] = l.i0 < expect;
-    const bool in = (unsigned)gx < (unsigned)W;
-    wx0[i] = in ? l.w0 : 0.f; wx1[i] = in ? l.w1 : 0.f;
-  }
-  float acc[ZSEG][2][4];
-#pragma unroll
-  for (int k = 0; k < ZSEG; ++k)
-#pragma unroll
-    for (int r = 0; r < 2; ++r)
-#pragma unroll
-      for (int i = 0; i < 4; ++i) acc[k][r][i] = 0.f;
-  prefetch(0);
-  commit(blk[0]);
-  __syncthreads();
-  const int wbase = ty * CU_RS + 2 * tx;
-  for (int c = 0; c < a.Cin; ++c) {
-    const float* const cur = blk[c & 1];
-    prefetch(c + 1);
-    float w[28];
-#pragma unroll
-    for (int i = 0; i < 28; i += 4) {
-      const float4 q = *reinterpret_cast<const float4*>(wl + c * 28 + i);
-      w[i] = q.x; w[i + 1] = q.y; w[i + 2] = q.z; w[i + 3] = q.w;
-    }
-    static_for<NP>([&](auto zi_) {
-      constexpr int zi = decltype(zi_)::value;
-      const int z = zs - 1 + zi;
-      if (z >= 0 && z <= min(ze, D - 1)) {
-        const LinIdx lz = lin_index(z, a.Di, D, a.sd, 1);
-        const int pa = lz.i0 - pz0, pb = lz.i1 - pz0;
-        float in[4][6];
-        {
-          float rz[3][4];
-#pragma unroll
-          for (int rr = 0; rr < 3; ++rr) {
-            const float* const qa = cur + pa * (CU_PY * CU_RS) + wbase + rr * CU_RS;
-            const float* const qb = cur + pb * (CU_PY * CU_RS) + wbase + rr * CU_RS;
-            const float2 a0 = *reinterpret_cast<const float2*>(qa), a1 = *reinterpret_cast<const float2*>(qa + 2);
-            const float2 b0 = *reinterpret_cast<const float2*>(qb), b1 = *reinterpret_cast<const float2*>(qb + 2);
-            rz[rr][0] = lerp2(lz.w0, a0.x, lz.w1, b0.x); rz[rr][1] = lerp2(lz.w0, a0.y, lz.w1, b0.y);
-            rz[rr][2] = lerp2(lz.w0, a1.x, lz.w1, b1.x); rz[rr][3] = lerp2(lz.w0, a1.y, lz.w1, b1.y);
+  const bool sel = a.sel_always || y0 + CU_TY >= H - 1 || x0 + CU_TX >= W - 1;
+  auto body = [&](auto sel_) {
+    constexpr bool SEL = decltype(sel_)::value;
+    float wy0[4], wy1[4], wx0[6], wx1[6];
+    bool ylow[4], xlow[6];
+  #pragma unroll
+    for (int r = 0; r < 4; ++r) {
+      const int gy = y0 + 2 * ty - 1 + r;
+      const LinIdx l = lin_index(min(max(gy, 0), H - 1), a.Hi, H, a.sh, 1);
+      const int expect = py0 + ty + (r >= 2 ? 1 : 0);
+      ylow[r] = l.i0 < expect;
+      const bool in = (unsigned)gy < (unsigned)H;
+      wy0[r] = in ? l.w0 : 0.f; wy1[r] = in ? l.w1 : 0.f;
+    }
+  #pragma unroll
+    for (int i = 0; i < 6; ++i) {
+      const int gx = x0 + 4 * tx - 1 + i;
+      const LinIdx l = lin_index(min(max(gx, 0), W - 1), a.Wi, W, a.sw, 1);
+      const int expect = px0 + 2 * tx + (i >= 4 ? 2 : (i >= 2 ? 1 : 0));
+      xlow[i] = l.i0 < expect;
+      const bool in = (unsigned)gx < (unsigned)W;
+      wx0[i] = in ? l.w0 : 0.f; wx1[i] = in ? l.w1 : 0.f;
+    }
+    float acc[ZSEG][2][4];
+  #pragma unroll
+    for (int k = 0; k < ZSEG; ++k)
+  #pragma unroll
+      for (int r = 0; r < 2; ++r)
+  #pragma unroll
+        for (int i = 0; i < 4; ++i) acc[k][r][i] = 0.f;
+    prefetch(0);
+    commit(blk[0]);
+    __syncthreads();
+    const int wbase = ty * CU_RS + 2 * tx;
+    for (int c = 0; c < a.Cin; ++c) {
+      const float* const cur = blk[c & 1];
+      prefetch(c + 1);
+      float w[28];
+  #pragma unroll
+      for (int i = 0; i < 28; i += 4) {
+        const float4 q = *reinterpret_cast<const float4*>(wl + c * 28 + i);
+        w[i] = q.x; w[i + 1] = q.y; w[i + 2] = q.z; w[i + 3] = q.w;
+      }
+      static_for<NP>([&](auto zi_) {
+        constexpr int zi = decltype(zi_)::value;
+        const int z = zs - 1 + zi;
+        if (z >= 0 && z <= min(ze, D - 1)) {
+          const LinIdx lz = lin_index(z, a.Di, D, a.sd, 1);
+          const int pa = lz.i0 - pz0, pb = lz.i1 - pz0;
+          float in[4][6];
+          {
+            float rz[3][4];
+  #pragma unroll
+            for (int rr = 0; rr < 3; ++rr) {
+              const float* const qa = cur + pa * (CU_PY * CU_RS) + wbase + rr * CU_RS;
+              const float* const qb = cur + pb * (CU_PY * CU_RS) + wbase + rr * CU_RS;
+              const float2 a0 = *reinterpret_cast<const float2*>(qa), a1 = *reinterpret_cast<const float2*>(qa + 2);
+              const float2 b0 = *reinterpret_cast<const float2*>(qb), b1 = *reinterpret_cast<const float2*>(qb + 2);
+              rz[rr][0] = lerp2(lz.w0, a0.x, lz.w1, b0.x); rz[rr][1] = lerp2(lz.w0, a0.y, lz.w1, b0.y);
+              rz[rr][2] = lerp2(lz.w0, a1.x, lz.w1, b1.x); rz[rr][3] = lerp2(lz.w0, a1.y, lz.w1, b1.y);
+            }
+            float yv[4][4];
+  #pragma unroll
+            for (int r = 0; r < 4; ++r)
+  #pragma unroll
+              for (int q = 0; q < 4; ++q) {
+                const float lo = r >= 2 ? ((SEL && ylow[r]) ? rz[0][q] : rz[1][q]) : rz[0][q];
+                const float hi = r >= 2 ? ((SEL && ylow[r]) ? rz[1][q] : rz[2][q]) : rz[1][q];
+                yv[r][q] = lerp2(wy0[r], lo, wy1[r], hi);
+              }
+  #pragma unroll
+            for (int r = 0; r < 4; ++r)
+  #pragma unroll
+              for (int i = 0; i < 6; ++i) {
+                const int e = i >= 4 ? 2 : (i >= 2 ? 1 : 0);
+                const float lo = e > 0 ? ((SEL && xlow[i]) ? yv[r][e - 1] : yv[r][e]) : yv[r][e];
+                const float hi = e > 0 ? ((SEL && xlow[i]) ? yv[r][e] : yv[r][e + 1]) : yv[r][e + 1];
+                in[r][i] = lerp2(wx0[i], lo, wx1[i], hi);
+              }
           }
-          float yv[4][4];
-#pragma unroll
-          for (int r = 0; r < 4; ++r)
-#pragma unroll
-            for (int q = 0; q < 4; ++q) {
-              const float lo = r >= 2 ? (ylow[r] ? rz[0][q] : rz[1][q]) : rz[0][q];
-              const float hi = r >= 2 ? (ylow[r] ? rz[1][q] : rz[2][q]) : rz[1][q];
-              yv[r][q] = lerp2(wy0[r], lo, wy1[r], hi);
+          static_for<3>([&](auto dz_) {
+            constexpr int dz = decltype(dz_)::value, k = zi - dz;
+            if constexpr (k >= 0 && k < ZSEG) {
+              if (zs + k < ze) {
+  #pragma unroll
+                for (int r = 0; r < 2; ++r)
+  #pragma unroll
+                  for (int dy = 0; dy < 3; ++dy)
+  #pragma unroll
+                    for (int dx = 0; dx < 3; ++dx)
+  #pragma unroll
+                      for (int i = 0; i < 4; ++i) acc[k][r][i] = fmaf(w[dz * 9 + dy * 3 + dx], in[r + dy][i + dx], acc[k][r][i]);
+              }
             }
-#pragma unroll
-          for (int r = 0; r < 4; ++r)
-#pragma unroll
-            for (int i = 0; i < 6; ++i) {
-              const int e = i >= 4 ? 2 : (i >= 2 ? 1 : 0);
-              const float lo = e > 0 ? (xlow[i] ? yv[r][e - 1] : yv[r][e]) : yv[r][e];
-              const float hi = e > 0 ? (xlow[i] ? yv[r][e] : yv[r][e + 1]) : yv[r][e + 1];
-              in[r][i] = lerp2(wx0[i], lo, wx1[i], hi);
-            }
+          });
         }
-        static_for<3>([&](auto dz_) {
-          constexpr int dz = decltype(dz_)::value, k = zi - dz;
-          if constexpr (k >= 0 && k < ZSEG) {
-            if (zs + k < ze) {
-#pragma unroll
-              for (int r = 0; r < 2; ++r)
-#pragma unroll
-                for (int dy = 0; dy < 3; ++dy)
-#pragma unroll
-                  for (int dx = 0; dx < 3; ++dx)
-#pragma unroll
-                    for (int i = 0; i < 4; ++i) acc[k][r][i] = fmaf(w[dz * 9 + dy * 3 + dx], in[r + dy][i + dx], acc[k][r][i]);
-            }
-          }
-        });
+      });
+      commit(blk[(c + 1) & 1]);
+      __syncthreads();
+    }
+    const float sc = a.scale ? a.scale[0] : 1.f, sh = a.shift ? a.shift[0] : 0.f;
+    const int64_t HW = (int64_t)H * W;
+    TO* const yb = static_cast<TO*>(a.y) + (int64_t)b * a.y_bstride + (int64_t)a.y_ch0 * HW * D;
+    const int gx = x0 + 4 * tx;
+  #pragma unroll
+    for (int k = 0; k < ZSEG; ++k) {
+      if (zs + k >= ze) continue;
+  #pragma unroll
+      for (int r = 0; r < 2; ++r) {
+        const int gy = y0 + 2 * ty + r;
+        if (gy >= H || gx >= W) continue;
+        float v[4];
+  #pragma unroll
+        for (int i = 0; i < 4; ++i) {
+          const float u = fmaf(acc[k][r][i], sc, sh);
+          v[i] = a.relu ? fmaxf(u, 0.f) : u;
+        }
+        TO* const dst = yb + (int64_t)(zs + k) * HW + (int64_t)gy * W + gx;
+        if ((W & 3) == 0) {
+          st4(dst, v);
+        } else {
+          st2(dst, v[0], v[1]);
+          if (gx + 2 < W) st2(dst + 2, v[2], v[3]);
+        }
       }
-    });
-    commit(blk[(c + 1) & 1]);
-    __syncthreads();
-  }
-  const float sc = a.scale ? a.scale[0] : 1.f, sh = a.shift ? a.shift[0] : 0.f;
-  const int64_t HW = (int64_t)H * W;
-  TO* const yb = static_cast<TO*>(a.y) + (int64_t)b * a.y_bstride + (int64_t)a.y_ch0 * HW * D;
-  const int gx = x0 + 4 * tx;
-#pragma unroll
-  for (int k = 0; k < ZSEG; ++k) {
-    if (zs + k >= ze) continue;
-#pragma unroll
-    for (int r = 0; r < 2; ++r) {
-      const int gy = y0 + 2 * ty + r;
-      if (gy >= H || gx >= W) continue;
-      float v[4];
-#pragma unroll
-      for (int i = 0; i < 4; ++i) {
-        const float u = fmaf(acc[k][r][i], sc, sh);
-        v[i] = a.relu ? fmaxf(u, 0.f) : u;
-      }
-      st4(yb + (int64_t)(zs + k) * HW + (int64_t)gy * W + gx, v);
-    }
-  }
+    }
+  };
+  if (sel) body(std::true_type{}); else body(std::false_type{});
 }
 
 template <class T, class TO>
@@ -350,27 +352,42 @@
 
 extern "C" int ragmi_upconv3d_c1_supported(int Cin, int Di, int Hi, int Wi) {
   using namespace ragmi;
-  return (Cin >= 1 && Cin <= C1_MAX_CIN && Di >= 2 && Hi >= 2 && Wi >= 2 && (2 * Wi) % 4 == 0 && (int64_t)Cin * Di * Hi * Wi < (1ll << 31)) ? 1 : 0;
+  return (Cin >= 1 && Cin <= C1_MAX_CIN && Di >= 2 && Hi >= 2 && Wi >= 2 && (int64_t)Cin * Di * Hi * Wi < (1ll << 31)) ? 1 : 0;
 }
 
 extern "C" int ragmi_upconv3d_c1_fwd(const void* x, int64_t x_bstride, const void* weight, const void* scale, const void* shift, int relu,
                                      void* y, int64_t y_bstride, int y_ch0, int B, int Cin, int Di, int Hi, int Wi, int dtype, int y_dtype,
                                      void* stream) {
+  return ragmi_upconv3d_c1_fwd_ex(x, x_bstride, weight, nullptr, scale, shift, relu, y, y_bstride, y_ch0, B, Cin, Di, Hi, Wi, dtype, y_dtype, 0, stream);
+}
+
+extern "C" int ragmi_upconv3d_c1_fwd_ex(const void* x, int64_t x_bstride, const void* weight, const void* packed, const void* scale,
+                                        const void* shift, int relu, void* y, int64_t y_bstride, int y_ch0, int B, int Cin, int Di, int Hi,
+                                        int Wi, int dtype, int y_dtype, int flags, void* stream) {
   using namespace ragmi;
+  RAGMI_REQUIRE((flags & ~(RAGMI_UPCONV_SELECT_BODY | RAGMI_UPCONV_NO_X3)) == 0, RAGMI_EINVAL, "upconv3d_c1: unknown flag bits %d", flags);
+  const bool x3 = dtype == RAGMI_F32X3;
+  if (x3) {
+    RAGMI_REQUIRE(y_dtype == RAGMI_F32X3 || y_dtype == RAGMI_F32, RAGMI_EUNSUPPORTED, "upconv3d_c1: dtype %d -> %d not built", dtype, y_dtype);
+    dtype = y_dtype = RAGMI_F32;
+  }
   RAGMI_REQUIRE(x && weight && y, RAGMI_EINVAL, "upconv3d_c1: null pointer");
   RAGMI_REQUIRE((scale == nullptr) == (shift == nullptr), RAGMI_EINVAL, "upconv3d_c1: scale/shift must both be given or both NULL");
   RAGMI_REQUIRE(B > 0 && B <= 65535 && y_ch0 >= 0, RAGMI_EINVAL, "upconv3d_c1: bad size");
   RAGMI_REQUIRE(dtype_ok(dtype) && (y_dtype == dtype || (dtype == RAGMI_BF16 && y_dtype == RAGMI_F32)), RAGMI_EUNSUPPORTED,
                 "upconv3d_c1: dtype %d -> %d not built", dtype, y_dtype);
   RAGMI_REQUIRE(ragmi_upconv3d_c1_supported(Cin, Di, Hi, Wi), RAGMI_EUNSUPPORTED,
-                "upconv3d_c1: needs 1..%d input channels, every input axis >= 2 and an even input width", C1_MAX_CIN);
+                "upconv3d_c1: needs 1..%d input channels and every input axis >= 2", C1_MAX_CIN);
   RAGMI_REQUIRE(y_bstride % 4 == 0 && aligned4(y, y_dtype), RAGMI_EUNSUPPORTED, "upconv3d_c1: output rows must be 16-byte aligned");
   CUArgs a{};
   a.x = x; a.w = (const float*)weight; a.scale = (const float*)scale; a.shift = (const float*)shift; a.y = y;
   a.x_bstride = x_bstride; a.y_bstride = y_bstride; a.y_ch0 = y_ch0; a.relu = relu ? 1 : 0;
   a.B = B; a.Cin = Cin; a.Di = Di; a.Hi = Hi; a.Wi = Wi;
   a.sd = lin_scale(Di, 2 * Di, 1); a.sh = lin_scale(Hi, 2 * Hi, 1); a.sw = lin_scale(Wi, 2 * Wi, 1);
+  a.sel_always = (flags & RAGMI_UPCONV_SELECT_BODY) ? 1 : 0;
   hipStream_t st = static_cast<hipStream_t>(stream);
+  if (x3 && packed && !(flags & RAGMI_UPCONV_NO_X3) && ragmi_upconv3d_c1_uses_x3(Cin, Di, Hi, Wi, RAGMI_F32X3))
+    return upconv_x3_launch(a, packed, st);
   if (dtype == RAGMI_BF16) return y_dtype == RAGMI_F32 ? upconv_launch_typed<bf16_t, float>(a, st) : upconv_launch_typed<bf16_t, bf16_t>(a, st);
   return upconv_launch_typed<float, float>(a, st);
 }
diff --git a/rag_amd/csrc/upconv3d_c1.h b/rag_amd/csrc/upconv3d_c1.h
--- /dev/null
+++ b/rag_amd/csrc/upconv3d_c1.h
@@ -0,0 +1,22 @@
+#pragma once
+#include "conv3d_k3.h"
+
+namespace ragmi {
+
+struct CUArgs {
+  const void* x;
+  const float* w;
+  const float* scale;
+  const float* shift;
+  void* y;
+  int64_t x_bstride, y_bstride;
+  int y_ch0, relu;
+  int B, Cin, Di, Hi, Wi;
+  float sd, sh, sw;
+  int tiles_x, tiles_y, nseg, nwork;
+  int sel_always;
+};
+
+int upconv_x3_launch(CUArgs a, const void* packed, hipStream_t st);
+
+}
diff --git a/rag_amd/csrc/upconv3d_c1_x3.hip b/rag_amd/csrc/upconv3d_c1_x3.hip
--- /dev/null
+++ b/rag_amd/csrc/upconv3d_c1_x3.hip
@@ -0,0 +1,307 @@
+#include "conv3d_x3_common.h"
+#include "upconv3d_c1.h"
+
+namespace ragmi {
+
+constexpr int UX_TY = 32, UX_NBLK = 4, UX_BW = 14, UX_TXW = UX_NBLK * UX_BW, UX_THREADS = 256;
+#ifndef UX_ZSEG_OVERRIDE
+constexpr int UX_ZSEG = 4;
+#else
+constexpr int UX_ZSEG = UX_ZSEG_OVERRIDE;
+#endif
+constexpr int UX_ROWS = UX_TY + 2;
+constexpr int UX_PZ = UX_ZSEG / 2 + 2, UX_PY = UX_TY / 2 + 2, UX_PX = UX_TXW / 2 + 2, UX_RS = UX_PX + 1;
+constexpr int UX_PP = UX_PY * UX_RS, UX_CB = UX_PZ * UX_PP;
+constexpr int UX_NPF = (UX_PZ * UX_PY * UX_PX + UX_THREADS - 1) / UX_THREADS;
+constexpr int UX_PAIRS = UX_ROWS / 2;
+constexpr int UX_UROW = (2 * UX_NBLK + 1) * 16, UX_UH = (UX_ROWS * UX_UROW + 255) / 256 * 256, UX_UC = 2 * UX_UH;
+constexpr int UX_LDS_BYTES = 2 * 2 * UX_CB * 4 + 2 * 2 * UX_UC + UX_PAIRS * 24 + 16;
+static_assert(UX_LDS_BYTES <= 80 * 1024, "two workgroups per CU");
+static_assert(UX_THREADS == 256 && UX_TY == 32 && UX_NBLK == 4 && UX_ZSEG % 2 == 0 && UX_ZSEG >= 2, "wave -> tile map, operand buffer parity");
+
+template <int ZSEG>
+__global__ __launch_bounds__(UX_THREADS, 2) void upconv3d_c1_x3_kernel(CUArgs a, const uint4* __restrict__ wf, const float* __restrict__ wmul) {
+  constexpr int NP = ZSEG + 2;
+  __shared__ __attribute__((aligned(16))) float blk[2][2 * UX_CB];
+  __shared__ __attribute__((aligned(16))) unsigned char ubuf[2][2 * UX_UC];
+  __shared__ __attribute__((aligned(16))) float4 pw[UX_PAIRS];
+  __shared__ int2 po[UX_PAIRS];
+  __shared__ float wmax[4];
+  const int tid = threadIdx.x, lane = tid & 63, wv = tid >> 6;
+  const int D = 2 * a.Di, H = 2 * a.Hi, W = 2 * a.Wi;
+  const int chunk = (a.nwork + 7) / 8, j = blockIdx.x;
+  int t = (j & 7) * chunk + (j >> 3);
+  if ((j >> 3) >= chunk || t >= a.nwork) return;
+  const int x0 = (t % a.tiles_x) * UX_TXW; t /= a.tiles_x;
+  const int y0 = (t % a.tiles_y) * UX_TY; t /= a.tiles_y;
+  const int seg = t % a.nseg, b = t / a.nseg;
+  const int zs = seg * ZSEG, ze = min(D, zs + ZSEG);
+  const int HWi = a.Hi * a.Wi;
+  const int64_t DHWi = (int64_t)HWi * a.Di;
+  const int pz0 = zs / 2 - 1, py0 = y0 / 2 - 1, px0 = x0 / 2 - 1;
+  const int ng = a.Cin / 2;
+  int soff[UX_NPF];
+#pragma unroll
+  for (int p = 0; p < UX_NPF; ++p) {
+    const int e = min(tid + p * UX_THREADS, UX_PZ * UX_PY * UX_PX - 1);
+    const int cx = e % UX_PX, cy = (e / UX_PX) % UX_PY, cz = e / (UX_PX * UX_PY);
+    soff[p] = min(max(pz0 + cz, 0), a.Di - 1) * HWi + min(max(py0 + cy, 0), a.Hi - 1) * a.Wi + min(max(px0 + cx, 0), a.Wi - 1);
+  }
+  const float* const xb = static_cast<const float*>(a.x) + (int64_t)b * a.x_bstride;
+  float pf[2][UX_NPF];
+  auto prefetch = [&](int g) {
+    const float* const pc = xb + (int64_t)(2 * min(g, ng - 1)) * DHWi;
+#pragma unroll
+    for (int c = 0; c < 2; ++c)
+#pragma unroll
+      for (int p = 0; p < UX_NPF; ++p) pf[c][p] = pc[c * DHWi + soff[p]];
+  };
+  auto commit = [&](float* buf) {
+#pragma unroll
+    for (int c = 0; c < 2; ++c)
+#pragma unroll
+      for (int p = 0; p < UX_NPF; ++p) {
+        const int e = tid + p * UX_THREADS;
+        if (e < UX_PZ * UX_PY * UX_PX) buf[c * UX_CB + (e / (UX_PX * UX_PY)) * UX_PP + ((e / UX_PX) % UX_PY) * UX_RS + e % UX_PX] = pf[c][p];
+      }
+  };
+  float amax = 0.f;
+#pragma unroll 3
+  for (int g = ng - 1; g >= 0; --g) {
+    prefetch(g);
+#pragma unroll
+    for (int c = 0; c < 2; ++c)
+#pragma unroll
+      for (int p = 0; p + 3 < UX_NPF; p += 4) amax = fmaxf(amax, x3_scalable_max4(pf[c][p], pf[c][p + 1], pf[c][p + 2], pf[c][p + 3]));
+#pragma unroll
+    for (int c = 0; c < 2; ++c)
+#pragma unroll
+      for (int p = UX_NPF / 4 * 4; p < UX_NPF; ++p) amax = fmaxf(amax, x3_scalable_max4(pf[c][p], 0.f, 0.f, 0.f));
+  }
+  amax = x3_wave_max(amax);
+  if (lane == 0) wmax[wv] = amax;
+  commit(blk[0]);
+  if (tid < UX_PAIRS) {
+    const int gya = y0 - 1 + 2 * tid, gyb = gya + 1;
+    const LinIdx la = lin_index(min(max(gya, 0), H - 1), a.Hi, H, a.sh, 1), lb = lin_index(min(max(gyb, 0), H - 1), a.Hi, H, a.sh, 1);
+    const bool ina = (unsigned)gya < (unsigned)H, inb = (unsigned)gyb < (unsigned)H;
+    const int i0 = ina ? la.i0 : lb.i0, i1 = ina ? la.i1 : lb.i1;
+    pw[tid] = make_float4(ina ? la.w0 : 0.f, ina ? la.w1 : 0.f, inb ? lb.w0 : 0.f, inb ? lb.w1 : 0.f);
+    po[tid] = make_int2(min(max(i0 - py0, 0), UX_PY - 1) * UX_RS, min(max(i1 - py0, 0), UX_PY - 1) * UX_RS);
+  }
+  const int hw = tid & 7, sblk = hw >> 1, sh_ = hw & 1, cb = 7 * sblk + 4 * sh_;
+  float wx0[8], wx1[8];
+  bool xlow[8];
+#pragma unroll
+  for (int i = 0; i < 8; ++i) {
+    const int gx = x0 + UX_BW * sblk - 1 + 8 * sh_ + i;
+    const LinIdx l = lin_index(min(max(gx, 0), W - 1), a.Wi, W, a.sw, 1);
+    const bool in = (unsigned)gx < (unsigned)W;
+    wx0[i] = in ? l.w0 : 0.f; wx1[i] = in ? l.w1 : 0.f;
+    xlow[i] = in && l.i0 < px0 + cb + (i >> 1);
+  }
+  __syncthreads();
+  amax = fmaxf(fmaxf(wmax[0], wmax[1]), fmaxf(wmax[2], wmax[3]));
+  const float amul = x3_pow2_scale(amax, X3_ACT_TARGET);
+  const int n = lane & 15, kb = lane >> 4, rg = wv & 1, bp = wv >> 1;
+  const int uboff = (kb >> 1) * UX_UC + (kb & 1) * UX_UH + (16 * rg + n) * UX_UROW + bp * 64;
+  auto plane_live = [&](int zi) { const int z = zs - 1 + zi; return z >= 0 && z <= min(ze, D - 1); };
+  const bool sel = x0 + UX_TXW >= W - 1;
+
+  auto body = [&](auto sel_) {
+    constexpr bool SEL = decltype(sel_)::value;
+    auto stage_item = [&](const float* cur, unsigned char* dstbuf, const LinIdx& lz, int pa, int pb, int cj) {
+      const int c = cj >= UX_PAIRS ? 1 : 0, jp = cj - c * UX_PAIRS;
+      const float4 wy = pw[jp];
+      const int2 o = po[jp];
+      const float* const q = cur + c * UX_CB + cb;
+      constexpr int Q0 = SEL ? -1 : 0;
+      float zr[2][6];
+#pragma unroll
+      for (int qq = Q0; qq < 5; ++qq) {
+        const int col = SEL ? max(cb + qq, 0) - cb : qq;
+        zr[0][qq + 1] = lerp2(lz.w0, q[pa + o.x + col], lz.w1, q[pb + o.x + col]);
+        zr[1][qq + 1] = lerp2(lz.w0, q[pa + o.y + col], lz.w1, q[pb + o.y + col]);
+      }
+#pragma unroll
+      for (int u = 0; u < 2; ++u) {
+        const float w0 = u ? wy.z : wy.x, w1 = u ? wy.w : wy.y;
+        float yv[6];
+#pragma unroll
+        for (int qq = Q0; qq < 5; ++qq) yv[qq + 1] = lerp2(w0, zr[0][qq + 1], w1, zr[1][qq + 1]);
+        float v[8];
+#pragma unroll
+        for (int i = 0; i < 8; ++i) {
+          const int e = (i >> 1) + 1;
+          const float lo = (SEL && xlow[i]) ? yv[e - 1] : yv[e];
+          const float hi = (SEL && xlow[i]) ? yv[e] : yv[e + 1];
+          v[i] = lerp2(wx0[i], lo, wx1[i], hi);
+        }
+        uint4 hi4, lo4;
+        hi4.x = x3_split2h(v[0], v[1], amul, lo4.x);
+        hi4.y = x3_split2h(v[2], v[3], amul, lo4.y);
+        hi4.z = x3_split2h(v[4], v[5], amul, lo4.z);
+        hi4.w = x3_split2h(v[6], v[7], amul, lo4.w);
+        uint4* const dst = reinterpret_cast<uint4*>(dstbuf + c * UX_UC + sh_ * UX_UH + (2 * jp + u) * UX_UROW + sblk * 32);
+        dst[0] = hi4;
+        dst[1] = lo4;
+      }
+    };
+    auto stage_plane = [&](const float* cur, unsigned char* dstbuf, int zi, int extra) {
+      const LinIdx lz = lin_index(zs - 1 + zi, a.Di, D, a.sd, 1);
+      const int pa = min(max(lz.i0 - pz0, 0), UX_PZ - 1) * UX_PP, pb = min(max(lz.i1 - pz0, 0), UX_PZ - 1) * UX_PP;
+      stage_item(cur, dstbuf, lz, pa, pb, tid >> 3);
+      if (wv == extra && lane < 16) stage_item(cur, dstbuf, lz, pa, pb, UX_THREADS / 8 + (lane >> 3));
+    };
+    f32x4 acc[ZSEG][2];
+#pragma unroll
+    for (int k = 0; k < ZSEG; ++k) { acc[k][0] = f32x4{0.f, 0.f, 0.f, 0.f}; acc[k][1] = f32x4{0.f, 0.f, 0.f, 0.f}; }
+    uint4 af[3][3][2];
+    auto load_af = [&](int g, int dz) {
+#pragma unroll
+      for (int dy = 0; dy < 3; ++dy)
+#pragma unroll
+        for (int hl = 0; hl < 2; ++hl) af[dz][dy][hl] = wf[(((min(g, ng - 1) * 3 + dz) * 3 + dy) * 2 + hl) * 64 + lane];
+    };
+    load_af(0, 0);
+    load_af(0, 1);
+    if (plane_live(0)) stage_plane(blk[0], ubuf[0], 0, 0);
+    __syncthreads();
+    for (int g = 0; g < ng; ++g) {
+      const float* const cur = blk[g & 1];
+      const bool more = g + 1 < ng;
+      load_af(g, 2);
+      static_for<NP>([&](auto zi_) {
+        constexpr int zi = decltype(zi_)::value;
+        if constexpr (zi == NP - 3) prefetch(g + 1);
+        if constexpr (zi + 1 < NP) {
+          if (plane_live(zi + 1)) stage_plane(cur, ubuf[(zi + 1) & 1], zi + 1, (zi + g) & 3);
+        } else {
+          if (more && plane_live(0)) stage_plane(blk[(g + 1) & 1], ubuf[0], 0, (zi + g) & 3);
+        }
+        if (plane_live(zi)) {
+          const unsigned char* const ub = ubuf[zi & 1] + uboff;
+#pragma unroll
+          for (int dy = 0; dy < 3; ++dy)
+#pragma unroll
+            for (int nt = 0; nt < 2; ++nt) {
+              const uint4* const q = reinterpret_cast<const uint4*>(ub + dy * UX_UROW + nt * 32);
+              const uint4 bh = q[0], bl = q[1];
+              static_for<3>([&](auto dz_) {
+                constexpr int dz = decltype(dz_)::value, k = zi - dz;
+                if constexpr (k >= 0 && k < ZSEG) acc[k][nt] = x3_mma<false>(af[dz][dy][1], bh, acc[k][nt]);
+              });
+              static_for<3>([&](auto dz_) {
+                constexpr int dz = decltype(dz_)::value, k = zi - dz;
+                if constexpr (k >= 0 && k < ZSEG) acc[k][nt] = x3_mma<false>(af[dz][dy][0], bl, acc[k][nt]);
+              });
+              static_for<3>([&](auto dz_) {
+                constexpr int dz = decltype(dz_)::value, k = zi - dz;
+                if constexpr (k >= 0 && k < ZSEG) acc[k][nt] = x3_mma<false>(af[dz][dy][0], bh, acc[k][nt]);
+              });
+            }
+        }
+        if constexpr (zi == NP - 2) { load_af(g + 1, 0); load_af(g + 1, 1); }
+        if constexpr (zi == NP - 2) { if (more) commit(blk[(g + 1) & 1]); }
+        __syncthreads();
+      });
+    }
+  const float es = (a.scale ? a.scale[0] : 1.f) * (wmul[0] * (1.f / amul)), sh = a.shift ? a.shift[0] : 0.f;
+  const int64_t HW = (int64_t)H * W;
+  float* const yb = static_cast<float*>(a.y) + (int64_t)b * a.y_bstride + (int64_t)a.y_ch0 * HW * D;
+  const int gy = y0 + 16 * rg + n;
+#pragma unroll
+  for (int k = 0; k < ZSEG; ++k) {
+    if (zs + k >= ze || gy >= H) continue;
+#pragma unroll
+    for (int nt = 0; nt < 2; ++nt) {
+      const int gx = x0 + UX_BW * (2 * bp + nt) + 4 * kb;
+      float* const dst = yb + (int64_t)(zs + k) * HW + (int64_t)gy * W + gx;
+#pragma unroll
+      for (int i = 0; i < 4; i += 2) {
+        if (4 * kb + i >= UX_BW || gx + i >= W) continue;
+        const float u0 = fmaf(acc[k][nt][i], es, sh), u1 = fmaf(acc[k][nt][i + 1], es, sh);
+        *reinterpret_cast<float2*>(dst + i) = make_float2(a.relu ? fmaxf(u0, 0.f) : u0, a.relu ? fmaxf(u1, 0.f) : u1);
+      }
+    }
+  }
+  };
+  if (sel) body(std::true_type{}); else body(std::false_type{});
+}
+
+__global__ void upconv3d_c1_pack_kernel(const float* __restrict__ w, uint4* __restrict__ wf, int Cin, int nsl) {
+  __shared__ unsigned wmaxbits;
+  if (threadIdx.x == 0) wmaxbits = 0u;
+  __syncthreads();
+  for (int i = threadIdx.x; i < Cin * 27; i += blockDim.x) {
+    const unsigned bits = __float_as_uint(fabsf(w[i]));
+    if (bits < 0x7f800000u) atomicMax(&wmaxbits, bits);
+  }
+  __syncthreads();
+  const float mul = x3_row_mul(wmaxbits);
+  if (threadIdx.x == 0) *reinterpret_cast<float*>(wf + (int64_t)nsl * 2 * 64) = 1.f / mul;
+  for (int idx = threadIdx.x; idx < nsl * 64; idx += blockDim.x) {
+    const int lane = idx & 63, s = idx >> 6, m = lane & 15, kb = lane >> 4;
+    const int ci = 2 * (s / 9) + (kb >> 1), dz = (s / 3) % 3, dy = s % 3;
+    unsigned short hi[8], lo[8];
+    for (int jj = 0; jj < 8; ++jj) {
+      const int dx = 8 * (kb & 1) + jj - m;
+      const float v = (m < UX_BW && dx >= 0 && dx <= 2 && ci < Cin) ? w[ci * 27 + dz * 9 + dy * 3 + dx] * mul : 0.f;
+      hi[jj] = x3_f16_bits(v);
+      lo[jj] = x3_f16_bits(v - (float)__builtin_bit_cast(_Float16, hi[jj]));
+    }
+    auto pk = [](const unsigned short* h) {
+      return make_uint4(h[0] | ((unsigned)h[1] << 16), h[2] | ((unsigned)h[3] << 16), h[4] | ((unsigned)h[5] << 16), h[6] | ((unsigned)h[7] << 16));
+    };
+    wf[(int64_t)(s * 2 + 0) * 64 + lane] = pk(hi);
+    wf[(int64_t)(s * 2 + 1) * 64 + lane] = pk(lo);
+  }
+}
+
+static int ux_slices(int Cin) { return (Cin + 1) / 2 * 9; }
+
+static bool ux_axis_regular(int n_in) {
+  const int n_out = 2 * n_in;
+  const float scale = lin_scale(n_in, n_out, 1);
+  for (int o = 1; o < n_out; ++o) {
+    const int expect = (o - 1) / 2, i0 = lin_index(o, n_in, n_out, scale, 1).i0;
+    if (i0 != expect && !(o == n_out - 1 && i0 == expect - 1)) return false;
+  }
+  return true;
+}
+
+int upconv_x3_launch(CUArgs a, const void* packed, hipStream_t st) {
+  const int D = 2 * a.Di, H = 2 * a.Hi, W = 2 * a.Wi;
+  RAGMI_REQUIRE(packed != nullptr && a.Cin % 4 == 0, RAGMI_EINVAL, "upconv3d_c1 (f16x3): needs the packed fragments and Cin %% 4 == 0");
+  RAGMI_REQUIRE((reinterpret_cast<uintptr_t>(packed) & 15) == 0, RAGMI_EUNSUPPORTED, "upconv3d_c1 (f16x3): packed fragments must be 16-byte aligned");
+  a.tiles_x = (int)ceil_div(W, UX_TXW); a.tiles_y = (int)ceil_div(H, UX_TY); a.nseg = (int)ceil_div(D, UX_ZSEG);
+  const int64_t nwork = (int64_t)a.tiles_x * a.tiles_y * a.nseg * a.B;
+  RAGMI_REQUIRE(nwork < (1ll << 28), RAGMI_EUNSUPPORTED, "upconv3d_c1 (f16x3): too many tiles");
+  a.nwork = (int)nwork;
+  const uint4* const wf = static_cast<const uint4*>(packed);
+  const float* const wmul = reinterpret_cast<const float*>(wf + (int64_t)ux_slices(a.Cin) * 2 * 64);
+  hipLaunchKernelGGL((upconv3d_c1_x3_kernel<UX_ZSEG>), dim3((unsigned)(ceil_div(nwork, 8) * 8)), dim3(UX_THREADS), 0, st, a, wf, wmul);
+  return check_launch("upconv3d_c1_x3");
+}
+
+}
+
+extern "C" int64_t ragmi_upconv3d_c1_pack_bytes(int Cin) {
+  if (Cin < 1 || Cin > 64) return 0;
+  return (int64_t)ragmi::ux_slices(Cin) * 2 * 64 * 16 + 16;
+}
+
+extern "C" int ragmi_upconv3d_c1_pack(const void* weight, int Cin, void* packed, void* stream) {
+  using namespace ragmi;
+  RAGMI_REQUIRE(weight && packed, RAGMI_EINVAL, "upconv3d_c1_pack: null pointer");
+  RAGMI_REQUIRE(Cin >= 1 && Cin <= 64, RAGMI_EUNSUPPORTED, "upconv3d_c1_pack: needs 1..64 input channels");
+  RAGMI_REQUIRE((reinterpret_cast<uintptr_t>(packed) & 15) == 0, RAGMI_EUNSUPPORTED, "upconv3d_c1_pack: packed must be 16-byte aligned");
+  hipLaunchKernelGGL(upconv3d_c1_pack_kernel, dim3(1), dim3(256), 0, static_cast<hipStream_t>(stream), static_cast<const float*>(weight),
+                     static_cast<uint4*>(packed), Cin, ux_slices(Cin));
+  return check_launch("upconv3d_c1_pack");
+}
+
+extern "C" int ragmi_upconv3d_c1_uses_x3(int Cin, int Di, int Hi, int Wi, int dtype) {
+  return (dtype == RAGMI_F32X3 && Cin % 4 == 0 && ragmi_upconv3d_c1_supported(Cin, Di, Hi, Wi) && ragmi::ux_axis_regular(Hi) &&
+          ragmi::ux_axis_regular(Wi)) ? 1 : 0;
+}
diff --git a/rag_amd/modules.py b/rag_amd/modules.py
--- a/rag_amd/modules.py
+++ b/rag_amd/modules.py
@@ -100,6 +100,15 @@
                     scale = shift = None
             self._cache = (stamp, wk, scale, shift)
         return self._cache[1], self._cache[2], self._cache[3]
+
+    def head_pack(self) -> torch.Tensor:
+        wk = self.prepared()[0]
+        hit = getattr(self, "_head_pack", None)
+        if hit is None or hit[0] is not self._cache:
+            with torch.no_grad():
+                hit = (self._cache, ops.upconv3d_c1_pack(wk))
+            self._head_pack = hit
+        return hit[1]
 
     def autograd_mode(self, *inputs) -> bool:
         return (ag.needs_grad(*inputs, self.conv.weight, self.bn.weight, self.bn.bias)
@@ -806,7 +815,8 @@
             if (up is ops.trilinear3d and m3._small() and m3.conv.out_channels == 1 and tuple(y.shape[2:]) == (d // 2, h // 2, w // 2)
                     and (d, h, w) == (2 * (d // 2), 2 * (h // 2), 2 * (w // 2)) and ops.upconv3d_c1_supported(y.shape[1], d // 2, h // 2, w // 2)):
                 wk, scale, shift = m3.prepared()
-                return ops.upconv3d_c1(y, wk, scale, shift, m3.relu, out_dtype=f32)
+                packed = m3.head_pack() if ops.upconv3d_c1_uses_x3(y.shape[1], d // 2, h // 2, w // 2, y.dtype) else None
+                return ops.upconv3d_c1(y, wk, scale, shift, m3.relu, out_dtype=f32, packed=packed)
             return m3(up(y, (d, h, w), True), out_dtype=f32)
 
         if last_output.size()[3] == h // 2:
diff --git a/rag_amd/ops.py b/rag_amd/ops.py
--- a/rag_amd/ops.py
+++ b/rag_amd/ops.py
@@ -176,6 +176,27 @@
     if not load_library().ragmi_quarter_store_rows(int(n_in), used):
         return None
     return [bool(v) for v in used]
+
+
+UPCONV_SELECT_BODY, UPCONV_NO_X3 = 1, 2
+_HEAD_X3 = [os.environ.get("RAGMI_HEAD_X3", "0") != "0"]
+_HEAD_SELECT_BODY = [False]
+
+
+def set_head_x3(enabled: bool) -> None:
+    _HEAD_X3[0] = bool(enabled)
+
+
+def head_x3_enabled() -> bool:
+    return _HEAD_X3[0]
+
+
+def set_head_select_body(enabled: bool) -> None:
+    _HEAD_SELECT_BODY[0] = bool(enabled)
+
+
+def head_select_body_enabled() -> bool:
+    return _HEAD_SELECT_BODY[0]
 
 
 def set_g4(enabled: bool) -> None:
@@ -617,8 +638,26 @@
     return bool(load_library().ragmi_upconv3d_c1_supported(int(cin), int(di), int(hi), int(wi)))
 
 
+def upconv3d_c1_uses_x3(cin: int, di: int, hi: int, wi: int, dtype: torch.dtype = torch.float32) -> bool:
+    return bool(_HEAD_X3[0] and load_library().ragmi_upconv3d_c1_uses_x3(int(cin), int(di), int(hi), int(wi), _conv_dt(_DT[dtype])))
+
+
+def upconv3d_c1_pack(weight: torch.Tensor) -> torch.Tensor:
+    _need_gpu(weight)
+    if weight.dim() != 5 or weight.shape[0] != 1 or tuple(weight.shape[2:]) != (3, 3, 3):
+        raise ValueError("upconv3d_c1_pack: weight must be [1, Cin, 3, 3, 3]")
+    cin = int(weight.shape[1])
+    nbytes = int(load_library().ragmi_upconv3d_c1_pack_bytes(cin))
+    if nbytes <= 0:
+        raise ValueError(f"upconv3d_c1_pack: {cin} input channels not built")
+    packed = torch.empty((nbytes,), device=weight.device, dtype=torch.uint8)
+    check(load_library().ragmi_upconv3d_c1_pack(weight.detach().contiguous().data_ptr(), cin, packed.data_ptr(), _stream()), "upconv3d_c1_pack")
+    return packed
+
+
 def upconv3d_c1(x: torch.Tensor, weight: torch.Tensor, scale: Optional[torch.Tensor], shift: Optional[torch.Tensor], relu: bool,
-                out: Optional[torch.Tensor] = None, out_ch0: int = 0, out_dtype: Optional[torch.dtype] = None) -> torch.Tensor:
+                out: Optional[torch.Tensor] = None, out_ch0: int = 0, out_dtype: Optional[torch.dtype] = None,
+                packed: Optional[torch.Tensor] = None) -> torch.Tensor:
     _need_gpu(weight, scale, shift)
     dt = _act(x)
     B, Cin, Di, Hi, Wi = x.shape
@@ -629,10 +668,18 @@
     ydt = _act(out)
     if tuple(out.shape[2:]) != (2 * Di, 2 * Hi, 2 * Wi) or out.shape[0] != B or out_ch0 >= out.shape[1]:
         raise ValueError("upconv3d_c1: out must be [B, >= out_ch0 + 1, 2Di, 2Hi, 2Wi]")
+    flags = (UPCONV_SELECT_BODY if _HEAD_SELECT_BODY[0] else 0) | (0 if _HEAD_X3[0] else UPCONV_NO_X3)
+    if ydt == F32:
+        dt = _conv_dt(dt)
+    if dt == F32X3 and upconv3d_c1_uses_x3(Cin, Di, Hi, Wi, x.dtype):
+        if packed is None:
+            packed = upconv3d_c1_pack(weight)
+    else:
+        packed = None
     ptr = lambda t: t.data_ptr() if t is not None else None
-    check(load_library().ragmi_upconv3d_c1_fwd(x.data_ptr(), _planes(x), weight.detach().contiguous().data_ptr(), ptr(scale), ptr(shift),
-                                               int(relu), out.data_ptr(), _planes(out), int(out_ch0), B, Cin, Di, Hi, Wi, dt, ydt, _stream()),
-          "upconv3d_c1")
+    check(load_library().ragmi_upconv3d_c1_fwd_ex(x.data_ptr(), _planes(x), weight.detach().contiguous().data_ptr(), ptr(packed), ptr(scale),
+                                                  ptr(shift), int(relu), out.data_ptr(), _planes(out), int(out_ch0), B, Cin, Di, Hi, Wi, dt,
+                                                  F32 if dt == F32X3 else ydt, flags, _stream()), "upconv3d_c1")
     return out
 
 
```

Result: no change. 1136 disparity maps/s (-0.4%).
